# CrashCartCapital/rust-local-rag

Measured on AMD Instinct MI355X. Metric: queries/sec, 768-d cosine top-100 over 10M chunks (single query, f32), higher is better.
Workload: dtype f32

## Files before the change

rust-local-rag_amd/build.py:

```python
from __future__ import annotations

import os
import subprocess
import sys
from concurrent.futures import ThreadPoolExecutor

HERE = os.path.dirname(os.path.abspath(__file__))
CSRC = os.path.join(HERE, "csrc")
OBJ = os.path.join(HERE, "_obj")
SO = os.path.join(HERE, "librlr_gpu.so")
ROOT = os.path.dirname(HERE)

SOURCES = ["scan.hip", "select.hip", "tail.hip", "exact.hip", "gemm.hip", "index.hip", "engine.cpp", "multi.cpp", "lexical.hip", "q8.hip",
           "jsonio.cpp", "text_batch.cpp"]
HEADERS = ["common.h", "kernels.h", "exact_dot.h", "lds_select.h", "staged_dot.h", "select_dev.h", "sort_emit.h", "pool_prepare.h",
           "engine_host.h", "lexical_internal.h", os.path.join(ROOT, "include", "rlr_gpu.h"),
           os.path.join(ROOT, "include", "rlr_engine.h"), os.path.join(ROOT, "include", "rlr_lexical.h")]

FLAGS = ["--offload-arch=gfx950", "-O3", "-std=c++17", "-fPIC", "-ffp-contract=off", "-fno-fast-math",
         "-Wall", "-Wno-unused-function", "-I", os.path.join(ROOT, "include")]


def _hipcc() -> str:
    for c in (os.environ.get("HIPCC"), "/opt/rocm/bin/hipcc", "hipcc"):
        if c and (os.path.isabs(c) and os.path.exists(c) or not os.path.isabs(c)):
            return c
    return "hipcc"


def _newest_header() -> float:
    t = 0.0
    for h in HEADERS:
        p = h if os.path.isabs(h) else os.path.join(CSRC, h)
        if os.path.exists(p):
            t = max(t, os.path.getmtime(p))
    return t


def _compile(src: str, force: bool, keep_temps: bool) -> str:
    sp = os.path.join(CSRC, src)
    obj = os.path.join(OBJ, os.path.splitext(src)[0] + ".o")
    stale = force or not os.path.exists(obj) or os.path.getmtime(obj) < max(os.path.getmtime(sp), _newest_header())
    if stale:
        cmd = [_hipcc(), *FLAGS, "-c", sp, "-o", obj]
        if src.endswith(".cpp"):
            cmd.insert(1, "-x")
            cmd.insert(2, "hip")
        if keep_temps:
            cmd += ["-save-temps=obj"]
        r = subprocess.run(cmd, capture_output=True, text=True, cwd=OBJ)
        if r.returncode != 0:
            raise RuntimeError(f"hipcc failed for {src}:\n{r.stdout}\n{r.stderr}")
        if r.stderr.strip():
            sys.stderr.write(r.stderr)
    return obj


def build(force: bool = False, keep_temps: bool = False) -> str:
    os.makedirs(OBJ, exist_ok=True)
    srcs = [s for s in SOURCES if os.path.exists(os.path.join(CSRC, s))]
    with ThreadPoolExecutor(max_workers=min(6, len(srcs))) as ex:
        objs = list(ex.map(lambda s: _compile(s, force, keep_temps), srcs))
    if force or not os.path.exists(SO) or any(os.path.getmtime(o) > os.path.getmtime(SO) for o in objs):
        cmd = [_hipcc(), "--offload-arch=gfx950", "-shared", "-fPIC", "-o", SO, *objs]
        r = subprocess.run(cmd, capture_output=True, text=True)
        if r.returncode != 0:
            raise RuntimeError(f"link failed:\n{r.stdout}\n{r.stderr}")
    return SO


if __name__ == "__main__":
    print(build(force="--force" in sys.argv, keep_temps="--keep-temps" in sys.argv))
```

rust-local-rag_amd/csrc/exact.hip:

```cpp
#include "common.h"
#include "exact_dot.h"
#include "staged_dot.h"
#include "sort_emit.h"
#include "kernels.h"
#include "../../include/rlr_gpu.h"

#include <algorithm>
#include <atomic>
#include <cstdlib>
#include <cstring>

namespace rlr {

namespace {

__device__ inline void stage_query(float *s_q, const float *__restrict__ query, uint32_t dim)
{
    for (uint32_t i = threadIdx.x; i < dim; i += blockDim.x)
        s_q[i] = query[i];
    __syncthreads();
}

template <bool F16>
__global__ __launch_bounds__(64) void rescore_kernel(const float4 *__restrict__ rows, uint32_t pitch16,
                                                     uint32_t dim, const float *__restrict__ query,
                                                     const uint32_t *__restrict__ cand,
                                                     const SelectState *__restrict__ st,
                                                     uint64_t *__restrict__ packed_out, uint32_t n_pad)
{
    extern __shared__ __attribute__((aligned(16))) float s_q[];
    stage_query(s_q, query, dim);
    const uint32_t n = min(st->n_cand, st->cap);
    const uint32_t i = blockIdx.x * 64 + threadIdx.x;
    if (i >= n_pad)
        return;
    if (i >= n) {
        packed_out[i] = 0;
        return;
    }
    const uint32_t r = cand[i];
    const float s = dot_ref_row<F16>(rows + static_cast<size_t>(r) * pitch16, s_q, dim);
    packed_out[i] = pack_result(s, r);
}

template <bool F16>
__global__ __launch_bounds__(256) void rescore_staged_kernel(const float4 *__restrict__ rows, uint32_t pitch16,
                                                             uint32_t dim, const float *__restrict__ query,
                                                             const uint32_t *__restrict__ cand,
                                                             const SelectState *__restrict__ st,
                                                             uint64_t *__restrict__ packed_out, uint32_t cpb,
                                                             uint32_t *__restrict__ hist_clear)
{
    extern __shared__ __attribute__((aligned(16))) float s_mem[];
    const uint32_t q_floats = (dim + 7) & ~7u;
    float *s_q = s_mem;
    float *s_p = s_mem + q_floats;
    const uint32_t tid = threadIdx.x;
    const uint32_t gid = blockIdx.x * 256 + tid;
    if (hist_clear && gid < 2 * kHistBins)
        hist_clear[gid] = 0;
    const uint32_t n = min(st->n_cand, st->cap);
    const uint32_t base = blockIdx.x * cpb;
    if (base >= n)
        return;
    const uint32_t cnt = min(cpb, n - base);
    __shared__ uint32_t s_cand[16];
    for (uint32_t i = tid; i < q_floats; i += 256)
        s_q[i] = i < dim ? query[i] : 0.0f;
    if (tid < cnt)
        s_cand[tid] = cand[base + tid];
    __syncthreads();
    const float sc = staged_reference_dot<F16>(rows, pitch16, dim, s_q, s_p, s_cand, cnt, tid);
    if (tid < cnt)
        packed_out[base + tid] = pack_result(sc, s_cand[tid]);
}

template <bool F16>
__global__ __launch_bounds__(256) void batch_rescore_kernel(const float4 *__restrict__ rows, uint32_t pitch16,
                                                            uint32_t dim, const float *__restrict__ queries,
                                                            uint32_t q_pitch, uint64_t *__restrict__ band,
                                                            uint32_t band_stride, const SelectState *__restrict__ st,
                                                            uint32_t cpb)
{
    extern __shared__ __attribute__((aligned(16))) float s_mem[];
    const uint32_t q_floats = (dim + 7) & ~7u;
    float *s_q = s_mem;
    float *s_p = s_mem + q_floats;
    __shared__ uint32_t s_cand[16];
    const uint32_t tid = threadIdx.x;
    const uint32_t q = blockIdx.y;
    const uint32_t n = st[q].pad;
    if (blockIdx.x * cpb >= n)
        return;
    const float *query = queries + static_cast<size_t>(q) * q_pitch;
    for (uint32_t i = tid; i < q_floats; i += 256)
        s_q[i] = i < dim ? query[i] : 0.0f;
    uint64_t *b = band + static_cast<size_t>(q) * band_stride;
    for (uint32_t base = blockIdx.x * cpb; base < n; base += gridDim.x * cpb) {
        const uint32_t cnt = min(cpb, n - base);
        __syncthreads();
        if (tid < cnt)
            s_cand[tid] = 0xFFFFFFFFu - static_cast<uint32_t>(b[base + tid] & 0xFFFFFFFFu);
        __syncthreads();
        const float sc = staged_reference_dot<F16>(rows, pitch16, dim, s_q, s_p, s_cand, cnt, tid);
        if (tid < cnt)
            b[base + tid] = pack_result(sc, s_cand[tid]);
    }
}

template <bool F16>
__global__ __launch_bounds__(64) void score_rows_kernel(const float4 *__restrict__ rows, uint32_t pitch16,
                                                        uint32_t dim, const float *__restrict__ query,
                                                        const uint32_t *__restrict__ list, uint32_t n,
                                                        float *__restrict__ out, const uint32_t *__restrict__ n_dev,
                                                        uint32_t n_rows_clamp)
{
    extern __shared__ __attribute__((aligned(16))) float s_q[];
    stage_query(s_q, query, dim);
    if (n_dev)
        n = min(n, *n_dev);
    const uint32_t i = blockIdx.x * 64 + threadIdx.x;
    if (i >= n)
        return;
    const uint32_t r = list[i] < n_rows_clamp ? list[i] : 0u;
    out[i] = dot_ref_row<F16>(rows + static_cast<size_t>(r) * pitch16, s_q, dim);
}

template <bool F16>
__global__ __launch_bounds__(64) void score_rows_batch_kernel(const float4 *__restrict__ rows, uint32_t pitch16, uint32_t dim,
                                                              const float *__restrict__ queries, uint32_t q_pitch,
                                                              const uint32_t *__restrict__ list, uint32_t stride,
                                                              float *__restrict__ out, const uint32_t *__restrict__ n_dev,
                                                              uint32_t n_dev_stride, uint32_t n_rows_clamp)
{
    const uint32_t q = blockIdx.y;
    const uint32_t n = min(stride, n_dev[static_cast<size_t>(q) * n_dev_stride]);
    if (blockIdx.x * 64 >= n)
        return;
    extern __shared__ __attribute__((aligned(16))) float s_q[];
    stage_query(s_q, queries + static_cast<size_t>(q) * q_pitch, dim);
    const uint32_t i = blockIdx.x * 64 + threadIdx.x;
    if (i >= n)
        return;
    const size_t at = static_cast<size_t>(q) * stride + i;
    const uint32_t r = list[at] < n_rows_clamp ? list[at] : 0u;
    out[at] = dot_ref_row<F16>(rows + static_cast<size_t>(r) * pitch16, s_q, dim);
}

template <bool F16>
__global__ __launch_bounds__(256) void score_rows_staged_kernel(const float4 *__restrict__ rows, uint32_t pitch16, uint32_t dim,
                                                               const float *__restrict__ query,
                                                               const uint32_t *__restrict__ list, uint32_t n,
                                                               float *__restrict__ out, uint32_t cpb,
                                                               const uint32_t *__restrict__ n_dev, uint32_t n_rows_clamp)
{
    extern __shared__ __attribute__((aligned(16))) float s_mem[];
    const uint32_t q_floats = (dim + 7) & ~7u;
    float *s_q = s_mem;
    float *s_p = s_mem + q_floats;
    __shared__ uint32_t s_cand[16];
    const uint32_t tid = threadIdx.x;
    const uint32_t base = blockIdx.x * cpb;
    if (n_dev)
        n = min(n, *n_dev);
    if (base >= n)
        return;
    const uint32_t cnt = min(cpb, n - base);
    for (uint32_t i = tid; i < q_floats; i += 256)
        s_q[i] = i < dim ? query[i] : 0.0f;
    if (tid < cnt) {
        const uint32_t r = list[base + tid];
        s_cand[tid] = r < n_rows_clamp ? r : 0u;
    }
    __syncthreads();
    const float sc = staged_reference_dot<F16>(rows, pitch16, dim, s_q, s_p, s_cand, cnt, tid);
    if (tid < cnt)
        out[base + tid] = sc;
}

__global__ __launch_bounds__(64) void sumsq_kernel(const float *__restrict__ staging, uint32_t n,
                                                   uint32_t dim, float *__restrict__ sumsq)
{
    const uint32_t r = blockIdx.x * 64 + threadIdx.x;
    if (r >= n)
        return;
    const float *v = staging + static_cast<size_t>(r) * dim;
    float s = 0.0f;
    for (uint32_t c = 0; c < dim; ++c) {
        float p = v[c] * v[c];
        s = s + p;
    }
    sumsq[r] = s;
}

__device__ inline float sqrt_rn(float x)
{
    float y = __builtin_sqrtf(x);
    const double xd = static_cast<double>(x);
#pragma unroll
    for (int it = 0; it < 2; ++it) {
        const uint32_t yb = __builtin_bit_cast(uint32_t, y);
        const float up = __builtin_bit_cast(float, yb + 1u);
        const float dn = __builtin_bit_cast(float, yb - 1u);
        const double m_hi = 0.5 * (static_cast<double>(y) + static_cast<double>(up));
        const double m_lo = 0.5 * (static_cast<double>(y) + static_cast<double>(dn));
        if (xd > m_hi * m_hi)
            y = up;
        else if (xd < m_lo * m_lo)
            y = dn;
    }
    return y;
}

__device__ inline float ref_scale(float v, float norm_sq, int do_normalize)
{
    if (do_normalize && norm_sq > 1e-20f)
        return __fdiv_rn(v, sqrt_rn(norm_sq));
    return v;
}

template <bool F16>
__global__ __launch_bounds__(256) void scale_store_kernel(const float *__restrict__ staging,
                                                          const float *__restrict__ sumsq, uint32_t n,
                                                          uint32_t dim, int do_normalize,
                                                          void *__restrict__ rows_out, uint32_t pitch16)
{
    const uint32_t pitch_e = F16 ? pitch16 * 8 : pitch16 * 4;
    const size_t total = static_cast<size_t>(n) * pitch_e;
    const size_t stride = static_cast<size_t>(gridDim.x) * 256;
    for (size_t i = static_cast<size_t>(blockIdx.x) * 256 + threadIdx.x; i < total; i += stride) {
        const uint32_t r = static_cast<uint32_t>(i / pitch_e);
        const uint32_t c = static_cast<uint32_t>(i - static_cast<size_t>(r) * pitch_e);
        float v = 0.0f;
        if (c < dim)
            v = ref_scale(staging[static_cast<size_t>(r) * dim + c], do_normalize ? sumsq[r] : 0.0f,
                          do_normalize);
        if constexpr (F16)
            static_cast<_Float16 *>(rows_out)[i] = static_cast<_Float16>(v);
        else
            static_cast<float *>(rows_out)[i] = v;
    }
}

__device__ inline uint64_t mix64(uint64_t z)
{
    z = (z ^ (z >> 30)) * 0xBF58476D1CE4E5B9ULL;
    z = (z ^ (z >> 27)) * 0x94D049BB133111EBULL;
    return z ^ (z >> 31);
}

__device__ inline int32_t ih4(uint64_t h)
{
    return static_cast<int32_t>((h & 0xFFFF) + ((h >> 16) & 0xFFFF) + ((h >> 32) & 0xFFFF) + (h >> 48)) - 131070;
}

__device__ inline float synth_raw(uint64_t s, uint64_t row, uint32_t col, uint32_t d, uint32_t n_clusters)
{
    const uint64_t idx = row * static_cast<uint64_t>(d) + col;
    int32_t t = ih4(mix64(s + (idx + 1) * 0x9E3779B97F4A7C15ULL));
    const bool tight = (n_clusters & 0x80000000u) != 0;
    n_clusters &= 0x7FFFFFFFu;
    if (n_clusters) {
        const uint64_t cl = mix64(s ^ (row + 0x632BE59BD9B4E019ULL)) % n_clusters;
        const uint64_t cidx = cl * static_cast<uint64_t>(d) + col;
        const int32_t c = ih4(mix64((s ^ 0xC1A57E55C1A57E55ULL) + (cidx + 1) * 0x9E3779B97F4A7C15ULL));
        if (tight)
            t = t / 16;
        t += 2 * c;
    }
    return static_cast<float>(t) * (1.0f / 65536.0f);
}

__global__ __launch_bounds__(64) void synth_sumsq_kernel(uint64_t s, uint64_t row0, uint32_t n, uint32_t dim,
                                                         uint32_t n_clusters, float *__restrict__ sumsq)
{
    const uint32_t r = blockIdx.x * 64 + threadIdx.x;
    if (r >= n)
        return;
    float acc = 0.0f;
    for (uint32_t c = 0; c < dim; ++c) {
        const float v = synth_raw(s, row0 + r, c, dim, n_clusters);
        float p = v * v;
        acc = acc + p;
    }
    sumsq[r] = acc;
}

template <bool F16>
__global__ __launch_bounds__(256) void synth_store_kernel(uint64_t s, uint64_t row0, uint32_t n, uint32_t dim,
                                                          uint32_t n_clusters, const float *__restrict__ sumsq,
                                                          void *__restrict__ rows_out, uint32_t pitch16)
{
    const uint32_t pitch_e = F16 ? pitch16 * 8 : pitch16 * 4;
    const size_t total = static_cast<size_t>(n) * pitch_e;
    const size_t stride = static_cast<size_t>(gridDim.x) * 256;
    for (size_t i = static_cast<size_t>(blockIdx.x) * 256 + threadIdx.x; i < total; i += stride) {
        const uint32_t r = static_cast<uint32_t>(i / pitch_e);
        const uint32_t c = static_cast<uint32_t>(i - static_cast<size_t>(r) * pitch_e);
        float v = 0.0f;
        if (c < dim)
            v = ref_scale(synth_raw(s, row0 + r, c, dim, n_clusters), sumsq[r], 1);
        if constexpr (F16)
            static_cast<_Float16 *>(rows_out)[i] = static_cast<_Float16>(v);
        else
            static_cast<float *>(rows_out)[i] = v;
    }
}

template <bool F16>
__global__ __launch_bounds__(256) void gather_f32_kernel(const void *__restrict__ rows, uint32_t pitch16,
                                                         uint32_t dim, const uint32_t *__restrict__ list,
                                                         uint32_t n, float *__restrict__ out)
{
    const size_t total = static_cast<size_t>(n) * dim;
    const size_t stride = static_cast<size_t>(gridDim.x) * 256;
    for (size_t i = static_cast<size_t>(blockIdx.x) * 256 + threadIdx.x; i < total; i += stride) {
        const uint32_t k = static_cast<uint32_t>(i / dim);
        const uint32_t c = static_cast<uint32_t>(i - static_cast<size_t>(k) * dim);
        const size_t r = list[k];
        if constexpr (F16)
            out[i] = h2f(static_cast<const uint16_t *>(rows)[r * pitch16 * 8 + c]);
        else
            out[i] = static_cast<const float *>(rows)[r * pitch16 * 4 + c];
    }
}

__global__ __launch_bounds__(256) void compact_rows_kernel(const float4 *__restrict__ src, float4 *__restrict__ dst,
                                                           uint32_t pitch16, const uint32_t *__restrict__ keep,
                                                           uint32_t n_keep)
{
    const size_t total = static_cast<size_t>(n_keep) * pitch16;
    const size_t stride = static_cast<size_t>(gridDim.x) * 256;
    for (size_t i = static_cast<size_t>(blockIdx.x) * 256 + threadIdx.x; i < total; i += stride) {
        const uint32_t k = static_cast<uint32_t>(i / pitch16);
        const uint32_t u = static_cast<uint32_t>(i - static_cast<size_t>(k) * pitch16);
        dst[i] = src[static_cast<size_t>(keep[k]) * pitch16 + u];
    }
}

__device__ inline bool finite_f(float x)
{
    return (__builtin_bit_cast(uint32_t, x) & 0x7F800000u) != 0x7F800000u;
}

__device__ inline float gram_entry(float dot)
{
    return finite_f(dot) ? dot : -__builtin_inff();
}

__global__ __launch_bounds__(64) void gram_kernel(const float *__restrict__ pool, uint32_t P, uint32_t dim,
                                                  float *__restrict__ gram)
{
    pool += static_cast<size_t>(blockIdx.z) * P * dim;
    gram += static_cast<size_t>(blockIdx.z) * P * P;
    const uint32_t i = blockIdx.y;
    const uint32_t j = blockIdx.x * 64 + threadIdx.x;
    if (j > i || i >= P)
        return;
    const float *a = pool + static_cast<size_t>(i) * dim;
    const float *b = pool + static_cast<size_t>(j) * dim;
    float s = 0.0f;
    uint32_t c = 0;
    if ((dim & 3u) == 0) {
        const float4 *a4 = reinterpret_cast<const float4 *>(a);
        const float4 *b4 = reinterpret_cast<const float4 *>(b);
        for (; c + 16 <= dim; c += 16) {
            float4 x[4], y[4];
#pragma unroll
            for (int u = 0; u < 4; ++u) {
                x[u] = a4[c / 4 + u];
                y[u] = b4[c / 4 + u];
            }
#pragma unroll
            for (int u = 0; u < 4; ++u) {
                float p;
                p = x[u].x * y[u].x; s = s + p;
                p = x[u].y * y[u].y; s = s + p;
                p = x[u].z * y[u].z; s = s + p;
                p = x[u].w * y[u].w; s = s + p;
            }
        }
    }
    for (; c < dim; ++c) {
        float p = a[c] * b[c];
        s = s + p;
    }
    s = gram_entry(s);
    gram[static_cast<size_t>(i) * P + j] = s;
    gram[static_cast<size_t>(j) * P + i] = s;
}

template <int SRC>
__device__ inline float4 gram_load4(const float *pool, const void *rows, uint32_t pitch16, uint32_t dim, uint32_t row, uint32_t col)
{
    if constexpr (SRC == 2) {
        const uint2 h = *reinterpret_cast<const uint2 *>(static_cast<const uint16_t *>(rows) + static_cast<size_t>(row) * pitch16 * 8 + col);
        return make_float4(h2f(static_cast<uint16_t>(h.x)), h2f(static_cast<uint16_t>(h.x >> 16)), h2f(static_cast<uint16_t>(h.y)),
                           h2f(static_cast<uint16_t>(h.y >> 16)));
    } else if constexpr (SRC == 1) {
        return *reinterpret_cast<const float4 *>(static_cast<const float *>(rows) + static_cast<size_t>(row) * pitch16 * 4 + col);
    } else {
        return *reinterpret_cast<const float4 *>(pool + static_cast<size_t>(row) * dim + col);
    }
}


template <int R, int SRC, int GK>
__global__ __launch_bounds__(256) void gram_tiled_kernel(const float *__restrict__ pool, uint32_t P, uint32_t dim,
                                                         float *__restrict__ gram, const void *__restrict__ rows,
                                                         uint32_t pitch16, const uint32_t *__restrict__ list)
{
    constexpr int kGT = 16 * R;
    constexpr int kGK = GK, kGPitch = GK + 4;
    __shared__ __attribute__((aligned(16))) float sa[kGT * kGPitch];
    __shared__ __attribute__((aligned(16))) float sb[kGT * kGPitch];
    if constexpr (SRC == 0)
        pool += static_cast<size_t>(blockIdx.z) * P * dim;
    else
        list += static_cast<size_t>(blockIdx.z) * P;
    gram += static_cast<size_t>(blockIdx.z) * P * P;
    uint32_t bi = 0, rem = blockIdx.x;
    while (rem > bi) {
        rem -= bi + 1;
        ++bi;
    }
    const uint32_t bj = rem;
    const uint32_t i0 = bi * kGT, j0 = bj * kGT;
    const uint32_t t = threadIdx.x, ty = t >> 4, tx = t & 15;
    float acc[R][R];
#pragma unroll
    for (int a = 0; a < R; ++a)
#pragma unroll
        for (int b = 0; b < R; ++b)
            acc[a][b] = 0.0f;
    const bool vec = (dim & 3u) == 0;
    constexpr int kPre = 2 * kGT * (kGK / 4) / 256;
    float4 pre[kPre];
    uint32_t src_row[kPre];
#pragma unroll
    for (int u = 0; u < kPre; ++u) {
        const uint32_t r = (t + 256 * u) / (kGK / 4);
        const uint32_t row = min(r >= kGT ? j0 + (r - kGT) : i0 + r, P - 1);
        src_row[u] = SRC == 0 ? row : list[row];
    }
    auto fetch = [&](uint32_t k0) {
        const uint32_t kc = min(static_cast<uint32_t>(kGK), dim - k0);
        if (vec) {
#pragma unroll
            for (int u = 0; u < kPre; ++u) {
                const uint32_t idx = t + 256 * u;
                const uint32_t r = idx / (kGK / 4), c4 = idx % (kGK / 4);
                const uint32_t row = r >= kGT ? j0 + (r - kGT) : i0 + r;
                const float4 v = gram_load4<SRC>(pool, rows, pitch16, dim, src_row[u], min(k0 + c4 * 4, dim - 4));
                pre[u] = (row < P && c4 * 4 < kc) ? v : make_float4(0.0f, 0.0f, 0.0f, 0.0f);
            }
            return;
        }
#pragma unroll
        for (int u = 0; u < kPre; ++u) {
            const uint32_t idx = t + 256 * u;
            const uint32_t r = idx / (kGK / 4), c4 = idx % (kGK / 4);
            const uint32_t row = r >= kGT ? j0 + (r - kGT) : i0 + r;
            float4 v = make_float4(0.0f, 0.0f, 0.0f, 0.0f);
            if (row < P && c4 * 4 < kc) {
                const uint32_t col = k0 + c4 * 4;
                if constexpr (SRC == 2) {
                    const uint16_t *src = static_cast<const uint16_t *>(rows) + static_cast<size_t>(src_row[u]) * pitch16 * 8 + col;
                    v.x = h2f(src[0]);
                    if (c4 * 4 + 1 < kc) v.y = h2f(src[1]);
                    if (c4 * 4 + 2 < kc) v.z = h2f(src[2]);
                    if (c4 * 4 + 3 < kc) v.w = h2f(src[3]);
                } else {
                    const float *src = SRC == 0 ? pool + static_cast<size_t>(row) * dim + col
                                                : static_cast<const float *>(rows) + static_cast<size_t>(src_row[u]) * pitch16 * 4 + col;
                    v.x = src[0];
                    if (c4 * 4 + 1 < kc) v.y = src[1];
                    if (c4 * 4 + 2 < kc) v.z = src[2];
                    if (c4 * 4 + 3 < kc) v.w = src[3];
                }
            }
            pre[u] = v;
        }
    };
    auto stash = [&]() {
#pragma unroll
        for (int u = 0; u < kPre; ++u) {
            const uint32_t idx = t + 256 * u;
            const uint32_t r = idx / (kGK / 4), c4 = idx % (kGK / 4);
            float *dst = (r >= kGT ? sb + (r - kGT) * kGPitch : sa + r * kGPitch) + c4 * 4;
            *reinterpret_cast<float4 *>(dst) = pre[u];
        }
    };
    fetch(0);
    stash();
    __syncthreads();
    for (uint32_t k0 = 0; k0 < dim; k0 += kGK) {
        const uint32_t kc = min(static_cast<uint32_t>(kGK), dim - k0);
        const bool more = k0 + kGK < dim;
        if (more)
            fetch(k0 + kGK);
        const uint32_t n4 = kc / 4;
        constexpr int kUnroll = R == 1 ? 8 : 1;
#pragma unroll kUnroll
        for (uint32_t c = 0; c < n4; ++c) {
            float4 xa[R], yb[R];
#pragma unroll
            for (int a = 0; a < R; ++a)
                xa[a] = reinterpret_cast<const float4 *>(sa + (ty + 16 * a) * kGPitch)[c];
#pragma unroll
            for (int b = 0; b < R; ++b)
                yb[b] = reinterpret_cast<const float4 *>(sb + (tx + 16 * b) * kGPitch)[c];
#pragma unroll
            for (int a = 0; a < R; ++a)
#pragma unroll
                for (int b = 0; b < R; ++b) {
                    float p;
                    p = xa[a].x * yb[b].x; acc[a][b] = acc[a][b] + p;
                    p = xa[a].y * yb[b].y; acc[a][b] = acc[a][b] + p;
                    p = xa[a].z * yb[b].z; acc[a][b] = acc[a][b] + p;
                    p = xa[a].w * yb[b].w; acc[a][b] = acc[a][b] + p;
                }
        }
        for (uint32_t e = n4 * 4; e < kc; ++e) {
#pragma unroll
            for (int a = 0; a < R; ++a)
#pragma unroll
                for (int b = 0; b < R; ++b) {
                    const float p = sa[(ty + 16 * a) * kGPitch + e] * sb[(tx + 16 * b) * kGPitch + e];
                    acc[a][b] = acc[a][b] + p;
                }
        }
        __syncthreads();
        if (more) {
            stash();
            __syncthreads();
        }
    }
#pragma unroll
    for (int a = 0; a < R; ++a)
#pragma unroll
        for (int b = 0; b < R; ++b) {
            const uint32_t ri = i0 + ty + 16 * a, cj = j0 + tx + 16 * b;
            if (ri < P && cj < P) {
                const float g = gram_entry(acc[a][b]);
                gram[static_cast<size_t>(ri) * P + cj] = g;
                gram[static_cast<size_t>(cj) * P + ri] = g;
            }
        }
}

__global__ __launch_bounds__(64) void mmr_greedy_kernel(const float *__restrict__ gram,
                                                        const float *__restrict__ scores, uint32_t P,
                                                        uint32_t k, float lambda, uint32_t *__restrict__ out_order,
                                                        float *__restrict__ out_mmr, uint32_t *__restrict__ out_n)
{
    extern __shared__ __attribute__((aligned(16))) unsigned char s_raw[];
    uint32_t *rem = reinterpret_cast<uint32_t *>(s_raw);
// ... 779 lines not shown
```

rust-local-rag_amd/csrc/exact_dot.h:

```cpp
#pragma once

#include "common.h"

namespace rlr {

template <bool F16>
__device__ inline float dot_ref_row(const float4 *__restrict__ row, const float *s_q, uint32_t dim)
{
    float s = 0.0f;
    constexpr uint32_t EPU = F16 ? 8 : 4;
    const uint32_t full = dim / EPU;
    uint32_t u = 0;
    for (; u + 4 <= full; u += 4) {
        float4 x[4];
#pragma unroll
        for (int i = 0; i < 4; ++i)
            x[i] = row[u + i];
#pragma unroll
        for (int i = 0; i < 4; ++i) {
            const float *q = s_q + (u + i) * EPU;
            if constexpr (F16) {
                const uint32_t w[4] = {__builtin_bit_cast(uint32_t, x[i].x), __builtin_bit_cast(uint32_t, x[i].y),
                                       __builtin_bit_cast(uint32_t, x[i].z), __builtin_bit_cast(uint32_t, x[i].w)};
#pragma unroll
                for (int j = 0; j < 4; ++j) {
                    float p0 = h2f(static_cast<uint16_t>(w[j] & 0xFFFF)) * q[2 * j];
                    s = s + p0;
                    float p1 = h2f(static_cast<uint16_t>(w[j] >> 16)) * q[2 * j + 1];
                    s = s + p1;
                }
            } else {
                float p;
                p = x[i].x * q[0]; s = s + p;
                p = x[i].y * q[1]; s = s + p;
                p = x[i].z * q[2]; s = s + p;
                p = x[i].w * q[3]; s = s + p;
            }
        }
    }
    if constexpr (F16) {
        const uint16_t *h = reinterpret_cast<const uint16_t *>(row);
        for (uint32_t e = u * EPU; e < dim; ++e) {
            float p = h2f(h[e]) * s_q[e];
            s = s + p;
        }
    } else {
        const float *f = reinterpret_cast<const float *>(row);
        for (uint32_t e = u * EPU; e < dim; ++e) {
            float p = f[e] * s_q[e];
            s = s + p;
        }
    }
    return s;
}

}
```

rust-local-rag_amd/csrc/gemm.hip:

```cpp
#include "common.h"
#include "exact_dot.h"
#include "kernels.h"
#include "lds_select.h"
#include "../../include/rlr_gpu.h"

#include <cstdlib>

namespace rlr {

namespace {

typedef _Float16 half8 __attribute__((ext_vector_type(8)));
typedef _Float16 half2v __attribute__((ext_vector_type(2)));
typedef float f32x4 __attribute__((ext_vector_type(4)));

constexpr int kQB = 256;
constexpr int kNB = kQB / 16;
constexpr int kRG = 2;
constexpr int kGemmWaves = 8;
constexpr int kBM = kGemmWaves * kRG * 16;
constexpr int kKsChunk = 2;
constexpr int kChunkFrags = kKsChunk * kNB * 64;

__global__ __launch_bounds__(256) void prep_queries_kernel(const float *__restrict__ q, uint32_t n_queries,
                                                           uint32_t q_pitch, uint32_t dim, uint32_t n_ksteps,
                                                           uint32_t n_qblocks, int f16_rows,
                                                           _Float16 *__restrict__ out)
{
    const size_t total = static_cast<size_t>(n_qblocks) * n_ksteps * kNB * 64 * 8;
    for (size_t e = static_cast<size_t>(blockIdx.x) * 256 + threadIdx.x; e < total; e += static_cast<size_t>(gridDim.x) * 256) {
        const uint32_t j = e & 7;
        const uint32_t lane = (e >> 3) & 63;
        const uint32_t nb = (e >> 9) & (kNB - 1);
        const size_t rest = e >> 13;
        const uint32_t ks = static_cast<uint32_t>(rest % n_ksteps);
        const uint32_t qb = static_cast<uint32_t>(rest / n_ksteps);
        const uint32_t query = qb * kQB + nb * 16 + (lane & 15);
        const uint32_t g = lane >> 4;
        const uint32_t k = ks * 32 + (f16_rows ? g * 8 + j : (j < 4 ? g * 4 + j : 16 + g * 4 + (j - 4)));
        float v = 0.0f;
        if (query < n_queries && k < dim)
            v = q[static_cast<size_t>(query) * q_pitch + k];
        out[e] = static_cast<_Float16>(v);
    }
}

__device__ inline half8 cvt8(float4 lo, float4 hi)
{
    half8 r;
    r[0] = static_cast<_Float16>(lo.x);
    r[1] = static_cast<_Float16>(lo.y);
    r[2] = static_cast<_Float16>(lo.z);
    r[3] = static_cast<_Float16>(lo.w);
    r[4] = static_cast<_Float16>(hi.x);
    r[5] = static_cast<_Float16>(hi.y);
    r[6] = static_cast<_Float16>(hi.z);
    r[7] = static_cast<_Float16>(hi.w);
    return r;
}

struct GemmArgs {
    const unsigned char *rows;
    uint32_t pitch_bytes;
    uint32_t row_begin, row_end;
    uint32_t n_ksteps;
    const half8 *qfrag;
    uint32_t n_qblocks, n_queries;
    const float *tau;
    uint64_t *cand;
    uint32_t cand_stride;
    SelectState *st;
    float *scores;
    size_t score_stride;
    uint32_t *sync;
    uint32_t sync_every;
    uint32_t a_nt_shared;
};

template <bool MATERIALISE>
__device__ __forceinline__ void gemm_epilogue(const GemmArgs &a, f32x4 (&acc)[kRG][kNB], uint32_t row0, uint32_t last_row,
                                              uint32_t qb, int lane)
{
    const uint32_t qcol = qb * kQB + (lane & 15);
    if constexpr (MATERIALISE) {
#pragma unroll
        for (int rg = 0; rg < kRG; ++rg) {
            const uint32_t r = row0 + rg * 16 + 4 * (lane >> 4);
            const uint32_t rel = r - a.row_begin;
#pragma unroll
            for (int nb = 0; nb < kNB; ++nb) {
                const uint32_t q = qcol + nb * 16;
                if (q >= a.n_queries)
                    continue;
                float *dst = a.scores + static_cast<size_t>(q) * a.score_stride + rel;
                const f32x4 v = acc[rg][nb];
                if (r + 3 <= last_row) {
                    *reinterpret_cast<float4 *>(dst) = make_float4(v[0], v[1], v[2], v[3]);
                } else {
#pragma unroll
                    for (int i = 0; i < 4; ++i)
                        if (r + i <= last_row)
                            dst[i] = v[i];
                }
            }
        }
    } else {
        float tau_l[kNB];
#pragma unroll
        for (int nb = 0; nb < kNB; ++nb) {
            const uint32_t q = qcol + nb * 16;
            tau_l[nb] = q < a.n_queries ? a.tau[q] : __builtin_inff();
        }
#pragma unroll
        for (int rg = 0; rg < kRG; ++rg) {
            const uint32_t r = row0 + rg * 16 + 4 * (lane >> 4);
#pragma unroll
            for (int nb = 0; nb < kNB; ++nb) {
                const f32x4 v = acc[rg][nb];
                const float t = tau_l[nb];
                if (v[0] >= t || v[1] >= t || v[2] >= t || v[3] >= t) {
                    const uint32_t q = qcol + nb * 16;
#pragma unroll
                    for (int i = 0; i < 4; ++i) {
                        if (v[i] >= t && r + i <= last_row) {
                            const uint32_t slot = atomicAdd(&a.st[q].n_cand, 1u);
                            if (slot < a.st[q].cap)
                                a.cand[static_cast<size_t>(q) * a.cand_stride + slot] = pack_result(v[i], r + i);
                        }
                    }
                }
            }
        }
    }
}

template <bool F16ROWS, bool MATERIALISE>
__global__ __launch_bounds__(512) void gemm_nominate_kernel(const GemmArgs a)
{
    __shared__ half8 s_b[2][kChunkFrags];

    const int tid = threadIdx.x;
    const int lane = tid & 63;
    const int wave = __builtin_amdgcn_readfirstlane(tid >> 6);
    const uint32_t bid = blockIdx.x;
    const uint32_t rt = (bid / (8 * a.n_qblocks)) * 8 + (bid & 7);
    const uint32_t qb = (bid >> 3) % a.n_qblocks;
    const uint32_t n_rows = a.row_end - a.row_begin;
    if (rt * kBM >= n_rows)
        return;
    const uint32_t row0 = a.row_begin + rt * kBM + wave * (kRG * 16);
    const uint32_t last_row = a.row_end - 1;

    const unsigned char *ap[kRG];
#pragma unroll
    for (int rg = 0; rg < kRG; ++rg) {
        const uint32_t r = min(row0 + rg * 16 + (lane & 15), last_row);
        ap[rg] = a.rows + static_cast<size_t>(r) * a.pitch_bytes + (lane >> 4) * 16;
    }
    constexpr int kStepBytes = F16ROWS ? 64 : 128;

    const uint32_t n_chunks = a.n_ksteps / kKsChunk;
    const half8 *bsrc = a.qfrag + static_cast<size_t>(qb) * a.n_ksteps * kNB * 64;

    f32x4 acc[kRG][kNB];
#pragma unroll
    for (int rg = 0; rg < kRG; ++rg)
#pragma unroll
        for (int nb = 0; nb < kNB; ++nb)
            acc[rg][nb] = f32x4{0.0f, 0.0f, 0.0f, 0.0f};

    half8 breg[4];
    float4 araw[kRG][kKsChunk][2];
    half8 a_cur[kRG][kKsChunk];

    auto load_b = [&](uint32_t c) {
#pragma unroll
        for (int i = 0; i < 4; ++i)
            breg[i] = bsrc[static_cast<size_t>(c) * kChunkFrags + tid + 512 * i];
    };
    auto store_b = [&](int buf) {
#pragma unroll
        for (int i = 0; i < 4; ++i)
            s_b[buf][tid + 512 * i] = breg[i];
    };
    auto load_a = [&](uint32_t c) {
#pragma unroll
        for (int rg = 0; rg < kRG; ++rg)
#pragma unroll
            for (int ks = 0; ks < kKsChunk; ++ks) {
                const unsigned char *p = ap[rg] + static_cast<size_t>(c * kKsChunk + ks) * kStepBytes;
                if constexpr (F16ROWS) {
                    araw[rg][ks][0] = *reinterpret_cast<const float4 *>(p);
                } else {
                    araw[rg][ks][0] = *reinterpret_cast<const float4 *>(p);
                    araw[rg][ks][1] = *reinterpret_cast<const float4 *>(p + 64);
                }
            }
    };
    auto convert_a = [&]() {
#pragma unroll
        for (int rg = 0; rg < kRG; ++rg)
#pragma unroll
            for (int ks = 0; ks < kKsChunk; ++ks) {
                if constexpr (F16ROWS)
                    a_cur[rg][ks] = __builtin_bit_cast(half8, araw[rg][ks][0]);
                else
                    a_cur[rg][ks] = cvt8(araw[rg][ks][0], araw[rg][ks][1]);
            }
    };

    load_b(0);
    load_a(0);
    store_b(0);
    convert_a();
    __syncthreads();

#pragma unroll 1
    for (uint32_t c = 0; c < n_chunks; ++c) {
        const bool has_next = c + 1 < n_chunks;
        if (has_next) {
            load_b(c + 1);
            load_a(c + 1);
        }
        const half8 *sb = s_b[c & 1];
#pragma unroll
        for (int ks = 0; ks < kKsChunk; ++ks) {
#pragma unroll
            for (int nb = 0; nb < kNB; ++nb) {
                const half8 b = sb[(ks * kNB + nb) * 64 + lane];
#pragma unroll
                for (int rg = 0; rg < kRG; ++rg)
                    acc[rg][nb] = __builtin_amdgcn_mfma_f32_16x16x32_f16(a_cur[rg][ks], b, acc[rg][nb], 0, 0, 0);
            }
        }
        if (has_next) {
            store_b((c + 1) & 1);
            convert_a();
        }
        __syncthreads();
    }

    gemm_epilogue<MATERIALISE>(a, acc, row0, last_row, qb, lane);
}

template <bool F16ROWS>
__global__ __launch_bounds__(256) void build_image_kernel(const unsigned char *__restrict__ rows, uint32_t pitch_bytes,
                                                          uint32_t n_rows, uint32_t n_chunks, uint32_t tile_begin,
                                                          uint32_t tile_end, half8 *__restrict__ image)
{
    const size_t per_tile = static_cast<size_t>(n_chunks) * 8 * 4 * 64;
    const size_t first = static_cast<size_t>(tile_begin) * per_tile;
    const size_t total = static_cast<size_t>(tile_end - tile_begin) * per_tile;
    for (size_t i = static_cast<size_t>(blockIdx.x) * 256 + threadIdx.x; i < total; i += static_cast<size_t>(gridDim.x) * 256) {
        const size_t e = first + i;
        const uint32_t lane = e & 63;
        const uint32_t ks = (e >> 6) & 1;
        const uint32_t rg = (e >> 7) & 1;
        const uint32_t w = (e >> 8) & 7;
        const size_t tc = e >> 11;
        const uint32_t c = static_cast<uint32_t>(tc % n_chunks);
        const uint32_t t = static_cast<uint32_t>(tc / n_chunks);
        const uint32_t row = t * 256 + w * 32 + rg * 16 + (lane & 15);
        const uint32_t k = c * 64 + ks * 32 + (lane >> 4) * 8;
        half8 v;
#pragma unroll
        for (int j = 0; j < 8; ++j)
            v[j] = static_cast<_Float16>(0.0f);
        if (row < n_rows) {
            const unsigned char *src = rows + static_cast<size_t>(row) * pitch_bytes;
            if constexpr (F16ROWS) {
                v = *reinterpret_cast<const half8 *>(src + k * 2);
            } else {
                const float4 lo = *reinterpret_cast<const float4 *>(src + k * 4);
                const float4 hi = *reinterpret_cast<const float4 *>(src + k * 4 + 16);
                v = cvt8(lo, hi);
            }
        }
        image[e] = v;
    }
}

constexpr int kRGI = 4;

template <bool MATERIALISE, int NBW>
__device__ __forceinline__ void gemm_image_epilogue(const GemmArgs &a, f32x4 (&acc)[kRGI][NBW], uint32_t row0,
                                                    uint32_t last_row, uint32_t q0, int lane)
{
    constexpr int kNBI = NBW;
    const uint32_t qcol = q0 + (lane & 15);
    if constexpr (MATERIALISE) {
#pragma unroll
        for (int rg = 0; rg < kRGI; ++rg) {
            const uint32_t r = row0 + rg * 16 + 4 * (lane >> 4);
            const uint32_t rel = r - a.row_begin;
#pragma unroll
            for (int nb = 0; nb < kNBI; ++nb) {
                const uint32_t q = qcol + nb * 16;
                if (q >= a.n_queries)
                    continue;
                float *dst = a.scores + static_cast<size_t>(q) * a.score_stride + rel;
                const f32x4 v = acc[rg][nb];
                if (r + 3 <= last_row) {
                    *reinterpret_cast<float4 *>(dst) = make_float4(v[0], v[1], v[2], v[3]);
                } else {
#pragma unroll
                    for (int i = 0; i < 4; ++i)
                        if (r + i <= last_row)
                            dst[i] = v[i];
                }
            }
        }
    } else {
        float tau_l[kNBI];
#pragma unroll
        for (int nb = 0; nb < kNBI; ++nb) {
            const uint32_t q = qcol + nb * 16;
            tau_l[nb] = q < a.n_queries ? a.tau[q] : __builtin_inff();
        }
#pragma unroll
        for (int rg = 0; rg < kRGI; ++rg) {
            const uint32_t r = row0 + rg * 16 + 4 * (lane >> 4);
#pragma unroll
            for (int nb = 0; nb < kNBI; ++nb) {
                const f32x4 v = acc[rg][nb];
                const float t = tau_l[nb];
                if (v[0] >= t || v[1] >= t || v[2] >= t || v[3] >= t) {
                    const uint32_t q = qcol + nb * 16;
#pragma unroll
                    for (int i = 0; i < 4; ++i) {
                        if (v[i] >= t && r + i <= last_row) {
                            const uint32_t slot = atomicAdd(&a.st[q].n_cand, 1u);
                            if (slot < a.st[q].cap)
                                a.cand[static_cast<size_t>(q) * a.cand_stride + slot] = pack_result(v[i], r + i);
                        }
                    }
                }
            }
        }
    }
}

constexpr int kHalfBytes = 16384;
constexpr uint32_t kG8ListCap = 2048;
constexpr int kG8OffPack = 8 * kHalfBytes;
constexpr int kG8OffQid = kG8OffPack + kG8ListCap * 8;
constexpr int kG8OffTau = kG8OffQid + kG8ListCap * 4;
constexpr int kG8OffCnt = kG8OffTau + 2 * 256 * 4;
constexpr int kG8LdsBytes = kG8OffCnt + 64;

#define RLR_GLDS16(src, dst)                                                                               \
    __builtin_amdgcn_global_load_lds((const __attribute__((address_space(1))) void *)(src),                \
                                     (__attribute__((address_space(3))) void *)(dst), 16, 0, 0)
#define RLR_FENCE() asm volatile("" ::: "memory")

__device__ __forceinline__ uint32_t lds_add_rtn_u32(uint32_t addr, uint32_t v)
{
    uint32_t r;
// ... 441 lines not shown
                                                                                 acc[rg][nb], 0, 0, 0);
                }
                RLR_RES_LOAD_A(min(cc + kResSlots, last_c), sl);
                __builtin_amdgcn_sched_barrier(0);
            }
        }
    }
#undef RLR_RES_LOAD_A
    gemm_image_epilogue<MATERIALISE, kResNB>(a, acc, row0, last_row, qg * kResQ, lane);
}

constexpr uint32_t kFinCap = 8192;
constexpr uint32_t kBandCap = 2048;

__device__ inline void bitonic_desc_lds(uint64_t *s, uint32_t n_pad, uint32_t nthreads)
{
    for (uint32_t k = 2; k <= n_pad; k <<= 1) {
        for (uint32_t j = k >> 1; j > 0; j >>= 1) {
            for (uint32_t i = threadIdx.x; i < n_pad; i += nthreads) {
                const uint32_t ixj = i ^ j;
                if (ixj > i) {
                    const uint64_t x = s[i], y = s[ixj];
                    const bool desc = (i & k) == 0;
                    if (desc ? (x < y) : (x > y)) {
                        s[i] = y;
                        s[ixj] = x;
                    }
                }
            }
            __syncthreads();
        }
    }
}

template <bool F16ROWS>
__global__ __launch_bounds__(256) void batch_finish_kernel(const float4 *__restrict__ rows, uint32_t pitch16, uint32_t dim,
                                                           const float *__restrict__ queries, uint32_t q_pitch,
                                                           const uint64_t *__restrict__ cand, uint32_t cand_stride,
                                                           const SelectState *__restrict__ st, uint32_t k, float two_eps,
                                                           uint64_t *__restrict__ out, uint32_t *__restrict__ status)
{
    __shared__ uint64_t s_c[kFinCap];
    __shared__ uint32_t s_band;
    extern __shared__ __attribute__((aligned(16))) float s_q[];
    const uint32_t q = blockIdx.x;
    const uint32_t n_raw = st[q].n_cand;
    uint64_t *o = out + static_cast<size_t>(q) * k;
    if (n_raw > st[q].cap || n_raw > kFinCap || n_raw < k) {
        if (threadIdx.x == 0)
            status[q] = n_raw < k ? 2u : 1u;
        return;
    }
    for (uint32_t i = threadIdx.x; i < dim; i += 256)
        s_q[i] = queries[static_cast<size_t>(q) * q_pitch + i];
    uint32_t n_pad = 1;
    while (n_pad < n_raw)
        n_pad <<= 1;
    const uint64_t *c = cand + static_cast<size_t>(q) * cand_stride;
    for (uint32_t i = threadIdx.x; i < n_pad; i += 256)
        s_c[i] = i < n_raw ? c[i] : 0ull;
    if (threadIdx.x == 0)
        s_band = 0;
    __syncthreads();
    bitonic_desc_lds(s_c, n_pad, 256);
    const float fk = key_score(static_cast<uint32_t>(s_c[k - 1] >> 32));
    const uint32_t key_lo = score_key(fk - two_eps);
    if (key_lo < st[q].key_lo) {
        if (threadIdx.x == 0)
            status[q] = 2u;
        return;
    }
    for (uint32_t i = threadIdx.x; i < n_raw; i += 256)
        if (static_cast<uint32_t>(s_c[i] >> 32) >= key_lo)
            atomicMax(&s_band, i + 1);
    __syncthreads();
    const uint32_t band = s_band;
    if (band > kBandCap) {
        if (threadIdx.x == 0)
            status[q] = 1u;
        return;
    }
    for (uint32_t i = threadIdx.x; i < band; i += 256) {
        const uint32_t r = 0xFFFFFFFFu - static_cast<uint32_t>(s_c[i] & 0xFFFFFFFFu);
        const float e = dot_ref_row<F16ROWS>(rows + static_cast<size_t>(r) * pitch16, s_q, dim);
        s_c[i] = pack_result(e, r);
    }
    uint32_t b_pad = 1;
    while (b_pad < band)
        b_pad <<= 1;
    for (uint32_t i = band + threadIdx.x; i < b_pad; i += 256)
        s_c[i] = 0ull;
    __syncthreads();
    bitonic_desc_lds(s_c, b_pad, 256);
    for (uint32_t i = threadIdx.x; i < k; i += 256)
        o[i] = s_c[i];
    if (threadIdx.x == 0)
        status[q] = 0u;
}

__global__ __launch_bounds__(1024) void batch_band_kernel(uint64_t *__restrict__ cand, uint32_t cand_stride,
                                                          SelectState *__restrict__ st, uint32_t k, float two_eps,
                                                          uint32_t *__restrict__ status)
{
    __shared__ uint64_t s_c[kFinCap];
    __shared__ uint32_t s_hist[2048];
    __shared__ uint32_t s_sel[3];
    __shared__ uint32_t s_band;
    const uint32_t q = blockIdx.x;
    const uint32_t n_raw = st[q].n_cand;
    if (n_raw > st[q].cap || n_raw > kFinCap || n_raw < k) {
        if (threadIdx.x == 0) {
            status[q] = n_raw < k ? 2u : 1u;
            st[q].pad = 0;
        }
        return;
    }
    uint64_t *c = cand + static_cast<size_t>(q) * cand_stride;
    for (uint32_t i = threadIdx.x; i < n_raw; i += 1024)
        s_c[i] = c[i];
    if (threadIdx.x == 0)
        s_band = 0;
    __syncthreads();
    const float fk = key_score(lds_kth_key(s_c, n_raw, k, s_hist, s_sel, 1024));
    const uint32_t key_lo = score_key(fk - two_eps);
    if (key_lo < st[q].key_lo) {
        if (threadIdx.x == 0) {
            status[q] = 2u;
            st[q].pad = 0;
        }
        return;
    }
    for (uint32_t i = threadIdx.x; i < n_raw; i += 1024) {
        const uint64_t v = s_c[i];
        if (static_cast<uint32_t>(v >> 32) >= key_lo) {
            const uint32_t slot = atomicAdd(&s_band, 1u);
            if (slot < kBandCap)
                c[slot] = v;
        }
    }
    __syncthreads();
    const uint32_t band = s_band;
    if (threadIdx.x == 0) {
        if (band > kBandCap) {
            status[q] = 1u;
            st[q].pad = 0;
        } else {
            st[q].pad = band;
            status[q] = 0u;
        }
    }
}

__global__ __launch_bounds__(1024) void batch_tighten_kernel(uint64_t *__restrict__ cand, uint32_t cand_stride,
                                                             SelectState *__restrict__ st, uint32_t k, float two_eps,
                                                             float *__restrict__ tau)
{
    __shared__ uint64_t s_c[kFinCap];
    __shared__ uint32_t s_keep;
    const uint32_t q = blockIdx.x;
    const uint32_t n_raw = st[q].n_cand;
    if (n_raw > st[q].cap || n_raw > kFinCap || n_raw < k)
        return;
    uint32_t n_pad = 1;
    while (n_pad < n_raw)
        n_pad <<= 1;
    uint64_t *c = cand + static_cast<size_t>(q) * cand_stride;
    for (uint32_t i = threadIdx.x; i < n_pad; i += 1024)
        s_c[i] = i < n_raw ? c[i] : 0ull;
    if (threadIdx.x == 0)
        s_keep = 0;
    __syncthreads();
    bitonic_desc_lds(s_c, n_pad, 1024);
    const float fk = key_score(static_cast<uint32_t>(s_c[k - 1] >> 32));
    const uint32_t key_lo = score_key(fk - two_eps);
    for (uint32_t i = threadIdx.x; i < n_raw; i += 1024)
        if (static_cast<uint32_t>(s_c[i] >> 32) >= key_lo)
            atomicMax(&s_keep, i + 1);
    __syncthreads();
    const uint32_t keep = s_keep;
    for (uint32_t i = threadIdx.x; i < keep; i += 1024)
        c[i] = s_c[i];
    if (threadIdx.x == 0) {
        st[q].n_cand = keep;
        tau[q] = key_lo == 0 ? -__builtin_inff() : key_score(key_lo);
    }
}

__global__ __launch_bounds__(1024) void batch_emit_kernel(const uint64_t *__restrict__ cand, uint32_t cand_stride,
                                                          const SelectState *__restrict__ st, uint32_t k,
                                                          uint64_t *__restrict__ out)
{
    __shared__ uint64_t s_c[kBandCap];
    const uint32_t q = blockIdx.x;
    const uint32_t band = st[q].pad;
    if (band == 0)
        return;
    uint32_t b_pad = 1;
    while (b_pad < band)
        b_pad <<= 1;
    const uint64_t *c = cand + static_cast<size_t>(q) * cand_stride;
    for (uint32_t i = threadIdx.x; i < b_pad; i += 1024)
        s_c[i] = i < band ? c[i] : 0ull;
    __syncthreads();
    bitonic_desc_lds(s_c, b_pad, 1024);
    uint64_t *o = out + static_cast<size_t>(q) * k;
    for (uint32_t i = threadIdx.x; i < k; i += 1024)
        o[i] = s_c[i];
}

}

float nomination_eps(uint32_t dim, int dtype, float prod, float norm_sum)
{
    const float op = dtype == RLR_F16 ? 4.8828125e-4f : 9.765625e-4f;
    const float acc = 2.0f * (static_cast<float>(dim) + 64.0f) * 5.9604645e-8f;
    const float sub = 2.9802322e-8f * __builtin_sqrtf(static_cast<float>(dim));
    return ((op * 1.001f + acc) * prod + sub * norm_sum) * 1.0625f;
}

hipError_t launch_prep_queries(const float *q, uint32_t n_queries, uint32_t q_pitch, uint32_t dim, int dtype,
                               void *qfrag, hipStream_t s)
{
    const uint32_t n_ksteps = dim / 32;
    const uint32_t n_qblocks = (n_queries + kQB - 1) / kQB;
    const size_t total = static_cast<size_t>(n_qblocks) * n_ksteps * kNB * 64 * 8;
    const uint32_t blocks = static_cast<uint32_t>(std::min<size_t>((total + 255) / 256, 4096));
    hipLaunchKernelGGL(prep_queries_kernel, dim3(blocks), dim3(256), 0, s, q, n_queries, q_pitch, dim, n_ksteps,
                       n_qblocks, dtype == RLR_F16 ? 1 : 0, static_cast<_Float16 *>(qfrag));
    return hipGetLastError();
}

bool gemm_image_usable(uint32_t dim)
{
    return dim % 128 == 0;
}

static uint32_t persistent_grid()
{
    static uint32_t cus[64] = {0};
    int dev = 0;
    if (hipGetDevice(&dev) != hipSuccess || dev < 0 || dev >= 64)
        return 256;
    if (cus[dev] == 0) {
        int n = 0;
        if (hipDeviceGetAttribute(&n, hipDeviceAttributeMultiprocessorCount, dev) != hipSuccess || n < 8)
            n = 256;
        cus[dev] = static_cast<uint32_t>(n) / 8 * 8;
    }
    return cus[dev];
}

hipError_t launch_gemm_nominate(const void *rows, uint32_t pitch16, uint32_t dim, int dtype, uint32_t row_begin,
                                uint32_t row_end, const void *qfrag, uint32_t n_queries, const float *tau,
                                uint64_t *cand, uint32_t cand_stride, SelectState *st, float *scores,
                                size_t score_stride, const void *image, hipStream_t s, uint32_t *sync_ws)
{
    if (row_end <= row_begin)
        return hipSuccess;
    GemmArgs a;
    a.rows = static_cast<const unsigned char *>(rows);
    a.pitch_bytes = pitch16 * 16;
    a.row_begin = row_begin;
    a.row_end = row_end;
    a.n_ksteps = dim / 32;
    a.qfrag = static_cast<const half8 *>(qfrag);
    a.n_qblocks = (n_queries + kQB - 1) / kQB;
    a.n_queries = n_queries;
    a.tau = tau;
    a.cand = cand;
    a.cand_stride = cand_stride;
    a.st = st;
    a.scores = scores;
    a.score_stride = score_stride;
    a.sync = nullptr;
    a.sync_every = 4;
    a.a_nt_shared = 0;
    const uint32_t n_rt = (row_end - row_begin + kBM - 1) / kBM;
    const uint32_t grid = ((n_rt + 7) / 8) * 8 * a.n_qblocks;
    const bool mat = scores != nullptr;
    static const uint32_t resident_max = [] {
        const char *v = getenv("RLR_GEMM_RESIDENT_MAX");
        return v ? static_cast<uint32_t>(strtoul(v, nullptr, 0)) : 128u;
    }();
    if (image && n_queries <= resident_max && row_begin % kBM == 0 && a.n_ksteps <= kResMaxKsteps &&
        a.n_ksteps % (kKsChunk * kResSlots) == 0) {
        const half8 *img = static_cast<const half8 *>(image);
        const uint32_t n_qg = (n_queries + kResQ - 1) / kResQ;
        const uint32_t n_rg = (row_end - row_begin + kResRows - 1) / kResRows;
        const uint32_t rgrid = ((n_rg + 7) / 8) * 8 * n_qg;
        if (mat)
            hipLaunchKernelGGL((gemm_resident_kernel<true>), dim3(rgrid), dim3(512), 0, s, a, img, n_qg);
        else
            hipLaunchKernelGGL((gemm_resident_kernel<false>), dim3(rgrid), dim3(512), 0, s, a, img, n_qg);
        return hipGetLastError();
    }
    if (image && row_begin % kBM == 0 && a.n_ksteps % 4 == 0) {
        const uint32_t n_units = n_rt * a.n_qblocks;
        const uint32_t g8 = std::max<uint32_t>(8, std::min<uint32_t>(persistent_grid(), (n_units + 7) / 8 * 8));
        const char *img = static_cast<const char *>(image);
        static const bool no_sync = getenv("RLR_GEMM8_NO_SIBLING_SYNC") != nullptr;
        if (sync_ws && a.n_qblocks > 1 && g8 == persistent_grid() && !no_sync) {
            const hipError_t e = hipMemsetAsync(sync_ws, 0, 256 * sizeof(uint32_t), s);
            if (e != hipSuccess)
                return e;
            a.sync = sync_ws;
            static const uint32_t every = getenv("RLR_GEMM8_SYNC_EVERY") ? static_cast<uint32_t>(std::max(1, atoi(getenv("RLR_GEMM8_SYNC_EVERY")))) : 4u;
            a.sync_every = every;
        }
        static const bool a_nt = getenv("RLR_GEMM8_A_NT") != nullptr;
        a.a_nt_shared = a_nt ? 1u : 0u;
        static const int var = [] {
// ... 127 lines not shown
```

rust-local-rag_amd/csrc/index.hip:

```cpp
#include "../../include/rlr_gpu.h"
#include "common.h"
#include "kernels.h"
#include "lds_select.h"
#include "sort_emit.h"
#include "pool_prepare.h"
#include "lexical_internal.h"

#include <algorithm>
#include <atomic>
#include <chrono>
#include <cmath>
#include <condition_variable>
#include <cstdarg>
#include <cstdio>
#include <cstring>
#include <mutex>
#include <memory>
#include <new>
#include <string>
#include <thread>
#include <vector>

#include <time.h>

using namespace rlr;

namespace {

thread_local char g_err[512] = "";

int32_t fail(int32_t code, const char *fmt, ...)
{
    va_list ap;
    va_start(ap, fmt);
    vsnprintf(g_err, sizeof(g_err), fmt, ap);
    va_end(ap);
    return code;
}

}

namespace rlr {
int32_t set_error(int32_t code, const char *fmt, ...)
{
    va_list ap;
    va_start(ap, fmt);
    vsnprintf(g_err, sizeof(g_err), fmt, ap);
    va_end(ap);
    return code;
}
}

namespace {

#define RLR_HIP(call)                                                                              \
    do {                                                                                           \
        hipError_t e_ = (call);                                                                    \
        if (e_ != hipSuccess)                                                                      \
            return fail(e_ == hipErrorOutOfMemory ? RLR_E_OOM : RLR_E_HIP, "%s failed: %s (%s:%d)", \
                        #call, hipGetErrorString(e_), __FILE__, __LINE__);                         \
    } while (0)

#define RLR_TRY(call)                                                                              \
    do {                                                                                           \
        int32_t s_ = (call);                                                                       \
        if (s_ != RLR_OK)                                                                          \
            return s_;                                                                             \
    } while (0)

constexpr uint32_t kLdsSortCap = 4096;
constexpr uint32_t kMaxDim = 8192;

uint32_t next_pow2(uint32_t v)
{
    uint32_t p = 1;
    while (p < v)
        p <<= 1;
    return p;
}

struct RowBlock {
    void *raw = nullptr;
    size_t raw_bytes = 0;
    std::vector<hipMemGenericAllocationHandle_t> handles;
    size_t slab = 0;
// ... 10 lines not shown
    float *d_query = nullptr;
    uint32_t q_cap = 0;
    float *d_scores = nullptr;
    uint64_t score_cap = 0;
    uint32_t *d_hist = nullptr;
    SelectState *d_state = nullptr;
    uint32_t *d_cand = nullptr;
    uint64_t *d_packed = nullptr;
    uint32_t cand_cap = 0;
    uint64_t *d_out = nullptr;
    uint64_t out_cap = 0;
    uint32_t *d_list = nullptr;
    float *d_vals = nullptr;
    uint32_t list_cap = 0;
    float *d_pool = nullptr;
    uint64_t pool_cap = 0;
    void *d_qfrag = nullptr;
    uint64_t qfrag_cap = 0;
    float *d_tau = nullptr;
    SelectState *d_bstate = nullptr;
    uint32_t *d_bhist = nullptr;
    uint32_t *d_bstatus = nullptr;
    uint32_t *d_gsync = nullptr;
    void *h_batch = nullptr;
    uint32_t bq_cap = 0;
    bool no_f16 = false;
    uint64_t *d_bcand = nullptr;
    uint64_t bcand_cap = 0;
    float *d_sample = nullptr;
    uint64_t sample_cap = 0;
    hipEvent_t bev[5] = {nullptr, nullptr, nullptr, nullptr, nullptr};
    void *h_pin = nullptr;
    size_t h_pin_bytes = 0;
    std::vector<float> q_norm;
    WaitEma wait_ema;
    const float *h_q_kq = nullptr;
    bool hist_dirty = false;
    uint32_t *h_assert = nullptr;
    hipStream_t pending_stream = nullptr;
    uint32_t pending_q = 0, pending_k = 0;
    bool pending_timed = false;
    const uint64_t *pending_meta = nullptr;
};

struct CoalesceMember {
    const float *query;
    uint32_t k;
    uint64_t *rows_out;
    float *cos_out;
    uint32_t *n_out;
};

struct CoalesceGroup {
    uint32_t key = 0;
    uint32_t cap = 0;
    std::vector<CoalesceMember *> members;
    bool sealed = false;
    bool go = false;
    bool done = false;
    int32_t status = 0;
    char msg[512] = "";
};

}

struct rlr_index {
    uint32_t dim = 0;
    int32_t dtype = RLR_F32;
    int32_t device = 0;
    uint32_t pitch16 = 0;
    uint32_t q_pitch = 0;
    uint64_t n_rows = 0;
    uint64_t cap_rows = 0;
    void *d_rows = nullptr;
    RowBlock rows_block;
    int n_cu = 256;
    int scan_variant = 0;
    int fused_tail = -1;
    uint32_t tail_direct_max = 3584;
    bool hybrid_fetch_full = false;
    uint32_t batch_min = 0;
    float max_row_sumsq = 1.0f;
    bool f16_overflow = false;
    bool image_enabled = false;
    bool image_scan = false;
    bool q8_enabled = false;
    void *d_q8 = nullptr;
    float *d_q8_scale = nullptr;
    uint32_t *d_q8_stats = nullptr;
    uint64_t q8_cap_rows = 0;
    float q8_delta = 0.0f, q8_scale_max = 0.0f;
    bool q8_has_inf = false;
    void *d_image = nullptr;
    size_t image_cap = 0;
    std::mutex mu;
    std::condition_variable ctx_cv;
    std::vector<Ctx *> free_ctx;
    int ctx_made = 0;
    int ctx_cap = 16;
    bool profiling = false;
    rlr_profile prof{};
    std::atomic<uint32_t> co_max{0};
    uint32_t co_linger_us = 0;
    std::mutex co_mu;
    std::condition_variable co_cv;
    int co_running = 0;
    std::vector<std::shared_ptr<CoalesceGroup>> co_pending;
    rlr_coalesce_stats co_stats{};
};

namespace {

size_t row_bytes(const rlr_index *ix)
{
    return static_cast<size_t>(ix->pitch16) * 16;
}

}

namespace rlr {
bool poison_mode()
{
    static const bool poison = [] {
        const char *v = getenv("RLR_POISON_ALLOC");
        return v && v[0] == '1';
    }();
    return poison;
}

hipError_t dev_malloc(void **p, size_t bytes)
{
    const bool poison = poison_mode();
    hipError_t e = hipMalloc(p, bytes);
    if (e != hipSuccess)
        (void)hipGetLastError();
    if (e == hipSuccess && poison && bytes) {
        e = hipMemset(*p, 0xFF, bytes);
        if (e == hipSuccess)
            e = hipDeviceSynchronize();
    }
    return e;
}
}

namespace {
int32_t use_device(const rlr_index *ix)
{
    RLR_HIP(hipSetDevice(ix->device));
    return RLR_OK;
}

template <typename T>
int32_t grow(T **p, uint64_t *cap, uint64_t want, bool keep = false)
{
    if (*cap >= want && *p)
        return RLR_OK;
    T *n = nullptr;
    RLR_HIP(rlr::dev_malloc(reinterpret_cast<void **>(&n), want * sizeof(T)));
    if (keep && *p && *cap) {
        RLR_HIP(hipMemcpy(n, *p, *cap * sizeof(T), hipMemcpyDeviceToDevice));
        RLR_HIP(hipStreamSynchronize(nullptr));
    }
    if (*p)
        (void)hipFree(*p);
    *p = n;
    *cap = want;
// ... 452 lines not shown
    const uint64_t want = std::max<uint64_t>(ix->cap_rows, ix->n_rows);
    if (ix->q8_cap_rows < want || !ix->d_q8) {
        if (ix->d_q8) (void)hipFree(ix->d_q8);
        if (ix->d_q8_scale) (void)hipFree(ix->d_q8_scale);
        ix->d_q8 = nullptr;
        ix->d_q8_scale = nullptr;
        ix->q8_cap_rows = 0;
        RLR_HIP(rlr::dev_malloc(&ix->d_q8, std::max<uint64_t>(want, 1) * ix->dim));
        RLR_HIP(rlr::dev_malloc(reinterpret_cast<void **>(&ix->d_q8_scale), std::max<uint64_t>(want, 1) * sizeof(float)));
        ix->q8_cap_rows = want;
        first_row = 0;
    }
    if (!ix->d_q8_stats)
        RLR_HIP(rlr::dev_malloc(reinterpret_cast<void **>(&ix->d_q8_stats), 4 * sizeof(uint32_t)));
    if (first_row == 0)
        RLR_HIP(hipMemset(ix->d_q8_stats, 0, 4 * sizeof(uint32_t)));
    RLR_HIP(launch_q8_build(ix->d_rows, ix->pitch16, ix->dim, ix->dtype, static_cast<uint32_t>(first_row),
                            static_cast<uint32_t>(ix->n_rows), ix->d_q8, ix->d_q8_scale, ix->d_q8_stats, nullptr));
    uint32_t h[4] = {0, 0, 0, 0};
    RLR_HIP(hipMemcpy(h, ix->d_q8_stats, sizeof(h), hipMemcpyDeviceToHost));
    std::memcpy(&ix->q8_delta, &h[0], 4);
    std::memcpy(&ix->q8_scale_max, &h[1], 4);
    ix->q8_has_inf = h[2] != 0;
    return RLR_OK;
}

int32_t sync_image(rlr_index *ix, uint64_t first_row)
{
    RLR_TRY(sync_q8(ix, first_row));
    if (!ix->image_enabled)
        return RLR_OK;
    const size_t need = image_bytes(ix->dim, std::max<uint64_t>(ix->cap_rows, ix->n_rows));
    if (ix->image_cap < need) {
        if (ix->d_image)
            (void)hipFree(ix->d_image);
        ix->d_image = nullptr;
        ix->image_cap = 0;
        RLR_HIP(rlr::dev_malloc(&ix->d_image, std::max<size_t>(need, 256)));
        ix->image_cap = std::max<size_t>(need, 256);
        first_row = 0;
    }
    const uint32_t t0 = static_cast<uint32_t>(first_row / 256);
    const uint32_t t1 = static_cast<uint32_t>((ix->n_rows + 255) / 256);
    RLR_HIP(launch_build_image(ix->d_rows, ix->pitch16, ix->dim, ix->dtype, static_cast<uint32_t>(ix->n_rows), t0, t1,
                               ix->d_image, nullptr));
    RLR_HIP(hipStreamSynchronize(nullptr));
    return RLR_OK;
}

static bool beyond_f16(const float *v, uint32_t n)
{
    for (uint32_t i = 0; i < n; ++i)
        if (std::fabs(v[i]) > 65504.0f)
            return true;
    return false;
}

constexpr double kF16MaxSq = 65504.0 * 65504.0;

int32_t ingest(rlr_index *ix, const float *rows, uint64_t n, uint64_t first, int normalize)
{
    if (n == 0)
        return RLR_OK;
    const uint64_t chunk_rows = std::max<uint64_t>(1, (64ull << 20) / (static_cast<uint64_t>(ix->dim) * 4));
    float *d_stage = nullptr, *d_norm = nullptr;
    const uint64_t cr = std::min(chunk_rows, n);
    RLR_HIP(rlr::dev_malloc(reinterpret_cast<void **>(&d_stage), cr * ix->dim * sizeof(float)));
    hipError_t e = rlr::dev_malloc(reinterpret_cast<void **>(&d_norm), cr * sizeof(float));
    if (e != hipSuccess) {
        (void)hipFree(d_stage);
        return fail(RLR_E_OOM, "staging allocation failed");
    }
    int32_t st = RLR_OK;
    std::vector<float> h_norm;
    for (uint64_t r0 = 0; r0 < n && st == RLR_OK; r0 += cr) {
        const uint64_t m = std::min(cr, n - r0);
        e = hipMemcpy(d_stage, rows + r0 * ix->dim, m * ix->dim * sizeof(float), hipMemcpyHostToDevice);
        if (e == hipSuccess)
            e = launch_normalize_store(d_stage, static_cast<uint32_t>(m), ix->dim, normalize,
                                       static_cast<char *>(ix->d_rows) + (first + r0) * row_bytes(ix), ix->pitch16,
                                       ix->dtype, d_norm, nullptr);
        if (e == hipSuccess)
            e = hipStreamSynchronize(nullptr);
        if (e == hipSuccess && !normalize) {
            h_norm.resize(m);
            e = hipMemcpy(h_norm.data(), d_norm, m * sizeof(float), hipMemcpyDeviceToHost);
            for (uint64_t i = 0; i < m && e == hipSuccess; ++i) {
                if (h_norm[i] > ix->max_row_sumsq)
                    ix->max_row_sumsq = h_norm[i];
                if (ix->dtype == RLR_F32 && !ix->f16_overflow && h_norm[i] > 0.999 * kF16MaxSq &&
                    beyond_f16(rows + (r0 + i) * ix->dim, ix->dim))
                    ix->f16_overflow = true;
            }
        }
        if (e != hipSuccess)
            st = fail(RLR_E_HIP, "row ingest failed: %s", hipGetErrorString(e));
    }
    (void)hipFree(d_stage);
    (void)hipFree(d_norm);
    return st;
}

enum WaitMode { kWaitHybrid = 0, kWaitSpin = 1, kWaitBlock = 2 };

WaitMode wait_mode()
{
    static const WaitMode m = [] {
        const char *v = getenv("RLR_WAIT");
        if (v && v[0] == 's')
            return kWaitSpin;
        if (v && v[0] == 'b')
            return kWaitBlock;
        return kWaitHybrid;
    }();
    return m;
}

inline void cpu_relax()
{
#if defined(__x86_64__) || defined(__i386__)
    __builtin_ia32_pause();
#else
    __asm__ __volatile__("" ::: "memory");
#endif
}

template <typename Complete>
int32_t wait_polling(Complete &&complete, hipStream_t s, WaitEma *c, uint32_t key)
{
    using clk = std::chrono::steady_clock;
    const WaitMode mode = wait_mode();
    if (mode == kWaitBlock) {
        RLR_HIP(hipStreamSynchronize(s));
        return RLR_OK;
    }
    const auto t0 = clk::now();
    bool slept = false;
    if (c && c->key != key) {
        c->key = key;
        c->us = 0.0;
    }
    if (mode == kWaitHybrid && c && c->us > 1500.0) {
        const double sleep_us = 0.7 * c->us - 150.0;
        if (sleep_us > 20.0) {
            timespec ts;
            clock_gettime(CLOCK_MONOTONIC, &ts);
            const long add = static_cast<long>(sleep_us * 1000.0);
            ts.tv_sec += (ts.tv_nsec + add) / 1000000000L;
            ts.tv_nsec = (ts.tv_nsec + add) % 1000000000L;
            (void)clock_nanosleep(CLOCK_MONOTONIC, TIMER_ABSTIME, &ts, nullptr);
            slept = true;
        }
    }
    uint32_t polls = 0;
    for (;;) {
        std::atomic_thread_fence(std::memory_order_acquire);
        if (complete())
            break;
        if ((++polls & 0x3FFu) == 0) {
            const hipError_t e = hipStreamQuery(s);
            if (e == hipSuccess) {
                bool ok = false;
                for (int spin = 0; spin < 100000 && !ok; ++spin) {
                    std::atomic_thread_fence(std::memory_order_acquire);
                    ok = complete();
                    cpu_relax();
                }
                if (ok)
                    break;
// ... 633 lines not shown
        if (!status && got < n_rows && got > 0) {
            const float t0 = w_e * key_score(s_emin);
            const float t1 = w_l * 0.0f;
            const float c_tail = t0 + t1;
            const bool ok = n_cand >= need && (c_tail != c_tail || s_cneed > c_tail);
            if (!ok)
                status = 2u;
        }
        info[0] = status ? 0u : n_pool;
        info[1] = status;
        s_pick[0] = status;
    }
    if (h_out) {
        __syncthreads();
        const uint32_t status = s_pick[0];
        hybrid_emit_body(list, comb, cosv, lexv, status ? 0u : min(n_pool, k_cap), status, k_cap, h_out);
    }
}

__global__ __launch_bounds__(1024) void hybrid_pool_kernel(const uint64_t *__restrict__ packed, uint32_t fetch, uint32_t need,
                                                           uint32_t n_rows, float w_e, float w_l,
                                                           const uint32_t *__restrict__ lrow, const float *__restrict__ lscore,
                                                           const float *__restrict__ lcos,
                                                           const HybridLexHeader *__restrict__ hdr,
                                                           float *__restrict__ cand, uint32_t *__restrict__ list,
                                                           float *__restrict__ comb, float *__restrict__ cosv,
                                                           float *__restrict__ lexv, uint32_t *__restrict__ info,
                                                           uint32_t k_cap, uint32_t *__restrict__ h_out)
{
    hybrid_pool_body(packed, fetch, need, n_rows, w_e, w_l, lrow, lscore, lcos, hdr, cand, list, comb, cosv, lexv, info, k_cap,
                     h_out);
}

__global__ __launch_bounds__(1024) void hybrid_pool_batch_kernel(const uint64_t *__restrict__ packed, uint32_t fetch, uint32_t need,
                                                                 uint32_t n_rows, float w_e, float w_l, uint32_t bound,
                                                                 const uint32_t *__restrict__ lrow, const float *__restrict__ lscore,
                                                                 const float *__restrict__ lcos,
                                                                 const HybridLexHeader *__restrict__ hdr, float *__restrict__ cand,
                                                                 uint32_t *__restrict__ list, float *__restrict__ comb,
                                                                 float *__restrict__ cosv, float *__restrict__ lexv,
                                                                 uint32_t *__restrict__ info, uint32_t *__restrict__ sizes)
{
    const uint32_t q = blockIdx.x;
    const size_t lo = static_cast<size_t>(q) * bound, po = static_cast<size_t>(q) * need;
    hybrid_pool_body(packed + static_cast<size_t>(q) * fetch, fetch, need, n_rows, w_e, w_l, lrow + lo, lscore + lo, lcos + lo,
                     hdr + q, cand + static_cast<size_t>(q) * 3 * kHybridSlots, list + po, comb + po, cosv + po, lexv + po,
                     info + 2 * q, 0u, nullptr);
    if (threadIdx.x == 0)
        sizes[q] = info[2 * q];
}

__global__ __launch_bounds__(256) void hybrid_emit_kernel(const uint32_t *__restrict__ list, const float *__restrict__ comb,
                                                          const float *__restrict__ cosv, const float *__restrict__ lexv,
                                                          const uint32_t *__restrict__ info, uint32_t k_cap,
                                                          uint32_t *__restrict__ h_out)
{
    hybrid_emit_body(list, comb, cosv, lexv, info[1] ? 0u : min(info[0], k_cap), info[1], k_cap, h_out);
}
}

namespace {

bool scan_over_image(const rlr_index *ix, const Ctx *c)
{
    return ix->image_scan && ix->image_enabled && ix->d_image && ix->dtype == RLR_F32 && !(c && c->no_f16);
}

void stage_query_norms(const rlr_index *ix, Ctx *c, const float *queries, uint32_t nq)
{
    if (!ix->q8_enabled)
        return;
    c->q_norm.resize(nq);
    for (uint32_t q = 0; q < nq; ++q) {
        const double s2 = sumsq_f64(queries + static_cast<size_t>(q) * ix->dim, ix->dim);
        c->q_norm[q] = std::isfinite(s2) ? static_cast<float>(std::sqrt(s2) * 1.000001) : 1.0f;
    }
}

bool scan_over_q8(const rlr_index *ix)
{
    return ix->q8_enabled && ix->d_q8 && !ix->q8_has_inf;
}

bool scans_take_host_query(const rlr_index *ix, const Ctx *c, const float *h_q)
{
    if (scan_over_q8(ix) || scan_over_image(ix, c) || ix->n_rows == 0)
        return false;
    ScanArgs sa;
    sa.rows = ix->d_rows;
    sa.query = nullptr;
    sa.scores = nullptr;
    sa.hist = nullptr;
    sa.n_rows = static_cast<uint32_t>(ix->n_rows);
    sa.dim = ix->dim;
    sa.pitch16 = ix->pitch16;
    sa.dtype = ix->dtype;
    sa.n_cu = ix->n_cu;
    sa.variant = ix->scan_variant;
    sa.query_host = h_q;
    return launch_scan_takes_host_query(sa);
}

float q8_two_eps(const rlr_index *ix, float q_norm, float guard_eps)
{
    const float dflt = rlr_default_guard_eps(ix->dim);
    const float scale = guard_eps > dflt ? guard_eps / dflt : 1.0f;
    const float qn = q_norm * 1.0001f + 1e-30f;
    return 2.0f * (ix->q8_delta * qn + q8_arith_eps(ix->dim, ix->q8_scale_max, qn) + dflt) * scale;
}

float image_two_eps(const rlr_index *ix, float eps, const SearchPlan &p)
{
    const float dflt = rlr_default_guard_eps(ix->dim) * p.scale;
    const float scale = eps > dflt ? eps / dflt : 1.0f;
    return 2.0f * nomination_eps(ix->dim, ix->dtype, p.scale, p.norm_sum) * scale;
}

void count_f16_fallbacks(rlr_index *ix, const SearchPlan &p, uint32_t nq, bool batch_f16)
{
    if (p.f16_ok || !(batch_f16 || scan_over_image(ix, nullptr)))
        return;
    std::lock_guard<std::mutex> lk(ix->mu);
    ix->prof.n_f16_range_fallbacks += nq;
}

int32_t check_hist_assert(Ctx *c)
{
    if (c->h_assert && *c->h_assert) {
        const uint32_t n = *c->h_assert;
        *c->h_assert = 0;
        return fail(RLR_E_INTERNAL, "zero-histogram invariant violated: %u non-zero bins in front of a scan", n);
    }
    return RLR_OK;
}

hipError_t enqueue_query_scan(rlr_index *ix, Ctx *c, uint32_t qi, bool timed)
{
    hipStream_t s = c->stream;
    hipError_t e;
    const uint32_t n = static_cast<uint32_t>(ix->n_rows);
    uint32_t *hist1 = c->d_hist;
    const float *dq = c->d_query + static_cast<size_t>(qi) * ix->q_pitch;

    if (c->h_assert) {
        hipLaunchKernelGGL(rlr::hist_assert_zero_kernel, dim3(4), dim3(256), 0, s, c->d_hist, 2u * kHistBins, c->h_assert);
        if ((e = hipGetLastError()) != hipSuccess) return e;
    }
    if (timed && (e = hipEventRecord(c->ev[0], s)) != hipSuccess) return e;
    ScanArgs sa;
    sa.rows = ix->d_rows;
    sa.query = dq;
    sa.scores = c->d_scores;
    sa.hist = hist1;
    sa.n_rows = n;
    sa.dim = ix->dim;
    sa.pitch16 = ix->pitch16;
    sa.dtype = ix->dtype;
    sa.n_cu = ix->n_cu;
    sa.variant = ix->scan_variant;
    sa.query_host = c->h_q_kq ? c->h_q_kq + static_cast<size_t>(qi) * ix->q_pitch : nullptr;
    static const bool variant_dyn = getenv("RLR_SCAN_VARIANT_DYN") != nullptr;
    if (variant_dyn)
        if (const char *v = getenv("RLR_SCAN_VARIANT"))
            sa.variant = static_cast<int>(strtol(v, nullptr, 0));
    const bool q8 = scan_over_q8(ix);
    const bool img = !q8 && scan_over_image(ix, c);
    if (q8)
        e = launch_q8_scan(ix->d_q8, ix->d_q8_scale, n, ix->dim, dq, c->d_scores, hist1, ix->n_cu, s);
    else if (img)
        e = launch_scan_image(ix->d_image, n, ix->dim, dq, c->d_scores, hist1, ix->n_cu, s);
    else
        e = launch_scan(sa, s);
    if (e != hipSuccess) return e;
    if (timed && (e = hipEventRecord(c->ev[1], s)) != hipSuccess) return e;
    return hipSuccess;
}

hipError_t enqueue_query_rest(rlr_index *ix, Ctx *c, uint32_t qi, const SearchPlan &p, uint64_t *d_out_q, uint64_t *d_meta_q,
                              bool timed, bool emit = true, const PoolArgs *pool = nullptr, bool *pool_done = nullptr)
{
    if (pool_done)
        *pool_done = false;
    hipStream_t s = c->stream;
    hipError_t e;
    const uint32_t n = static_cast<uint32_t>(ix->n_rows);
    uint32_t *hist1 = c->d_hist, *hist2 = c->d_hist + kHistBins;
    SelectState *st = c->d_state + qi;
    const float *dq = c->d_query + static_cast<size_t>(qi) * ix->q_pitch;
    const bool q8 = scan_over_q8(ix);
    const bool img = !q8 && scan_over_image(ix, c);
    const float band = q8 ? q8_two_eps(ix, qi < c->q_norm.size() ? c->q_norm[qi] : 1.0f, p.two_eps * 0.5f)
                          : (img ? p.two_eps_img : p.two_eps);
    const bool fused = ix->fused_tail < 0 ? ix->n_rows <= 4000000ull : ix->fused_tail != 0;
    if (fused && p.cap <= kLdsSortCap && tail_fits(ix->pitch16, ix->dim, ix->dtype)) {
        TailArgs ta;
        ta.scores = c->d_scores;
        ta.n = n;
        ta.hist = c->d_hist;
        ta.st = st;
        ta.k = p.k;
        ta.cap = p.cap;
        ta.two_eps = band;
        ta.rows = ix->d_rows;
        ta.pitch16 = ix->pitch16;
        ta.dim = ix->dim;
        ta.dtype = ix->dtype;
        ta.query = dq;
        ta.packed = c->d_packed;
        ta.out = emit ? d_out_q : nullptr;
        ta.meta = d_meta_q;
        ta.unordered = p.unordered;
        ta.pool = emit ? nullptr : pool;
        ta.direct_max = ta.pool ? std::min<uint32_t>(ix->tail_direct_max, 1024u) : ix->tail_direct_max;
        ta.n_cu = ix->n_cu;
        if (pool_done)
            *pool_done = ta.pool != nullptr;
        if ((e = launch_tail_stage1(ta, s)) != hipSuccess) return e;
        if (timed && (e = hipEventRecord(c->ev[2], s)) != hipSuccess) return e;
        if ((e = launch_tail_stage2(ta, s)) != hipSuccess) return e;
        if (timed && (e = hipEventRecord(c->ev[3], s)) != hipSuccess) return e;
        return hipSuccess;
    }
    if ((e = launch_hist2_find1(c->d_scores, n, hist1, hist2, st, p.k, p.cap, ix->n_cu, s)) != hipSuccess) return e;
    if ((e = launch_collect_find2(c->d_scores, n, hist2, st, band, c->d_cand, ix->n_cu, s)) != hipSuccess)
        return e;
    if (timed && (e = hipEventRecord(c->ev[2], s)) != hipSuccess) return e;
    const uint32_t n_max = std::min<uint32_t>(p.cap, kLdsSortCap);
    if (!launch_rescore_staged(ix->d_rows, ix->pitch16, ix->dim, ix->dtype, dq, c->d_cand, st, c->d_packed, n_max,
                               c->d_hist, s, &e)) {
        if ((e = launch_rescore(ix->d_rows, ix->pitch16, ix->dim, ix->dtype, dq, c->d_cand, st, c->d_packed, n_max, s)) !=
            hipSuccess)
            return e;
        e = hipMemsetAsync(c->d_hist, 0, 2 * kHistBins * sizeof(uint32_t), s);
    }
    if (e != hipSuccess) return e;
    if (emit) {
        hipLaunchKernelGGL(rlr::sort_emit_kernel, dim3(1), dim3(1024), 0, s, c->d_packed, st, d_out_q, p.k, d_meta_q, p.unordered);
        if ((e = hipGetLastError()) != hipSuccess) return e;
    }
    if (timed && (e = hipEventRecord(c->ev[3], s)) != hipSuccess) return e;
    return hipSuccess;
}

hipError_t enqueue_query(rlr_index *ix, Ctx *c, uint32_t qi, const SearchPlan &p, uint64_t *d_out_q, uint64_t *d_meta_q,
                         bool timed, bool emit = true, const PoolArgs *pool = nullptr, bool *pool_done = nullptr)
{
    const hipError_t e = enqueue_query_scan(ix, c, qi, timed);
    return e != hipSuccess ? e : enqueue_query_rest(ix, c, qi, p, d_out_q, d_meta_q, timed, emit, pool, pool_done);
}

int32_t big_query(rlr_index *ix, Ctx *c, uint32_t qi, const SearchPlan &p, uint32_t n_cand, bool rescan,
                  uint64_t *d_out_q)
{
    hipStream_t s = c->stream;
    const uint32_t n = static_cast<uint32_t>(ix->n_rows);
    const uint32_t cap = next_pow2(std::max<uint32_t>(n_cand, p.k));
    SearchPlan big = p;
    big.cap = cap;
    if (c->cand_cap < cap) {
        if (c->d_cand) (void)hipFree(c->d_cand);
        if (c->d_packed) (void)hipFree(c->d_packed);
        c->d_cand = nullptr;
        c->d_packed = nullptr;
        c->cand_cap = 0;
        RLR_HIP(rlr::dev_malloc(reinterpret_cast<void **>(&c->d_cand), static_cast<size_t>(cap) * sizeof(uint32_t)));
        RLR_HIP(rlr::dev_malloc(reinterpret_cast<void **>(&c->d_packed), static_cast<size_t>(cap) * sizeof(uint64_t)));
        c->cand_cap = cap;
    }
    SelectState *st = c->d_state + qi;
    const float *dq = c->d_query + static_cast<size_t>(qi) * ix->q_pitch;
    if (rescan) {
        ScanArgs sa;
        sa.rows = ix->d_rows;
        sa.query = dq;
        sa.scores = c->d_scores;
        sa.hist = nullptr;
        sa.n_rows = n;
        sa.dim = ix->dim;
        sa.pitch16 = ix->pitch16;
        sa.dtype = ix->dtype;
        sa.n_cu = ix->n_cu;
        sa.variant = ix->scan_variant;
        RLR_HIP(launch_scan(sa, s));
    }
    SelectState h;
    RLR_HIP(hipMemcpyAsync(&h, st, sizeof(h), hipMemcpyDeviceToHost, s));
    RLR_HIP(hipStreamSynchronize(s));
    h.n_cand = 0;
    h.cap = cap;
    RLR_HIP(hipMemcpyAsync(st, &h, sizeof(h), hipMemcpyHostToDevice, s));
    RLR_HIP(launch_collect(c->d_scores, n, st, c->d_cand, ix->n_cu, s));
    static const bool old_finish = getenv("RLR_BIG_QUERY_SORT") != nullptr;
    hipError_t e = hipSuccess;
    const bool second_level = !old_finish && p.k <= kLdsSortCap;
    const bool staged = second_level && launch_rescore_staged(ix->d_rows, ix->pitch16, ix->dim, ix->dtype, dq, c->d_cand, st,
                                                              c->d_packed, cap, nullptr, s, &e);
    RLR_HIP(e);
    if (!staged)
        RLR_HIP(launch_rescore(ix->d_rows, ix->pitch16, ix->dim, ix->dtype, dq, c->d_cand, st, c->d_packed, cap, s));
    if (second_level) {
        hipLaunchKernelGGL(rlr::topk_global_kernel, dim3(1), dim3(1024), 0, s, c->d_packed, st, cap, d_out_q, p.k);
    } else {
        RLR_HIP(launch_sort_desc(c->d_packed, cap, s));
        hipLaunchKernelGGL(rlr::emit_kernel, dim3((p.k + 255) / 256), dim3(256), 0, s, c->d_packed, n_cand, d_out_q, p.k);
    }
    RLR_HIP(hipGetLastError());
    RLR_HIP(hipStreamSynchronize(s));
    return RLR_OK;
}

constexpr uint32_t kBatchMaxQueries = 1024;

bool env_is_one(const char *name)
{
    const char *v = getenv(name);
    return v && v[0] == '1';
}

bool batch_multi_shape(const rlr_index *ix, uint32_t nq, bool coalesced = false)
{
    if (coalesced && ix->dtype == RLR_F16)
        return nq <= 8 && ix->pitch16 % 32 == 0 && ix->pitch16 / 32 <= 4 && ix->pitch16 * 8 == ix->dim;
    return nq <= 8 && ix->dtype == RLR_F32 && ix->pitch16 % 64 == 0 && ix->pitch16 / 64 <= 4 && ix->pitch16 * 4 == ix->dim;
}

bool batch_eligible(const rlr_index *ix, uint32_t nq, uint32_t k, bool f16_ok = true, bool coalesced = false)
{
    if (nq < 2 || ix->dim % 128 != 0 || ix->n_rows < 4096 || k * 8 > batch_finish_capacity())
        return false;
    if (!f16_ok && !(batch_multi_shape(ix, nq, coalesced) && !(ix->image_enabled && ix->d_image) && !env_is_one("RLR_NO_MULTI_SCAN")))
        return false;
    if (ix->batch_min > 0)
        return nq >= ix->batch_min;
    const double row_bytes = static_cast<double>(ix->n_rows) * ix->dim * (ix->dtype == RLR_F16 ? 2.0 : 4.0);
    const double scan_bytes = static_cast<double>(ix->n_rows) * ix->dim *
                              (scan_over_q8(ix) ? 1.0 : (scan_over_image(ix, nullptr) || ix->dtype == RLR_F16) ? 2.0 : 4.0);
    const double t_single = 60e-6 + scan_bytes / 6.2e12;
    const bool image = ix->image_enabled && ix->d_image;
    const double pass = image ? static_cast<double>(ix->n_rows) * ix->dim * 2.0 / (nq <= 128 ? 5.0e12 : 3.0e12)
                              : row_bytes / 3.7e12;
    const bool multi = batch_multi_shape(ix, nq, coalesced) && !image;
    if (multi)
        return nq * t_single > 0.3e-3 + row_bytes / 5.5e12 + nq * (static_cast<double>(ix->n_rows) * 12.0 / 3.0e12);
    const double t_batch = 0.8e-3 + pass * ((nq + 255) / 256);
    return nq * t_single > t_batch;
}

int32_t run_batched(rlr_index *ix, Ctx *c, uint32_t q0, uint32_t nq, const SearchPlan &p, uint64_t *d_out,
                    std::vector<uint32_t> &h_status, uint64_t *h_res_out, bool coalesced = false)
{
    hipStream_t s = c->stream;
    const uint32_t n = static_cast<uint32_t>(ix->n_rows);
    const uint32_t fin_cap = batch_finish_capacity();
    const uint32_t n_qblocks = (nq + 255) / 256;
    const bool use_multi = batch_multi_shape(ix, nq, coalesced) && !(ix->image_enabled && ix->d_image) && !env_is_one("RLR_NO_MULTI_SCAN");
    const float eps_nom = use_multi ? 0.5f * p.two_eps : nomination_eps(ix->dim, ix->dtype, p.scale, p.norm_sum);
    const float two_eps = 2.0f * eps_nom;
    static const uint32_t rank_div = [] {
        const char *v = getenv("RLR_BATCH_RANK_DIV");
        const long d = v ? strtol(v, nullptr, 10) : 4;
        return static_cast<uint32_t>(d >= 1 && d <= 64 ? d : 4);
    }();
    uint32_t rank = std::max<uint32_t>(std::min<uint32_t>(p.k, 16), p.k / rank_div);
    uint64_t S = (static_cast<uint64_t>(rank) * n * 5 / 2 + fin_cap - 1) / fin_cap;
    S = std::max<uint64_t>(S, std::min<uint64_t>(n, 65536));
// ... 489 lines not shown
            const auto left = deadline - std::chrono::steady_clock::now();
            ix->co_cv.wait_until(lk, std::chrono::system_clock::now() +
                                         std::chrono::duration_cast<std::chrono::system_clock::duration>(left));
        } else
            ix->co_cv.wait(lk);
    }
    g->sealed = true;
    ix->co_pending.erase(std::find(ix->co_pending.begin(), ix->co_pending.end(), g));
    int32_t st;
    if (g->members.size() == 1) {
        ix->co_stats.n_solo += 1;
        lk.unlock();
        st = search_topk_host(ix, query, 1, k, guard_eps, rows_out, cos_out, n_out);
        lk.lock();
        g->status = st;
    } else {
        lk.unlock();
        coalesce_run(ix, g.get(), guard_eps);
        lk.lock();
        st = g->status;
    }
    g->done = true;
    coalesce_retire(ix);
    return st;
}

bool coalesce_hands_back(rlr_index *ix, uint32_t k)
{
    if (ix->co_max.load(std::memory_order_relaxed) < 2 || !coalesce_eligible(ix, k))
        return false;
    std::lock_guard<std::mutex> lk(ix->co_mu);
    ix->co_stats.n_engine_handbacks += 1;
    return true;
}

}

extern "C" {

int32_t rlr_version(void)
{
    return RLR_VERSION;
}

int32_t rlr_device_count(void)
{
    int n = 0;
    if (hipGetDeviceCount(&n) != hipSuccess)
        return 0;
    return n;
}

const char *rlr_last_error(void)
{
    return g_err;
}

float rlr_default_guard_eps(uint32_t dim)
{
    return (static_cast<float>(dim) + 64.0f) * 5.9604645e-8f * 1.0625f;
}

int32_t rlr_index_create(uint32_t dim, int32_t dtype, int32_t device_id, rlr_index **out)
{
    if (!out)
        return fail(RLR_E_INVALID, "out is null");
    *out = nullptr;
    if (dim == 0 || dim > kMaxDim)
        return fail(RLR_E_INVALID, "dim must be in [1, %u]", kMaxDim);
    if (dtype != RLR_F32 && dtype != RLR_F16)
        return fail(RLR_E_INVALID, "unknown dtype %d", dtype);
    int n_dev = rlr_device_count();
    if (n_dev <= 0)
        return fail(RLR_E_NO_DEVICE, "no HIP device is visible (this library has no CPU path)");
    if (device_id < 0 || device_id >= n_dev)
        return fail(RLR_E_NO_DEVICE, "device %d out of range (%d visible)", device_id, n_dev);
    rlr_index *ix = new (std::nothrow) rlr_index();
    if (!ix)
        return fail(RLR_E_OOM, "host allocation failed");
    ix->dim = dim;
    ix->dtype = dtype;
    ix->device = device_id;
    const uint32_t elem = dtype == RLR_F16 ? 2 : 4;
    ix->pitch16 = (dim * elem + 15) / 16;
    ix->q_pitch = ix->pitch16 * (16 / elem);
    hipDeviceProp_t prop;
    if (hipSetDevice(device_id) != hipSuccess || hipGetDeviceProperties(&prop, device_id) != hipSuccess) {
        delete ix;
        return fail(RLR_E_HIP, "cannot query device %d", device_id);
    }
    ix->n_cu = prop.multiProcessorCount > 0 ? prop.multiProcessorCount : 256;
    if (const char *v = getenv("RLR_SCAN_VARIANT"))
        ix->scan_variant = static_cast<int>(strtol(v, nullptr, 0));
    if (const char *v = getenv("RLR_TAIL"))
        ix->fused_tail = v[0] != '0' ? 1 : 0;
    if (const char *v = getenv("RLR_TAIL_DIRECT_MAX"))
        ix->tail_direct_max = static_cast<uint32_t>(std::min<unsigned long>(strtoul(v, nullptr, 0), 4096));
    if (const char *v = getenv("RLR_HYBRID_FETCH"))
        ix->hybrid_fetch_full = !strcmp(v, "full");
    if (const char *v = getenv("RLR_BATCH_MIN"))
        ix->batch_min = static_cast<uint32_t>(strtoul(v, nullptr, 0));
    if (const char *v = getenv("RLR_MAX_CONTEXTS"))
        ix->ctx_cap = static_cast<int>(std::min<long>(std::max<long>(strtol(v, nullptr, 0), 1), 64));
    *out = ix;
    return RLR_OK;
}

int32_t rlr_index_destroy(rlr_index *ix)
{
    if (!ix)
        return RLR_OK;
    (void)hipSetDevice(ix->device);
    (void)hipDeviceSynchronize();
    for (Ctx *c : ix->free_ctx)
        ctx_free(c);
    rows_free(&ix->rows_block);
    ix->d_rows = nullptr;
    if (ix->d_q8) (void)hipFree(ix->d_q8);
    if (ix->d_q8_scale) (void)hipFree(ix->d_q8_scale);
    if (ix->d_q8_stats) (void)hipFree(ix->d_q8_stats);
    if (ix->d_image)
        (void)hipFree(ix->d_image);
    delete ix;
    return RLR_OK;
}

int32_t rlr_index_info(const rlr_index *ix, uint64_t *n_rows, uint32_t *dim, int32_t *dtype, int32_t *device_id)
{
    RLR_TRY(check_handle(ix));
    if (n_rows) *n_rows = ix->n_rows;
    if (dim) *dim = ix->dim;
    if (dtype) *dtype = ix->dtype;
    if (device_id) *device_id = ix->device;
    return RLR_OK;
}

int32_t rlr_index_reserve(rlr_index *ix, uint64_t n_rows)
{
    RLR_TRY(check_handle(ix));
    RLR_TRY(use_device(ix));
    return ensure_rows(ix, n_rows);
}

int32_t rlr_index_upload(rlr_index *ix, const float *rows, uint64_t n_rows, int32_t normalize_on_device)
{
    RLR_TRY(check_handle(ix));
    if (n_rows && !rows)
        return fail(RLR_E_INVALID, "rows is null");
    RLR_TRY(use_device(ix));
    ix->n_rows = 0;
    ix->max_row_sumsq = 1.0f;
    ix->f16_overflow = false;
    RLR_TRY(ensure_rows(ix, n_rows));
    RLR_TRY(ingest(ix, rows, n_rows, 0, normalize_on_device));
    ix->n_rows = n_rows;
    return sync_image(ix, 0);
}

int32_t rlr_index_append(rlr_index *ix, const float *rows, uint64_t n_rows, int32_t normalize_on_device,
                         uint64_t *first_row_out)
{
    RLR_TRY(check_handle(ix));
    if (n_rows && !rows)
        return fail(RLR_E_INVALID, "rows is null");
    RLR_TRY(use_device(ix));
    const uint64_t first = ix->n_rows;
    RLR_TRY(ensure_rows(ix, first + n_rows));
    RLR_TRY(ingest(ix, rows, n_rows, first, normalize_on_device));
    ix->n_rows = first + n_rows;
    if (first_row_out)
        *first_row_out = first;
    return sync_image(ix, first);
}

int32_t rlr_index_delete_rows(rlr_index *ix, const uint64_t *rows, uint64_t n)
{
    RLR_TRY(check_handle(ix));
    if (n == 0)
        return RLR_OK;
    if (!rows)
        return fail(RLR_E_INVALID, "rows is null");
    RLR_TRY(use_device(ix));
    const uint64_t N = ix->n_rows;
    std::vector<uint8_t> dead(N, 0);
    for (uint64_t i = 0; i < n; ++i) {
        if (rows[i] >= N)
            return fail(RLR_E_RANGE, "row %llu out of range (index holds %llu rows)",
                        static_cast<unsigned long long>(rows[i]), static_cast<unsigned long long>(N));
        dead[rows[i]] = 1;
    }
    uint64_t first_dead = 0;
    while (first_dead < N && !dead[first_dead])
        ++first_dead;
    std::vector<uint32_t> keep;
    keep.reserve(N - first_dead);
    for (uint64_t r = first_dead; r < N; ++r)
        if (!dead[r])
            keep.push_back(static_cast<uint32_t>(r));
    const uint64_t chunk = std::max<uint64_t>(1, (256ull << 20) / row_bytes(ix));
    void *d_bounce = nullptr;
    uint32_t *d_keep = nullptr;
    const uint64_t cr = std::min<uint64_t>(chunk, std::max<size_t>(keep.size(), 1));
    RLR_HIP(rlr::dev_malloc(&d_bounce, cr * row_bytes(ix)));
    hipError_t e = rlr::dev_malloc(reinterpret_cast<void **>(&d_keep), cr * sizeof(uint32_t));
    if (e != hipSuccess) {
        (void)hipFree(d_bounce);
        return fail(RLR_E_OOM, "compaction buffer allocation failed");
    }
    int32_t st = RLR_OK;
    for (uint64_t i0 = 0; i0 < keep.size() && st == RLR_OK; i0 += cr) {
        const uint64_t m = std::min<uint64_t>(cr, keep.size() - i0);
        e = hipMemcpy(d_keep, keep.data() + i0, m * sizeof(uint32_t), hipMemcpyHostToDevice);
        if (e == hipSuccess)
            e = launch_compact_rows(ix->d_rows, d_bounce, ix->pitch16, d_keep, static_cast<uint32_t>(m), nullptr);
        if (e == hipSuccess)
            e = hipMemcpyAsync(static_cast<char *>(ix->d_rows) + (first_dead + i0) * row_bytes(ix), d_bounce,
                               m * row_bytes(ix), hipMemcpyDeviceToDevice, nullptr);
        if (e == hipSuccess)
            e = hipStreamSynchronize(nullptr);
        if (e != hipSuccess)
            st = fail(RLR_E_HIP, "row compaction failed: %s", hipGetErrorString(e));
    }
    (void)hipFree(d_bounce);
    (void)hipFree(d_keep);
    if (st == RLR_OK) {
        ix->n_rows = first_dead + keep.size();
        st = sync_image(ix, first_dead);
    }
    return st;
}

int32_t rlr_index_enable_batch_image(rlr_index *ix, int32_t enable)
{
    RLR_TRY(check_handle(ix));
    RLR_TRY(use_device(ix));
// ... 1291 lines not shown
```

rust-local-rag_amd/csrc/kernels.h:

```cpp
#pragma once

#include <hip/hip_runtime.h>
#include <stdint.h>

namespace rlr {

hipError_t dev_malloc(void **p, size_t bytes);
bool poison_mode();

int32_t set_error(int32_t code, const char *fmt, ...);

struct ScanArgs {
    const void *rows;
    const float *query;
    float *scores;
    uint32_t *hist;
    uint32_t n_rows;
    uint32_t dim;
    uint32_t pitch16;
    int dtype;
    int n_cu;
    int variant;
    const float *query_host = nullptr;
};
hipError_t launch_scan(const ScanArgs &a, hipStream_t stream);
bool launch_scan_takes_host_query(const ScanArgs &a);
bool launch_scan_multi(const ScanArgs &a, uint32_t q_pitch, uint32_t n_queries, size_t score_stride, hipStream_t s,
                       hipError_t *err);
bool launch_scan_multi_f16(const ScanArgs &a, uint32_t q_pitch, uint32_t n_queries, size_t score_stride, hipStream_t s,
                           hipError_t *err);

hipError_t launch_probe_read(const void *p, size_t bytes, float *sink, int n_cu, int shape, hipStream_t s);

struct SelectState {
    uint32_t k;
    uint32_t bin1;
    uint32_t k2;
    uint32_t bin2;
    uint32_t key_lo;
    uint32_t n_cand;
    uint32_t cap;
    uint32_t pad;
    uint32_t n_work;
    uint32_t done;
    uint32_t flags;
    uint32_t mode;
};
hipError_t launch_collect(const float *scores, uint32_t n, SelectState *st, uint32_t *cand,
                          int n_cu, hipStream_t s);
hipError_t launch_hist2_find1(const float *scores, uint32_t n, const uint32_t *hist1, uint32_t *hist2,
                              SelectState *st, uint32_t k, uint32_t cap, int n_cu, hipStream_t s);
hipError_t launch_collect_find2(const float *scores, uint32_t n, const uint32_t *hist2, SelectState *st,
                                float two_eps, uint32_t *cand, int n_cu, hipStream_t s);
hipError_t launch_sort_desc(uint64_t *packed, uint32_t n_pad, hipStream_t s);

hipError_t launch_batch_select(const float *scores, uint32_t n, size_t score_stride, uint32_t q_count,
                               uint32_t *hist, SelectState *st, float two_eps, float *tau_out, uint64_t *cand,
                               uint32_t cand_stride, int n_cu, hipStream_t s);

struct PoolArgs {
    uint32_t fetch, need, n_rows;
    float w_e, w_l;
    uint32_t *list;
    float *comb;
    float *cosv;
    uint32_t *info;
};
struct TailArgs {
    const float *scores;
    uint32_t n;
    uint32_t *hist;
    SelectState *st;
    uint32_t k, cap;
    float two_eps;
    const void *rows;
    uint32_t pitch16, dim;
    int dtype;
    const float *query;
    uint64_t *packed;
    uint64_t *out;
    uint64_t *meta;
    bool unordered;
    uint32_t direct_max;
    int n_cu;
    const PoolArgs *pool = nullptr;
};
bool tail_fits(uint32_t pitch16, uint32_t dim, int dtype);
hipError_t launch_tail_stage1(const TailArgs &a, hipStream_t s);
hipError_t launch_tail_stage2(const TailArgs &a, hipStream_t s);

float nomination_eps(uint32_t dim, int dtype, float prod = 1.0f, float norm_sum = 2.0f);
uint32_t batch_finish_capacity();
hipError_t launch_prep_queries(const float *q, uint32_t n_queries, uint32_t q_pitch, uint32_t dim, int dtype,
                               void *qfrag, hipStream_t s);
hipError_t launch_gemm_nominate(const void *rows, uint32_t pitch16, uint32_t dim, int dtype, uint32_t row_begin,
                                uint32_t row_end, const void *qfrag, uint32_t n_queries, const float *tau,
                                uint64_t *cand, uint32_t cand_stride, SelectState *st, float *scores,
                                size_t score_stride, const void *image, hipStream_t s, uint32_t *sync_ws = nullptr);
size_t image_bytes(uint32_t dim, uint64_t n_rows);
bool gemm_image_usable(uint32_t dim);
hipError_t launch_scan_image(const void *image, uint32_t n_rows, uint32_t dim, const float *query, float *scores,
                             uint32_t *hist, int n_cu, hipStream_t s);
hipError_t launch_build_image(const void *rows, uint32_t pitch16, uint32_t dim, int dtype, uint32_t n_rows,
                              uint32_t tile_begin, uint32_t tile_end, void *image, hipStream_t s);
hipError_t launch_batch_finish(const void *rows, uint32_t pitch16, uint32_t dim, int dtype, const float *queries,
                               uint32_t q_pitch, uint32_t n_queries, uint64_t *cand, uint32_t cand_stride,
// ... 53 lines not shown
```

rust-local-rag_amd/csrc/q8.hip:

```cpp
#include "common.h"
#include "kernels.h"
#include "../../include/rlr_gpu.h"

#include <algorithm>
#include <cstdlib>

namespace rlr {

namespace {

typedef unsigned int u32x4 __attribute__((ext_vector_type(4)));

__device__ inline float wave_max_abs(float v)
{
#pragma unroll
    for (int off = 32; off > 0; off >>= 1)
        v = fmaxf(v, __shfl_xor(v, off));
    return v;
}

__device__ inline float wave_add_all(float v)
{
#pragma unroll
    for (int off = 32; off > 0; off >>= 1)
        v += __shfl_xor(v, off);
    return v;
}

template <bool F16>
__global__ __launch_bounds__(256) void q8_build_kernel(const void *__restrict__ rows, uint32_t pitch_bytes, uint32_t dim,
                                                       uint32_t row_begin, uint32_t n_rows, uint8_t *__restrict__ q8,
                                                       float *__restrict__ scale, uint32_t *__restrict__ stats)
{
    const int lane = threadIdx.x & 63;
    const uint32_t row = row_begin + blockIdx.x * 4 + (threadIdx.x >> 6);
    if (row >= n_rows)
        return;
    const unsigned char *rowp = static_cast<const unsigned char *>(rows) + static_cast<size_t>(row) * pitch_bytes;
    auto elem = [&](uint32_t e) -> float {
        if constexpr (F16)
            return h2f(reinterpret_cast<const uint16_t *>(rowp)[e]);
        else
            return reinterpret_cast<const float *>(rowp)[e];
    };
    float m = 0.0f;
    bool has_nan = false, has_inf = false;
    for (uint32_t e = lane; e < dim; e += 64) {
        const float v = elem(e);
        has_nan |= v != v;
        has_inf |= __builtin_fabsf(v) > 3.4028234e38f;
        m = fmaxf(m, __builtin_fabsf(v));
    }
    has_nan = __ballot(has_nan) != 0;
    has_inf = __ballot(has_inf) != 0;
    const bool bad = has_nan || has_inf;
    m = wave_max_abs(m);
    const float s = (bad || m == 0.0f) ? 1.0f : m / 127.0f;
    float err2 = 0.0f;
    uint8_t *out = q8 + static_cast<size_t>(row) * dim;
    for (uint32_t e = lane; e < dim; e += 64) {
        const float v = bad ? 0.0f : elem(e);
        float k = __builtin_rintf(v / s);
        k = fminf(fmaxf(k, -127.0f), 127.0f);
        const float d = v - s * k;
        err2 += d * d;
        out[e] = static_cast<uint8_t>(static_cast<int>(k) + 128);
    }
    err2 = wave_add_all(err2);
    if (lane == 0) {
        scale[row] = bad ? __builtin_bit_cast(float, 0x7FC00000u) : s;
        if (has_inf && !has_nan)
            atomicOr(&stats[2], 1u);
        const float delta = __builtin_sqrtf(err2) * 1.001f + 1e-30f;
        if (!bad) {
            atomicMax(&stats[0], __builtin_bit_cast(uint32_t, delta));
            atomicMax(&stats[1], __builtin_bit_cast(uint32_t, s));
        }
    }
}

template <int B>
__device__ inline float ubyte_f32(uint32_t w)
{
    return static_cast<float>((w >> (8 * B)) & 0xFFu);
}

__device__ inline float dot16_u8(u32x4 x, const float (&q)[16], float acc)
{
    acc = __builtin_fmaf(ubyte_f32<0>(x[0]), q[0], acc);
    acc = __builtin_fmaf(ubyte_f32<1>(x[0]), q[1], acc);
    acc = __builtin_fmaf(ubyte_f32<2>(x[0]), q[2], acc);
    acc = __builtin_fmaf(ubyte_f32<3>(x[0]), q[3], acc);
    acc = __builtin_fmaf(ubyte_f32<0>(x[1]), q[4], acc);
    acc = __builtin_fmaf(ubyte_f32<1>(x[1]), q[5], acc);
    acc = __builtin_fmaf(ubyte_f32<2>(x[1]), q[6], acc);
    acc = __builtin_fmaf(ubyte_f32<3>(x[1]), q[7], acc);
    acc = __builtin_fmaf(ubyte_f32<0>(x[2]), q[8], acc);
    acc = __builtin_fmaf(ubyte_f32<1>(x[2]), q[9], acc);
    acc = __builtin_fmaf(ubyte_f32<2>(x[2]), q[10], acc);
    acc = __builtin_fmaf(ubyte_f32<3>(x[2]), q[11], acc);
    acc = __builtin_fmaf(ubyte_f32<0>(x[3]), q[12], acc);
    acc = __builtin_fmaf(ubyte_f32<1>(x[3]), q[13], acc);
    acc = __builtin_fmaf(ubyte_f32<2>(x[3]), q[14], acc);
    acc = __builtin_fmaf(ubyte_f32<3>(x[3]), q[15], acc);
    return acc;
}

template <int R, int L>
__global__ __launch_bounds__(256) void q8_scan_kernel(const uint8_t *__restrict__ q8, const float *__restrict__ scale,
                                                      const float *__restrict__ query, float *__restrict__ scores,
                                                      uint32_t *__restrict__ g_hist, uint32_t n_rows, uint32_t dim,
                                                      uint32_t group_rows)
{
    __shared__ uint32_t s_hist[kHistBins];
    const int tid = threadIdx.x;
    const int lane = tid & 63;
    const int wave = __builtin_amdgcn_readfirstlane(tid >> 6);
    for (int i = tid; i < kHistBins; i += 256)
        s_hist[i] = 0;
    const uint32_t p16 = dim / 16;
    bool active[L];
    float qv[L][16];
    float qs = 0.0f;
#pragma unroll
    for (int l = 0; l < L; ++l) {
        active[l] = static_cast<uint32_t>(lane + 64 * l) < p16;
// ... 217 lines not shown
```

rust-local-rag_amd/csrc/scan.hip:

```cpp
#include <algorithm>
#include <cstring>

#include "common.h"
#include "kernels.h"
#include "../../include/rlr_gpu.h"

namespace rlr {

namespace {

typedef float f32x4 __attribute__((ext_vector_type(4)));

template <bool NT>
__device__ inline float4 ld16(const float4 *p)
{
    if constexpr (NT) {
        const f32x4 v = __builtin_nontemporal_load(reinterpret_cast<const f32x4 *>(p));
        return make_float4(v.x, v.y, v.z, v.w);
    } else {
        return *p;
    }
}

__device__ inline float dot4(float4 x, float4 q, float acc)
{
    acc = __builtin_fmaf(x.x, q.x, acc);
    acc = __builtin_fmaf(x.y, q.y, acc);
    acc = __builtin_fmaf(x.z, q.z, acc);
    acc = __builtin_fmaf(x.w, q.w, acc);
    return acc;
}

__device__ inline float dot8h(float4 raw, float4 q0, float4 q1, float acc)
{
    uint32_t w0 = __builtin_bit_cast(uint32_t, raw.x), w1 = __builtin_bit_cast(uint32_t, raw.y);
    uint32_t w2 = __builtin_bit_cast(uint32_t, raw.z), w3 = __builtin_bit_cast(uint32_t, raw.w);
    acc = __builtin_fmaf(h2f(static_cast<uint16_t>(w0 & 0xFFFF)), q0.x, acc);
    acc = __builtin_fmaf(h2f(static_cast<uint16_t>(w0 >> 16)), q0.y, acc);
    acc = __builtin_fmaf(h2f(static_cast<uint16_t>(w1 & 0xFFFF)), q0.z, acc);
    acc = __builtin_fmaf(h2f(static_cast<uint16_t>(w1 >> 16)), q0.w, acc);
    acc = __builtin_fmaf(h2f(static_cast<uint16_t>(w2 & 0xFFFF)), q1.x, acc);
    acc = __builtin_fmaf(h2f(static_cast<uint16_t>(w2 >> 16)), q1.y, acc);
    acc = __builtin_fmaf(h2f(static_cast<uint16_t>(w3 & 0xFFFF)), q1.z, acc);
    acc = __builtin_fmaf(h2f(static_cast<uint16_t>(w3 >> 16)), q1.w, acc);
    return acc;
}

__device__ inline void hist_flush(const uint32_t *s_hist, uint32_t *g_hist)
{
    for (int i = threadIdx.x; i < kHistBins; i += blockDim.x) {
        uint32_t c = s_hist[i];
        if (c)
            atomicAdd(&g_hist[i], c);
    }
}

template <int CH>
struct QueryArg {
    float4 v[CH * 64];
};

template <int CH, int R, bool F16, bool NT, bool KQ = false>
__global__ __launch_bounds__(256) void scan_fixed_kernel(const float4 *__restrict__ rows,
                                                         const float *__restrict__ query,
                                                         float *__restrict__ scores,
                                                         uint32_t *__restrict__ g_hist,
                                                         uint32_t n_rows, uint32_t group_rows,
                                                         QueryArg<KQ ? CH : 0> qarg = QueryArg<KQ ? CH : 0>())
{
    constexpr int P16 = CH * 64;
    constexpr int QF4 = F16 ? 2 * P16 : P16;
    __shared__ float4 s_q[QF4];
    __shared__ uint32_t s_hist[kHistBins];

    const int tid = threadIdx.x;
    const int lane = tid & 63;
    const int wave = __builtin_amdgcn_readfirstlane(tid >> 6);
    if constexpr (KQ) {
        for (int i = tid; i < QF4; i += 256) {
            const float4 v = qarg.v[i];
            s_q[i] = v;
            if (blockIdx.x == 0)
                reinterpret_cast<float4 *>(const_cast<float *>(query))[i] = v;
        }
    } else {
        for (int i = tid; i < QF4; i += 256)
            s_q[i] = reinterpret_cast<const float4 *>(query)[i];
    }
    for (int i = tid; i < kHistBins; i += 256)
        s_hist[i] = 0;
    __syncthreads();

    float4 qv[F16 ? 2 * CH : CH];
#pragma unroll
    for (int c = 0; c < CH; ++c) {
        if constexpr (F16) {
            qv[2 * c] = s_q[2 * (c * 64 + lane)];
            qv[2 * c + 1] = s_q[2 * (c * 64 + lane) + 1];
        } else {
            qv[c] = s_q[c * 64 + lane];
        }
    }

    const uint32_t n_groups = (n_rows + group_rows - 1) / group_rows;
    const uint32_t n_waves = gridDim.x * 4;
    for (uint32_t g = blockIdx.x * 4 + wave; g < n_groups; g += n_waves) {
        const uint32_t row0 = g * group_rows;
        const uint32_t nr = min(group_rows, n_rows - row0);
        float mine = 0.0f;
        for (uint32_t r = 0; r < nr; r += R) {
            float4 x[R][CH];
#pragma unroll
            for (int rr = 0; rr < R; ++rr) {
                const uint32_t row = min(row0 + r + rr, row0 + nr - 1);
                const float4 *p = rows + static_cast<size_t>(row) * P16 + lane;
#pragma unroll
                for (int c = 0; c < CH; ++c)
                    x[rr][c] = ld16<NT>(p + c * 64);
            }
#pragma unroll
            for (int rr = 0; rr < R; ++rr) {
                float acc = 0.0f;
#pragma unroll
                for (int c = 0; c < CH; ++c) {
                    if constexpr (F16)
                        acc = dot8h(x[rr][c], qv[2 * c], qv[2 * c + 1], acc);
                    else
                        acc = dot4(x[rr][c], qv[c], acc);
                }
                const float tot = wave_sum(acc);
                if (static_cast<uint32_t>(lane) == r + rr)
                    mine = tot;
            }
        }
        if (static_cast<uint32_t>(lane) < nr) {
            scores[row0 + lane] = mine;
            if (g_hist)
                atomicAdd(&s_hist[score_key(mine) >> 21], 1u);
        }
    }
    if (g_hist) {
        __syncthreads();
        hist_flush(s_hist, g_hist);
    }
}

template <int CH, int Q>
__global__ __launch_bounds__(256) void scan_multi_kernel(const float4 *__restrict__ rows, const float *__restrict__ queries,
                                                         uint32_t q_pitch, uint32_t n_queries, float *__restrict__ scores,
                                                         size_t score_stride, uint32_t n_rows, uint32_t group_rows)
{
    constexpr int P16 = CH * 64;
    constexpr int R = 2;
    const int tid = threadIdx.x;
    const int lane = tid & 63;
    const int wave = __builtin_amdgcn_readfirstlane(tid >> 6);
    float4 qv[Q][CH];
#pragma unroll
    for (int q = 0; q < Q; ++q)
#pragma unroll
        for (int c = 0; c < CH; ++c)
            qv[q][c] = static_cast<uint32_t>(q) < n_queries
                           ? reinterpret_cast<const float4 *>(queries + static_cast<size_t>(q) * q_pitch)[c * 64 + lane]
                           : make_float4(0.0f, 0.0f, 0.0f, 0.0f);

    const uint32_t n_groups = (n_rows + group_rows - 1) / group_rows;
    const uint32_t n_waves = gridDim.x * 4;
    for (uint32_t g = blockIdx.x * 4 + wave; g < n_groups; g += n_waves) {
        const uint32_t row0 = g * group_rows;
        const uint32_t nr = min(group_rows, n_rows - row0);
        float mine[Q];
#pragma unroll
        for (int q = 0; q < Q; ++q)
            mine[q] = 0.0f;
        for (uint32_t r = 0; r < nr; r += R) {
            float4 x[R][CH];
#pragma unroll
            for (int rr = 0; rr < R; ++rr) {
                const uint32_t row = min(row0 + r + rr, row0 + nr - 1);
                const float4 *p = rows + static_cast<size_t>(row) * P16 + lane;
#pragma unroll
                for (int c = 0; c < CH; ++c)
                    x[rr][c] = ld16<true>(p + c * 64);
            }
#pragma unroll
            for (int rr = 0; rr < R; ++rr) {
#pragma unroll
                for (int q = 0; q < Q; ++q) {
                    float acc = 0.0f;
#pragma unroll
                    for (int c = 0; c < CH; ++c)
                        acc = dot4(x[rr][c], qv[q][c], acc);
                    const float tot = wave_sum(acc);
                    if (static_cast<uint32_t>(lane) == r + rr)
                        mine[q] = tot;
                }
            }
        }
        if (static_cast<uint32_t>(lane) < nr) {
#pragma unroll
            for (int q = 0; q < Q; ++q)
                if (static_cast<uint32_t>(q) < n_queries)
                    scores[static_cast<size_t>(q) * score_stride + row0 + lane] = mine[q];
        }
    }
}

typedef float f32x2 __attribute__((ext_vector_type(2)));

__device__ inline f32x2 h2f_lo(uint32_t w)
{
    return f32x2{h2f(static_cast<uint16_t>(w & 0xFFFF)), h2f(static_cast<uint16_t>(w >> 16))};
}

template <int C, int Q>
__global__ __launch_bounds__(256) void scan_multi_h_kernel(const uint2 *__restrict__ rows, const float *__restrict__ queries,
                                                           uint32_t q_pitch, uint32_t n_queries, float *__restrict__ scores,
                                                           size_t score_stride, uint32_t n_rows, uint32_t group_rows)
{
    constexpr int P8 = C * 64;
    constexpr int R = 2;
    const int tid = threadIdx.x;
    const int lane = tid & 63;
    const int wave = __builtin_amdgcn_readfirstlane(tid >> 6);
    f32x2 qv[Q][C][2];
#pragma unroll
    for (int q = 0; q < Q; ++q)
#pragma unroll
        for (int c = 0; c < C; ++c) {
            float4 v = make_float4(0.0f, 0.0f, 0.0f, 0.0f);
            if (static_cast<uint32_t>(q) < n_queries)
                v = reinterpret_cast<const float4 *>(queries + static_cast<size_t>(q) * q_pitch)[c * 64 + lane];
            qv[q][c][0] = f32x2{v.x, v.y};
            qv[q][c][1] = f32x2{v.z, v.w};
        }

    const uint32_t n_groups = (n_rows + group_rows - 1) / group_rows;
    const uint32_t n_waves = gridDim.x * 4;
    for (uint32_t g = blockIdx.x * 4 + wave; g < n_groups; g += n_waves) {
        const uint32_t row0 = g * group_rows;
        const uint32_t nr = min(group_rows, n_rows - row0);
        float mine[Q];
#pragma unroll
        for (int q = 0; q < Q; ++q)
            mine[q] = 0.0f;
        for (uint32_t r = 0; r < nr; r += R) {
            uint2 x[R][C];
#pragma unroll
            for (int rr = 0; rr < R; ++rr) {
                const uint32_t row = min(row0 + r + rr, row0 + nr - 1);
                const uint2 *p = rows + static_cast<size_t>(row) * P8 + lane;
#pragma unroll
                for (int c = 0; c < C; ++c) {
                    typedef unsigned int u32x2 __attribute__((ext_vector_type(2)));
                    const u32x2 v = __builtin_nontemporal_load(reinterpret_cast<const u32x2 *>(p + c * 64));
                    x[rr][c] = make_uint2(v.x, v.y);
                }
            }
#pragma unroll
            for (int rr = 0; rr < R; ++rr) {
                f32x2 xf[C][2];
#pragma unroll
                for (int c = 0; c < C; ++c) {
                    xf[c][0] = h2f_lo(x[rr][c].x);
                    xf[c][1] = h2f_lo(x[rr][c].y);
                }
#pragma unroll
                for (int q = 0; q < Q; ++q) {
                    f32x2 acc = f32x2{0.0f, 0.0f};
#pragma unroll
                    for (int c = 0; c < C; ++c) {
                        acc = __builtin_elementwise_fma(xf[c][0], qv[q][c][0], acc);
                        acc = __builtin_elementwise_fma(xf[c][1], qv[q][c][1], acc);
                    }
                    const float tot = wave_sum(acc.x + acc.y);
                    if (static_cast<uint32_t>(lane) == r + rr)
                        mine[q] = tot;
                }
            }
        }
        if (static_cast<uint32_t>(lane) < nr) {
#pragma unroll
            for (int q = 0; q < Q; ++q)
                if (static_cast<uint32_t>(q) < n_queries)
                    scores[static_cast<size_t>(q) * score_stride + row0 + lane] = mine[q];
        }
    }
}

constexpr int pack_gcd(int a, int b) { return b == 0 ? a : pack_gcd(b, a % b); }

template <int P16>
struct PackShape {
    static constexpr int G = 64 / pack_gcd(P16, 64);
    static constexpr int M = G * P16 / 64;
    static constexpr int R = M >= 9 ? 1 : (M >= 5 ? 2 : (M >= 2 ? 4 : 8));
};

template <int P16, bool F16>
__global__ __launch_bounds__(256) void scan_packed_kernel(const float4 *__restrict__ rows,
                                                          const float *__restrict__ query,
                                                          float *__restrict__ scores,
                                                          uint32_t *__restrict__ g_hist,
                                                          uint32_t n_rows, uint32_t group_rows)
{
    constexpr int G = PackShape<P16>::G, M = PackShape<P16>::M, R = PackShape<P16>::R;
    constexpr int QF4 = F16 ? 2 * P16 : P16;
    __shared__ float4 s_q[QF4];
    __shared__ uint32_t s_hist[kHistBins];

    const int tid = threadIdx.x;
    const int lane = tid & 63;
    const int wave = __builtin_amdgcn_readfirstlane(tid >> 6);
    for (int i = tid; i < QF4; i += 256)
        s_q[i] = reinterpret_cast<const float4 *>(query)[i];
    for (int i = tid; i < kHistBins; i += 256)
        s_hist[i] = 0;
    __syncthreads();

    float4 qv[F16 ? 2 * M : M];
#pragma unroll
    for (int j = 0; j < M; ++j) {
        const int col = (j * 64 + lane) % P16;
        if constexpr (F16) {
            qv[2 * j] = s_q[2 * col];
            qv[2 * j + 1] = s_q[2 * col + 1];
        } else {
            qv[j] = s_q[col];
        }
    }

    const size_t last_unit = static_cast<size_t>(n_rows) * P16 - 1;
    const uint32_t n_groups = (n_rows + group_rows - 1) / group_rows;
    const uint32_t n_waves = gridDim.x * 4;
    for (uint32_t g = blockIdx.x * 4 + wave; g < n_groups; g += n_waves) {
        const uint32_t row0 = g * group_rows;
        const uint32_t nr = min(group_rows, n_rows - row0);
        float mine = 0.0f;
        for (uint32_t r = 0; r < nr; r += R * G) {
            float4 x[R][M];
#pragma unroll
            for (int rr = 0; rr < R; ++rr) {
                const uint32_t pack_row = min(row0 + r + rr * G, row0 + ((nr - 1) / G) * G);
                const size_t base = static_cast<size_t>(pack_row) * P16 + lane;
#pragma unroll
                for (int j = 0; j < M; ++j)
                    x[rr][j] = ld16<true>(rows + min(base + j * 64, last_unit));
            }
#pragma unroll
            for (int rr = 0; rr < R; ++rr) {
                float acc[G];
#pragma unroll
                for (int k = 0; k < G; ++k)
                    acc[k] = 0.0f;
#pragma unroll
                for (int j = 0; j < M; ++j) {
                    const int g_lo = (j * 64) / P16, g_hi = (j * 64 + 63) / P16;
                    if (g_lo == g_hi) {
                        if constexpr (F16)
                            acc[g_lo] = dot8h(x[rr][j], qv[2 * j], qv[2 * j + 1], acc[g_lo]);
                        else
                            acc[g_lo] = dot4(x[rr][j], qv[j], acc[g_lo]);
                    } else {
                        float t;
                        if constexpr (F16)
                            t = dot8h(x[rr][j], qv[2 * j], qv[2 * j + 1], 0.0f);
                        else
                            t = dot4(x[rr][j], qv[j], 0.0f);
                        const int lane_row = (j * 64 + lane) / P16;
#pragma unroll
                        for (int k = 0; k < G; ++k)
                            if (k >= g_lo && k <= g_hi)
                                acc[k] += lane_row == k ? t : 0.0f;
                    }
                }
#pragma unroll
                for (int k = 0; k < G; ++k) {
                    const float tot = wave_sum(acc[k]);
                    if (static_cast<uint32_t>(lane) == r + rr * G + k)
                        mine = tot;
                }
            }
        }
        if (static_cast<uint32_t>(lane) < nr) {
            scores[row0 + lane] = mine;
            if (g_hist)
                atomicAdd(&s_hist[score_key(mine) >> 21], 1u);
        }
    }
    if (g_hist) {
        __syncthreads();
        hist_flush(s_hist, g_hist);
    }
}

template <int R, bool F16>
__global__ __launch_bounds__(256) void scan_generic_kernel(const float4 *__restrict__ rows,
                                                           const float *__restrict__ query,
                                                           float *__restrict__ scores,
                                                           uint32_t *__restrict__ g_hist,
                                                           uint32_t n_rows, uint32_t group_rows,
                                                           uint32_t pitch16)
{
    extern __shared__ __attribute__((aligned(16))) unsigned char s_raw[];
    uint32_t *s_hist = reinterpret_cast<uint32_t *>(s_raw);
    float4 *s_q = reinterpret_cast<float4 *>(s_raw + kHistBins * sizeof(uint32_t));

    const int tid = threadIdx.x;
    const int lane = tid & 63;
    const int wave = __builtin_amdgcn_readfirstlane(tid >> 6);
    const uint32_t qf4 = F16 ? 2 * pitch16 : pitch16;
    for (uint32_t i = tid; i < qf4; i += 256)
        s_q[i] = reinterpret_cast<const float4 *>(query)[i];
    for (int i = tid; i < kHistBins; i += 256)
        s_hist[i] = 0;
    __syncthreads();

    const uint32_t n_groups = (n_rows + group_rows - 1) / group_rows;
    const uint32_t n_waves = gridDim.x * 4;
    for (uint32_t g = blockIdx.x * 4 + wave; g < n_groups; g += n_waves) {
        const uint32_t row0 = g * group_rows;
        const uint32_t nr = min(group_rows, n_rows - row0);
        float mine = 0.0f;
        for (uint32_t r = 0; r < nr; r += R) {
            float acc[R];
            const float4 *p[R];
#pragma unroll
            for (int rr = 0; rr < R; ++rr) {
                acc[rr] = 0.0f;
                const uint32_t row = min(row0 + r + rr, row0 + nr - 1);
                p[rr] = rows + static_cast<size_t>(row) * pitch16;
            }
            for (uint32_t c = lane; c < pitch16; c += 64) {
                float4 x[R];
#pragma unroll
                for (int rr = 0; rr < R; ++rr)
                    x[rr] = ld16<true>(p[rr] + c);
                if constexpr (F16) {
                    const float4 q0 = s_q[2 * c], q1 = s_q[2 * c + 1];
#pragma unroll
                    for (int rr = 0; rr < R; ++rr)
                        acc[rr] = dot8h(x[rr], q0, q1, acc[rr]);
                } else {
                    const float4 q0 = s_q[c];
#pragma unroll
                    for (int rr = 0; rr < R; ++rr)
                        acc[rr] = dot4(x[rr], q0, acc[rr]);
                }
            }
#pragma unroll
            for (int rr = 0; rr < R; ++rr) {
                const float tot = wave_sum(acc[rr]);
                if (static_cast<uint32_t>(lane) == r + rr)
                    mine = tot;
            }
        }
        if (static_cast<uint32_t>(lane) < nr) {
            scores[row0 + lane] = mine;
            if (g_hist)
                atomicAdd(&s_hist[score_key(mine) >> 21], 1u);
        }
    }
    if (g_hist) {
        __syncthreads();
        hist_flush(s_hist, g_hist);
    }
}

struct ScanPlan {
    uint32_t group_rows;
    uint32_t blocks;
    int r;
    bool nt;
};

ScanPlan plan_scan(const ScanArgs &a)
{
    ScanPlan p;
    const int v = a.variant;
    const int r_code = v & 0xF;
    const bool small = (a.n_rows + 15) / 16 < static_cast<uint32_t>(a.n_cu) * 4 * 4 * 3;
    p.r = r_code == 0 ? (small ? 4 : 8) : r_code;
    p.nt = ((v >> 4) & 1) == 0;
    int blocks_per_cu = (v >> 8) & 0xFF;
    if (blocks_per_cu == 0)
        blocks_per_cu = small ? 8 : 4;
    uint32_t group = (v >> 16) & 0xFF;
    const uint32_t max_blocks = static_cast<uint32_t>(a.n_cu) * blocks_per_cu;
    if (group == 0) {
        group = 64;
        while (group > 16 && (a.n_rows + group - 1) / group < max_blocks * 4 * 4)
            group >>= 1;
        if (a.dtype == RLR_F32 && a.pitch16 == 192)
            group = 16;
    }
    if (group > 64)
        group = 64;
    group = (group / p.r) * p.r;
    if (group == 0)
        group = p.r;
    if (r_code == 0 && ((v >> 8) & 0xFF) == 0 && ((v >> 16) & 0xFF) == 0) {
        const uint32_t elems = a.dtype == RLR_F16 ? a.pitch16 * 8 : a.pitch16 * 4;
        if (elems == a.dim && a.dtype == RLR_F32 && a.pitch16 == 192) {
            p.r = 4;
            blocks_per_cu = 1;
            group = 8;
        } else if (elems == a.dim && a.dtype == RLR_F32 && a.pitch16 == 384) {
            blocks_per_cu = 1;
            group = 8;
        } else if (elems == a.dim && a.dtype == RLR_F16 && a.pitch16 == 192) {
            blocks_per_cu = 1;
            group = 16;
        }
    }
    p.group_rows = group;
    const uint32_t n_groups = (a.n_rows + group - 1) / group;
    uint32_t blocks = (n_groups + 3) / 4;
    if (blocks > static_cast<uint32_t>(a.n_cu) * blocks_per_cu)
        blocks = static_cast<uint32_t>(a.n_cu) * blocks_per_cu;
    if (blocks == 0)
        blocks = 1;
    p.blocks = blocks;
    return p;
}

bool kq_enabled()
{
    static const bool on = [] {
        const char *v = getenv("RLR_SCAN_KQ");
        return !(v && v[0] == '0');
    }();
    return on;
}

template <int CH>
hipError_t launch_fixed_kq(const ScanArgs &a, const ScanPlan &p, hipStream_t s)
{
    const float4 *rows = static_cast<const float4 *>(a.rows);
    QueryArg<CH> q;
    std::memcpy(q.v, a.query_host, sizeof(q.v));
#define RLR_SCAN_KQ_CASE(RV)                                                                                  \
    hipLaunchKernelGGL((scan_fixed_kernel<CH, RV, false, true, true>), dim3(p.blocks), dim3(256), 0, s, rows, \
                       a.query, a.scores, a.hist, a.n_rows, p.group_rows, q)
    switch (p.r) {
    case 1: RLR_SCAN_KQ_CASE(1); break;
    case 2: RLR_SCAN_KQ_CASE(2); break;
    case 8: RLR_SCAN_KQ_CASE(8); break;
    default: RLR_SCAN_KQ_CASE(4); break;
    }
#undef RLR_SCAN_KQ_CASE
    return hipGetLastError();
}

template <int CH, bool F16>
hipError_t launch_fixed(const ScanArgs &a, const ScanPlan &p, hipStream_t s)
{
    if constexpr (!F16 && CH <= 3) {
        if (a.query_host && p.nt && kq_enabled())
            return launch_fixed_kq<CH>(a, p, s);
    }
    const float4 *rows = static_cast<const float4 *>(a.rows);
#define RLR_SCAN_CASE(RV, NTV)                                                                    \
    hipLaunchKernelGGL((scan_fixed_kernel<CH, RV, F16, NTV>), dim3(p.blocks), dim3(256), 0, s,   \
                       rows, a.query, a.scores, a.hist, a.n_rows, p.group_rows)
    if (p.nt) {
        switch (p.r) {
        case 1: RLR_SCAN_CASE(1, true); break;
        case 2: RLR_SCAN_CASE(2, true); break;
        case 8: RLR_SCAN_CASE(8, true); break;
        default: RLR_SCAN_CASE(4, true); break;
        }
    } else {
        switch (p.r) {
        case 1: RLR_SCAN_CASE(1, false); break;
        case 2: RLR_SCAN_CASE(2, false); break;
        case 8: RLR_SCAN_CASE(8, false); break;
        default: RLR_SCAN_CASE(4, false); break;
        }
    }
#undef RLR_SCAN_CASE
    return hipGetLastError();
}

bool fixed_shape(const ScanArgs &a, int *ch)
{
    if (a.pitch16 % 64 != 0)
        return false;
    const int c = a.pitch16 / 64;
    const uint32_t elems = a.dtype == RLR_F16 ? a.pitch16 * 8 : a.pitch16 * 4;
    if (elems != a.dim)
        return false;
    if (a.dtype == RLR_F16) {
        if (c < 1 || c > 4)
            return false;
    } else if (c < 1 || c > 8 || c == 7) {
        return false;
    }
    *ch = c;
    return true;
}

template <int CH, bool F16>
hipError_t launch_fixed_wide(const ScanArgs &a, ScanPlan p, hipStream_t s)
{
    p.r = 2;
    p.group_rows = std::max<uint32_t>((p.group_rows / 2) * 2, 2);
    p.blocks = std::max<uint32_t>(1, std::min<uint32_t>(p.blocks, ((a.n_rows + p.group_rows - 1) / p.group_rows + 3) / 4));
    hipLaunchKernelGGL((scan_fixed_kernel<CH, 2, F16, true>), dim3(p.blocks), dim3(256), 0, s,
                       static_cast<const float4 *>(a.rows), a.query, a.scores, a.hist, a.n_rows, p.group_rows);
    return hipGetLastError();
}

template <int P16, bool F16>
hipError_t launch_packed_one(const ScanArgs &a, ScanPlan p, hipStream_t s)
{
    constexpr uint32_t step = PackShape<P16>::R * PackShape<P16>::G;
    uint32_t group = std::max<uint32_t>(p.group_rows, step);
    group = std::min<uint32_t>(64, (group / step) * step);
    const uint32_t n_groups = (a.n_rows + group - 1) / group;
    const uint32_t blocks = std::max<uint32_t>(1, std::min<uint32_t>((n_groups + 3) / 4, static_cast<uint32_t>(a.n_cu) * 8));
    hipLaunchKernelGGL((scan_packed_kernel<P16, F16>), dim3(blocks), dim3(256), 0, s, static_cast<const float4 *>(a.rows),
                       a.query, a.scores, a.hist, a.n_rows, group);
    return hipGetLastError();
}

bool launch_packed(const ScanArgs &a, const ScanPlan &p, hipStream_t s, hipError_t *e)
{
    const uint32_t elems = a.dtype == RLR_F16 ? a.pitch16 * 8 : a.pitch16 * 4;
    if (elems != a.dim || (a.variant & 0x20))
        return false;
    const bool h = a.dtype == RLR_F16;
    switch (a.pitch16) {
    case 16: *e = h ? launch_packed_one<16, true>(a, p, s) : launch_packed_one<16, false>(a, p, s); return true;
    case 32: *e = h ? launch_packed_one<32, true>(a, p, s) : launch_packed_one<32, false>(a, p, s); return true;
    default: return false;
    }
}

}

bool launch_scan_takes_host_query(const ScanArgs &a)
{
    int ch = 0;
    if (!a.query_host || a.n_rows == 0 || a.dtype != RLR_F32 || !fixed_shape(a, &ch) || ch > 3 || !kq_enabled())
        return false;
    return plan_scan(a).nt;
}

hipError_t launch_scan(const ScanArgs &a, hipStream_t s)
{
    if (a.n_rows == 0)
        return hipSuccess;
    ScanPlan p = plan_scan(a);
    int ch = 0;
    if (fixed_shape(a, &ch)) {
        if (a.dtype == RLR_F16) {
            if (p.r == 8) {
                p.r = 4;
                p.group_rows = (p.group_rows / 4) * 4;
            }
            switch (ch) {
            case 1: return launch_fixed<1, true>(a, p, s);
            case 2: return launch_fixed<2, true>(a, p, s);
            case 3: return launch_fixed_wide<3, true>(a, p, s);
            default: return launch_fixed_wide<4, true>(a, p, s);
            }
        }
        switch (ch) {
        case 1: return launch_fixed<1, false>(a, p, s);
        case 2: return launch_fixed<2, false>(a, p, s);
        case 3: return launch_fixed<3, false>(a, p, s);
        case 4: return launch_fixed<4, false>(a, p, s);
        case 5: return launch_fixed_wide<5, false>(a, p, s);
        case 6: return launch_fixed_wide<6, false>(a, p, s);
        default: return launch_fixed_wide<8, false>(a, p, s);
        }
    }
    hipError_t pe = hipSuccess;
    if (launch_packed(a, p, s, &pe))
        return pe;
    const uint32_t qf4 = a.dtype == RLR_F16 ? 2 * a.pitch16 : a.pitch16;
    const size_t lds = kHistBins * sizeof(uint32_t) + static_cast<size_t>(qf4) * 16;
    const float4 *rows = static_cast<const float4 *>(a.rows);
    p.r = 2;
    p.group_rows = (p.group_rows / 2) * 2;
    if (p.group_rows == 0)
        p.group_rows = 2;
    if (a.dtype == RLR_F16)
        hipLaunchKernelGGL((scan_generic_kernel<2, true>), dim3(p.blocks), dim3(256), lds, s, rows,
                           a.query, a.scores, a.hist, a.n_rows, p.group_rows, a.pitch16);
    else
        hipLaunchKernelGGL((scan_generic_kernel<2, false>), dim3(p.blocks), dim3(256), lds, s, rows,
                           a.query, a.scores, a.hist, a.n_rows, p.group_rows, a.pitch16);
    return hipGetLastError();
}

template <int U>
__global__ __launch_bounds__(256) void probe_read_kernel(const float4 *__restrict__ p, size_t n_kib, float *__restrict__ sink)
{
    const int lane = threadIdx.x & 63;
    const size_t wave = static_cast<size_t>(blockIdx.x) * 4 + (threadIdx.x >> 6);
    const size_t n_waves = static_cast<size_t>(gridDim.x) * 4;
    float acc = 0.0f;
    for (size_t b = wave * U; b < n_kib; b += n_waves * U) {
        float4 x[U];
#pragma unroll
        for (int u = 0; u < U; ++u)
            x[u] = ld16<true>(p + min(b + u, n_kib - 1) * 64 + lane);
#pragma unroll
        for (int u = 0; u < U; ++u)
            acc += (x[u].x + x[u].y) + (x[u].z + x[u].w);
    }
    sink[wave * 64 + lane] = acc;
}

hipError_t launch_probe_read(const void *p, size_t bytes, float *sink, int n_cu, int shape, hipStream_t s)
{
    const size_t n_kib = bytes / 1024;
    if (n_kib == 0)
        return hipSuccess;
    const float4 *p4 = static_cast<const float4 *>(p);
    if (shape == 0)
        hipLaunchKernelGGL(probe_read_kernel<12>, dim3(n_cu), dim3(256), 0, s, p4, n_kib, sink);
    else if (shape == 1)
        hipLaunchKernelGGL(probe_read_kernel<8>, dim3(n_cu * 4), dim3(256), 0, s, p4, n_kib, sink);
    else
        hipLaunchKernelGGL(probe_read_kernel<4>, dim3(n_cu * 8), dim3(256), 0, s, p4, n_kib, sink);
    return hipGetLastError();
}

bool launch_scan_multi_f16(const ScanArgs &a, uint32_t q_pitch, uint32_t n_queries, size_t score_stride, hipStream_t s,
                           hipError_t *err)
{
    if (a.dtype != RLR_F16 || n_queries < 2 || n_queries > 8 || a.pitch16 % 32 != 0 || a.pitch16 / 32 < 1 ||
        a.pitch16 / 32 > 4 || a.pitch16 * 8 != a.dim || q_pitch < a.dim)
        return false;
    const uint32_t group = 32;
    const uint32_t n_groups = (a.n_rows + group - 1) / group;
    const uint32_t wgs = n_queries > 4 && a.pitch16 / 32 >= 3 ? 2u : 4u;
    const uint32_t blocks = std::max<uint32_t>(1, std::min<uint32_t>((n_groups + 3) / 4, static_cast<uint32_t>(a.n_cu) * wgs));
    const uint2 *rows = static_cast<const uint2 *>(a.rows);
#define RLR_MULTI_H(CV, QV)                                                                                      \
    hipLaunchKernelGGL((scan_multi_h_kernel<CV, QV>), dim3(blocks), dim3(256), 0, s, rows, a.query, q_pitch,     \
                       n_queries, a.scores, score_stride, a.n_rows, group)
#define RLR_MULTI_H_Q(CV)                                 \
    do {                                                  \
        if (n_queries <= 2) RLR_MULTI_H(CV, 2);           \
        else if (n_queries <= 4) RLR_MULTI_H(CV, 4);      \
        else RLR_MULTI_H(CV, 8);                          \
    } while (0)
    switch (a.pitch16 / 32) {
    case 1: RLR_MULTI_H_Q(1); break;
    case 2: RLR_MULTI_H_Q(2); break;
    case 3: RLR_MULTI_H_Q(3); break;
    default: RLR_MULTI_H_Q(4); break;
    }
#undef RLR_MULTI_H_Q
#undef RLR_MULTI_H
    *err = hipGetLastError();
    return true;
}

bool launch_scan_multi(const ScanArgs &a, uint32_t q_pitch, uint32_t n_queries, size_t score_stride, hipStream_t s,
                       hipError_t *err)
{
    int ch = 0;
    if (a.dtype != RLR_F32 || n_queries < 2 || n_queries > 8 || !fixed_shape(a, &ch) || ch > 4)
        return false;
    static const int tune = [] {
        const char *v = getenv("RLR_SCAN_MULTI_VARIANT");
        return v ? static_cast<int>(strtol(v, nullptr, 0)) : 0;
    }();
    const uint32_t group = ((tune >> 8) & 0xFF) ? static_cast<uint32_t>((tune >> 8) & 0xFE) : 32u;
    const uint32_t wgs = (tune & 0xFF) ? static_cast<uint32_t>(tune & 0xFF) : 4u;
    const uint32_t n_groups = (a.n_rows + group - 1) / group;
    const uint32_t blocks = std::max<uint32_t>(1, std::min<uint32_t>((n_groups + 3) / 4, static_cast<uint32_t>(a.n_cu) * wgs));
// ... 24 lines not shown
```

rust-local-rag_amd/csrc/staged_dot.h:

```cpp
#pragma once

#include "common.h"

namespace rlr {

__device__ inline float chain_sum_lds(const float4 *__restrict__ p4, const float *__restrict__ p, uint32_t dim)
{
    float s = 0.0f;
    const uint32_t units = dim / 4;
    uint32_t u = 0;
    float4 a[4], b[4];
    if (units >= 4) {
#pragma unroll
        for (int i = 0; i < 4; ++i)
            a[i] = p4[i];
    }
    for (; u + 8 <= units; u += 8) {
#pragma unroll
        for (int i = 0; i < 4; ++i)
            b[i] = p4[u + 4 + i];
#pragma unroll
        for (int i = 0; i < 4; ++i) {
            s = s + a[i].x; s = s + a[i].y; s = s + a[i].z; s = s + a[i].w;
        }
        if (u + 12 <= units) {
#pragma unroll
            for (int i = 0; i < 4; ++i)
                a[i] = p4[u + 8 + i];
        }
#pragma unroll
        for (int i = 0; i < 4; ++i) {
            s = s + b[i].x; s = s + b[i].y; s = s + b[i].z; s = s + b[i].w;
        }
    }
    if (u + 4 <= units) {
#pragma unroll
        for (int i = 0; i < 4; ++i) {
            s = s + a[i].x; s = s + a[i].y; s = s + a[i].z; s = s + a[i].w;
        }
        u += 4;
    }
    for (uint32_t e = u * 4; e < dim; ++e)
        s = s + p[e];
    return s;
}

template <bool F16, int NT = 256>
__device__ __forceinline__ float staged_reference_dot(const float4 *__restrict__ rows, uint32_t pitch16, uint32_t dim,
                                                      const float *s_q, float *s_p, const uint32_t *s_cand, uint32_t cnt,
                                                      uint32_t tid)
{
    const uint32_t q_floats = (dim + 7) & ~7u;
    const uint32_t p_pitch = q_floats + 4;
    const uint32_t units = F16 ? q_floats / 8 : q_floats / 4;
    const uint32_t total = cnt * units;
    constexpr int kBatch = 6;
    for (uint32_t idx0 = tid; idx0 < total; idx0 += NT * kBatch) {
        float4 x[kBatch];
        uint32_t ci[kBatch], uu[kBatch];
#pragma unroll
        for (int j = 0; j < kBatch; ++j) {
            const uint32_t idx = idx0 + NT * j;
            ci[j] = idx / units;
            uu[j] = idx - ci[j] * units;
            if (idx < total)
                x[j] = rows[static_cast<size_t>(s_cand[ci[j]]) * pitch16 + uu[j]];
        }
#pragma unroll
        for (int j = 0; j < kBatch; ++j) {
            if (idx0 + NT * j >= total)
                continue;
            const uint32_t u = uu[j];
            float *dst = s_p + ci[j] * p_pitch;
            if constexpr (F16) {
                const uint32_t w[4] = {__builtin_bit_cast(uint32_t, x[j].x), __builtin_bit_cast(uint32_t, x[j].y),
                                       __builtin_bit_cast(uint32_t, x[j].z), __builtin_bit_cast(uint32_t, x[j].w)};
                const float *q = s_q + u * 8;
                float4 lo, hi;
                lo.x = h2f(static_cast<uint16_t>(w[0] & 0xFFFF)) * q[0];
                lo.y = h2f(static_cast<uint16_t>(w[0] >> 16)) * q[1];
                lo.z = h2f(static_cast<uint16_t>(w[1] & 0xFFFF)) * q[2];
                lo.w = h2f(static_cast<uint16_t>(w[1] >> 16)) * q[3];
                hi.x = h2f(static_cast<uint16_t>(w[2] & 0xFFFF)) * q[4];
                hi.y = h2f(static_cast<uint16_t>(w[2] >> 16)) * q[5];
                hi.z = h2f(static_cast<uint16_t>(w[3] & 0xFFFF)) * q[6];
                hi.w = h2f(static_cast<uint16_t>(w[3] >> 16)) * q[7];
                reinterpret_cast<float4 *>(dst)[2 * u] = lo;
                reinterpret_cast<float4 *>(dst)[2 * u + 1] = hi;
            } else {
                const float4 q = reinterpret_cast<const float4 *>(s_q)[u];
                float4 pr;
                pr.x = x[j].x * q.x;
                pr.y = x[j].y * q.y;
                pr.z = x[j].z * q.z;
                pr.w = x[j].w * q.w;
                reinterpret_cast<float4 *>(dst)[u] = pr;
            }
        }
    }
    __syncthreads();
    float sc = 0.0f;
    if (tid < cnt) {
        const float *pr = s_p + tid * p_pitch;
        sc = chain_sum_lds(reinterpret_cast<const float4 *>(pr), pr, dim);
    }
    return sc;
}

}
```

Baseline: 220.1.

## Store f32 rows as split hi/lo halves and scan only high halves

Result: faster. 404.2 (median of 6 runs) (+83.7%).

```diff
diff --git a/rust-local-rag_amd/build.py b/rust-local-rag_amd/build.py
--- a/rust-local-rag_amd/build.py
+++ b/rust-local-rag_amd/build.py
@@ -13,7 +13,7 @@
 
 SOURCES = ["scan.hip", "select.hip", "tail.hip", "exact.hip", "gemm.hip", "index.hip", "engine.cpp", "multi.cpp", "lexical.hip", "q8.hip",
            "jsonio.cpp", "text_batch.cpp"]
-HEADERS = ["common.h", "kernels.h", "exact_dot.h", "lds_select.h", "staged_dot.h", "select_dev.h", "sort_emit.h", "pool_prepare.h",
+HEADERS = ["common.h", "kernels.h", "row_layout.h", "exact_dot.h", "lds_select.h", "staged_dot.h", "select_dev.h", "sort_emit.h", "pool_prepare.h",
            "engine_host.h", "lexical_internal.h", os.path.join(ROOT, "include", "rlr_gpu.h"),
            os.path.join(ROOT, "include", "rlr_engine.h"), os.path.join(ROOT, "include", "rlr_lexical.h")]
 
diff --git a/rust-local-rag_amd/csrc/exact.hip b/rust-local-rag_amd/csrc/exact.hip
--- a/rust-local-rag_amd/csrc/exact.hip
+++ b/rust-local-rag_amd/csrc/exact.hip
@@ -2,6 +2,7 @@
 #include "exact_dot.h"
 #include "staged_dot.h"
 #include "sort_emit.h"
+#include "row_layout.h"
 #include "kernels.h"
 #include "../../include/rlr_gpu.h"
 
@@ -39,7 +40,7 @@
         return;
     }
     const uint32_t r = cand[i];
-    const float s = dot_ref_row<F16>(rows + static_cast<size_t>(r) * pitch16, s_q, dim);
+    const float s = dot_ref_row<F16>(rows + static_cast<size_t>(r) * pitch16, s_q, dim, pitch16);
     packed_out[i] = pack_result(s, r);
 }
 
@@ -123,7 +124,7 @@
     if (i >= n)
         return;
     const uint32_t r = list[i] < n_rows_clamp ? list[i] : 0u;
-    out[i] = dot_ref_row<F16>(rows + static_cast<size_t>(r) * pitch16, s_q, dim);
+    out[i] = dot_ref_row<F16>(rows + static_cast<size_t>(r) * pitch16, s_q, dim, pitch16);
 }
 
 template <bool F16>
@@ -144,7 +145,7 @@
         return;
     const size_t at = static_cast<size_t>(q) * stride + i;
     const uint32_t r = list[at] < n_rows_clamp ? list[at] : 0u;
-    out[at] = dot_ref_row<F16>(rows + static_cast<size_t>(r) * pitch16, s_q, dim);
+    out[at] = dot_ref_row<F16>(rows + static_cast<size_t>(r) * pitch16, s_q, dim, pitch16);
 }
 
 template <bool F16>
@@ -238,7 +239,7 @@
         if constexpr (F16)
             static_cast<_Float16 *>(rows_out)[i] = static_cast<_Float16>(v);
         else
-            static_cast<float *>(rows_out)[i] = v;
+            split_store(static_cast<char *>(rows_out) + static_cast<size_t>(r) * pitch16 * 16, pitch16, c, v);
     }
 }
 
@@ -303,7 +304,7 @@
         if constexpr (F16)
             static_cast<_Float16 *>(rows_out)[i] = static_cast<_Float16>(v);
         else
-            static_cast<float *>(rows_out)[i] = v;
+            split_store(static_cast<char *>(rows_out) + static_cast<size_t>(r) * pitch16 * 16, pitch16, c, v);
     }
 }
 
@@ -321,7 +322,7 @@
         if constexpr (F16)
             out[i] = h2f(static_cast<const uint16_t *>(rows)[r * pitch16 * 8 + c]);
         else
-            out[i] = static_cast<const float *>(rows)[r * pitch16 * 4 + c];
+            out[i] = split_load(static_cast<const char *>(rows) + r * pitch16 * 16, pitch16, c);
     }
 }
 
@@ -398,7 +399,7 @@
         return make_float4(h2f(static_cast<uint16_t>(h.x)), h2f(static_cast<uint16_t>(h.x >> 16)), h2f(static_cast<uint16_t>(h.y)),
                            h2f(static_cast<uint16_t>(h.y >> 16)));
     } else if constexpr (SRC == 1) {
-        return *reinterpret_cast<const float4 *>(static_cast<const float *>(rows) + static_cast<size_t>(row) * pitch16 * 4 + col);
+        return split_load4(static_cast<const char *>(rows) + static_cast<size_t>(row) * pitch16 * 16, pitch16, col);
     } else {
         return *reinterpret_cast<const float4 *>(pool + static_cast<size_t>(row) * dim + col);
     }
@@ -470,9 +471,14 @@
                     if (c4 * 4 + 1 < kc) v.y = h2f(src[1]);
                     if (c4 * 4 + 2 < kc) v.z = h2f(src[2]);
                     if (c4 * 4 + 3 < kc) v.w = h2f(src[3]);
+                } else if constexpr (SRC == 1) {
+                    const char *src = static_cast<const char *>(rows) + static_cast<size_t>(src_row[u]) * pitch16 * 16;
+                    v.x = split_load(src, pitch16, col);
+                    if (c4 * 4 + 1 < kc) v.y = split_load(src, pitch16, col + 1);
+                    if (c4 * 4 + 2 < kc) v.z = split_load(src, pitch16, col + 2);
+                    if (c4 * 4 + 3 < kc) v.w = split_load(src, pitch16, col + 3);
                 } else {
-                    const float *src = SRC == 0 ? pool + static_cast<size_t>(row) * dim + col
-                                                : static_cast<const float *>(rows) + static_cast<size_t>(src_row[u]) * pitch16 * 4 + col;
+                    const float *src = pool + static_cast<size_t>(row) * dim + col;
                     v.x = src[0];
                     if (c4 * 4 + 1 < kc) v.y = src[1];
                     if (c4 * 4 + 2 < kc) v.z = src[2];
diff --git a/rust-local-rag_amd/csrc/exact_dot.h b/rust-local-rag_amd/csrc/exact_dot.h
--- a/rust-local-rag_amd/csrc/exact_dot.h
+++ b/rust-local-rag_amd/csrc/exact_dot.h
@@ -1,11 +1,12 @@
 #pragma once
 
 #include "common.h"
+#include "row_layout.h"
 
 namespace rlr {
 
 template <bool F16>
-__device__ inline float dot_ref_row(const float4 *__restrict__ row, const float *s_q, uint32_t dim)
+__device__ inline float dot_ref_row(const float4 *__restrict__ row, const float *s_q, uint32_t dim, uint32_t pitch16)
 {
     float s = 0.0f;
     constexpr uint32_t EPU = F16 ? 8 : 4;
@@ -14,8 +15,12 @@
     for (; u + 4 <= full; u += 4) {
         float4 x[4];
 #pragma unroll
-        for (int i = 0; i < 4; ++i)
-            x[i] = row[u + i];
+        for (int i = 0; i < 4; ++i) {
+            if constexpr (F16)
+                x[i] = row[u + i];
+            else
+                x[i] = split_load4(row, pitch16, (u + i) * 4);
+        }
 #pragma unroll
         for (int i = 0; i < 4; ++i) {
             const float *q = s_q + (u + i) * EPU;
@@ -45,9 +50,8 @@
             s = s + p;
         }
     } else {
-        const float *f = reinterpret_cast<const float *>(row);
         for (uint32_t e = u * EPU; e < dim; ++e) {
-            float p = f[e] * s_q[e];
+            float p = split_load(row, pitch16, e) * s_q[e];
             s = s + p;
         }
     }
diff --git a/rust-local-rag_amd/csrc/gemm.hip b/rust-local-rag_amd/csrc/gemm.hip
--- a/rust-local-rag_amd/csrc/gemm.hip
+++ b/rust-local-rag_amd/csrc/gemm.hip
@@ -1,4 +1,5 @@
 #include "common.h"
+#include "row_layout.h"
 #include "exact_dot.h"
 #include "kernels.h"
 #include "lds_select.h"
@@ -24,8 +25,7 @@
 
 __global__ __launch_bounds__(256) void prep_queries_kernel(const float *__restrict__ q, uint32_t n_queries,
                                                            uint32_t q_pitch, uint32_t dim, uint32_t n_ksteps,
-                                                           uint32_t n_qblocks, int f16_rows,
-                                                           _Float16 *__restrict__ out)
+                                                           uint32_t n_qblocks, _Float16 *__restrict__ out)
 {
     const size_t total = static_cast<size_t>(n_qblocks) * n_ksteps * kNB * 64 * 8;
     for (size_t e = static_cast<size_t>(blockIdx.x) * 256 + threadIdx.x; e < total; e += static_cast<size_t>(gridDim.x) * 256) {
@@ -37,7 +37,7 @@
         const uint32_t qb = static_cast<uint32_t>(rest / n_ksteps);
         const uint32_t query = qb * kQB + nb * 16 + (lane & 15);
         const uint32_t g = lane >> 4;
-        const uint32_t k = ks * 32 + (f16_rows ? g * 8 + j : (j < 4 ? g * 4 + j : 16 + g * 4 + (j - 4)));
+        const uint32_t k = ks * 32 + g * 8 + j;
         float v = 0.0f;
         if (query < n_queries && k < dim)
             v = q[static_cast<size_t>(query) * q_pitch + k];
@@ -157,7 +157,7 @@
         const uint32_t r = min(row0 + rg * 16 + (lane & 15), last_row);
         ap[rg] = a.rows + static_cast<size_t>(r) * a.pitch_bytes + (lane >> 4) * 16;
     }
-    constexpr int kStepBytes = F16ROWS ? 64 : 128;
+    constexpr int kStepBytes = 64;
 
     const uint32_t n_chunks = a.n_ksteps / kKsChunk;
     const half8 *bsrc = a.qfrag + static_cast<size_t>(qb) * a.n_ksteps * kNB * 64;
@@ -189,12 +189,9 @@
 #pragma unroll
             for (int ks = 0; ks < kKsChunk; ++ks) {
                 const unsigned char *p = ap[rg] + static_cast<size_t>(c * kKsChunk + ks) * kStepBytes;
-                if constexpr (F16ROWS) {
-                    araw[rg][ks][0] = *reinterpret_cast<const float4 *>(p);
-                } else {
-                    araw[rg][ks][0] = *reinterpret_cast<const float4 *>(p);
-                    araw[rg][ks][1] = *reinterpret_cast<const float4 *>(p + 64);
-                }
+                araw[rg][ks][0] = *reinterpret_cast<const float4 *>(p);
+                if constexpr (!F16ROWS)
+                    araw[rg][ks][1] = *reinterpret_cast<const float4 *>(p + a.pitch_bytes / 2);
             }
     };
     auto convert_a = [&]() {
@@ -202,10 +199,13 @@
         for (int rg = 0; rg < kRG; ++rg)
 #pragma unroll
             for (int ks = 0; ks < kKsChunk; ++ks) {
-                if constexpr (F16ROWS)
+                if constexpr (F16ROWS) {
                     a_cur[rg][ks] = __builtin_bit_cast(half8, araw[rg][ks][0]);
-                else
-                    a_cur[rg][ks] = cvt8(araw[rg][ks][0], araw[rg][ks][1]);
+                } else {
+                    float4 lo, hi;
+                    split_decode8(__builtin_bit_cast(uint4, araw[rg][ks][0]), __builtin_bit_cast(uint4, araw[rg][ks][1]), &lo, &hi);
+                    a_cur[rg][ks] = cvt8(lo, hi);
+                }
             }
     };
 
@@ -271,8 +271,9 @@
             if constexpr (F16ROWS) {
                 v = *reinterpret_cast<const half8 *>(src + k * 2);
             } else {
-                const float4 lo = *reinterpret_cast<const float4 *>(src + k * 4);
-                const float4 hi = *reinterpret_cast<const float4 *>(src + k * 4 + 16);
+                float4 lo, hi;
+                split_decode8(*reinterpret_cast<const uint4 *>(src + k * 2),
+                              *reinterpret_cast<const uint4 *>(src + (pitch_bytes / 2) + k * 2), &lo, &hi);
                 v = cvt8(lo, hi);
             }
         }
@@ -880,7 +881,7 @@
     }
     for (uint32_t i = threadIdx.x; i < band; i += 256) {
         const uint32_t r = 0xFFFFFFFFu - static_cast<uint32_t>(s_c[i] & 0xFFFFFFFFu);
-        const float e = dot_ref_row<F16ROWS>(rows + static_cast<size_t>(r) * pitch16, s_q, dim);
+        const float e = dot_ref_row<F16ROWS>(rows + static_cast<size_t>(r) * pitch16, s_q, dim, pitch16);
         s_c[i] = pack_result(e, r);
     }
     uint32_t b_pad = 1;
@@ -1024,7 +1025,7 @@
     const size_t total = static_cast<size_t>(n_qblocks) * n_ksteps * kNB * 64 * 8;
     const uint32_t blocks = static_cast<uint32_t>(std::min<size_t>((total + 255) / 256, 4096));
     hipLaunchKernelGGL(prep_queries_kernel, dim3(blocks), dim3(256), 0, s, q, n_queries, q_pitch, dim, n_ksteps,
-                       n_qblocks, dtype == RLR_F16 ? 1 : 0, static_cast<_Float16 *>(qfrag));
+                       n_qblocks, static_cast<_Float16 *>(qfrag));
     return hipGetLastError();
 }
 
diff --git a/rust-local-rag_amd/csrc/index.hip b/rust-local-rag_amd/csrc/index.hip
--- a/rust-local-rag_amd/csrc/index.hip
+++ b/rust-local-rag_amd/csrc/index.hip
@@ -1,6 +1,7 @@
 #include "../../include/rlr_gpu.h"
 #include "common.h"
 #include "kernels.h"
+#include "row_layout.h"
 #include "lds_select.h"
 #include "sort_emit.h"
 #include "pool_prepare.h"
@@ -177,6 +178,7 @@
     uint32_t batch_min = 0;
     float max_row_sumsq = 1.0f;
     bool f16_overflow = false;
+    bool nonfinite_rows = false;
     bool image_enabled = false;
     bool image_scan = false;
     bool q8_enabled = false;
@@ -795,9 +797,14 @@
                                        ix->dtype, d_norm, nullptr);
         if (e == hipSuccess)
             e = hipStreamSynchronize(nullptr);
-        if (e == hipSuccess && !normalize) {
+        if (e == hipSuccess && (!normalize || ix->dtype == RLR_F32)) {
             h_norm.resize(m);
             e = hipMemcpy(h_norm.data(), d_norm, m * sizeof(float), hipMemcpyDeviceToHost);
+        }
+        for (uint64_t i = 0; i < m && e == hipSuccess && ix->dtype == RLR_F32 && !ix->nonfinite_rows; ++i)
+            if (!std::isfinite(h_norm[i]))
+                ix->nonfinite_rows = true;
+        if (e == hipSuccess && !normalize) {
             for (uint64_t i = 0; i < m && e == hipSuccess; ++i) {
                 if (h_norm[i] > ix->max_row_sumsq)
                     ix->max_row_sumsq = h_norm[i];
@@ -1597,6 +1604,16 @@
     return ix->q8_enabled && ix->d_q8 && !ix->q8_has_inf;
 }
 
+bool scan_over_hi(const rlr_index *ix)
+{
+    if (ix->dtype != RLR_F32 || ix->nonfinite_rows)
+        return false;
+    static const char *force = getenv("RLR_SCAN_HI");
+    if (force)
+        return force[0] != '0';
+    return ix->n_rows * row_bytes(ix) >= (1ull << 30);
+}
+
 bool scans_take_host_query(const rlr_index *ix, const Ctx *c, const float *h_q)
 {
     if (scan_over_q8(ix) || scan_over_image(ix, c) || ix->n_rows == 0)
@@ -1613,6 +1630,7 @@
     sa.n_cu = ix->n_cu;
     sa.variant = ix->scan_variant;
     sa.query_host = h_q;
+    sa.full_rows = !scan_over_hi(ix);
     return launch_scan_takes_host_query(sa);
 }
 
@@ -1622,6 +1640,16 @@
     const float scale = guard_eps > dflt ? guard_eps / dflt : 1.0f;
     const float qn = q_norm * 1.0001f + 1e-30f;
     return 2.0f * (ix->q8_delta * qn + q8_arith_eps(ix->dim, ix->q8_scale_max, qn) + dflt) * scale;
+}
+
+float split_hi_two_eps(const rlr_index *ix, float eps, const SearchPlan &p)
+{
+    const float dflt = rlr_default_guard_eps(ix->dim) * p.scale;
+    const float scale = eps > dflt ? eps / dflt : 1.0f;
+    const float trunc = 7.8125e-3f * 1.001f;
+    const float acc = 2.0f * (static_cast<float>(ix->dim) + 64.0f) * 5.9604645e-8f;
+    const float sub = 1.0e-38f * __builtin_sqrtf(static_cast<float>(ix->dim));
+    return 2.0f * ((trunc + acc) * p.scale + sub * p.norm_sum) * 1.0625f * scale;
 }
 
 float image_two_eps(const rlr_index *ix, float eps, const SearchPlan &p)
@@ -1674,6 +1702,7 @@
     sa.n_cu = ix->n_cu;
     sa.variant = ix->scan_variant;
     sa.query_host = c->h_q_kq ? c->h_q_kq + static_cast<size_t>(qi) * ix->q_pitch : nullptr;
+    sa.full_rows = !scan_over_hi(ix);
     static const bool variant_dyn = getenv("RLR_SCAN_VARIANT_DYN") != nullptr;
     if (variant_dyn)
         if (const char *v = getenv("RLR_SCAN_VARIANT"))
@@ -1705,7 +1734,7 @@
     const bool q8 = scan_over_q8(ix);
     const bool img = !q8 && scan_over_image(ix, c);
     const float band = q8 ? q8_two_eps(ix, qi < c->q_norm.size() ? c->q_norm[qi] : 1.0f, p.two_eps * 0.5f)
-                          : (img ? p.two_eps_img : p.two_eps);
+                          : img ? p.two_eps_img : scan_over_hi(ix) ? split_hi_two_eps(ix, p.two_eps * 0.5f, p) : p.two_eps;
     const bool fused = ix->fused_tail < 0 ? ix->n_rows <= 4000000ull : ix->fused_tail != 0;
     if (fused && p.cap <= kLdsSortCap && tail_fits(ix->pitch16, ix->dim, ix->dtype)) {
         TailArgs ta;
@@ -1796,6 +1825,7 @@
         sa.dtype = ix->dtype;
         sa.n_cu = ix->n_cu;
         sa.variant = ix->scan_variant;
+        sa.full_rows = scan_over_q8(ix) || scan_over_image(ix, c) || !scan_over_hi(ix);
         RLR_HIP(launch_scan(sa, s));
     }
     SelectState h;
@@ -2451,7 +2481,7 @@
     ix->dtype = dtype;
     ix->device = device_id;
     const uint32_t elem = dtype == RLR_F16 ? 2 : 4;
-    ix->pitch16 = (dim * elem + 15) / 16;
+    ix->pitch16 = dtype == RLR_F16 ? (dim * elem + 15) / 16 : split_pitch16(dim);
     ix->q_pitch = ix->pitch16 * (16 / elem);
     hipDeviceProp_t prop;
     if (hipSetDevice(device_id) != hipSuccess || hipGetDeviceProperties(&prop, device_id) != hipSuccess) {
@@ -2520,6 +2550,7 @@
     ix->n_rows = 0;
     ix->max_row_sumsq = 1.0f;
     ix->f16_overflow = false;
+    ix->nonfinite_rows = false;
     RLR_TRY(ensure_rows(ix, n_rows));
     RLR_TRY(ingest(ix, rows, n_rows, 0, normalize_on_device));
     ix->n_rows = n_rows;
diff --git a/rust-local-rag_amd/csrc/kernels.h b/rust-local-rag_amd/csrc/kernels.h
--- a/rust-local-rag_amd/csrc/kernels.h
+++ b/rust-local-rag_amd/csrc/kernels.h
@@ -22,6 +22,7 @@
     int n_cu;
     int variant;
     const float *query_host = nullptr;
+    bool full_rows = true;
 };
 hipError_t launch_scan(const ScanArgs &a, hipStream_t stream);
 bool launch_scan_takes_host_query(const ScanArgs &a);
diff --git a/rust-local-rag_amd/csrc/q8.hip b/rust-local-rag_amd/csrc/q8.hip
--- a/rust-local-rag_amd/csrc/q8.hip
+++ b/rust-local-rag_amd/csrc/q8.hip
@@ -1,4 +1,5 @@
 #include "common.h"
+#include "row_layout.h"
 #include "kernels.h"
 #include "../../include/rlr_gpu.h"
 
@@ -41,7 +42,7 @@
         if constexpr (F16)
             return h2f(reinterpret_cast<const uint16_t *>(rowp)[e]);
         else
-            return reinterpret_cast<const float *>(rowp)[e];
+            return split_load(rowp, pitch_bytes / 16, e);
     };
     float m = 0.0f;
     bool has_nan = false, has_inf = false;
diff --git a/rust-local-rag_amd/csrc/row_layout.h b/rust-local-rag_amd/csrc/row_layout.h
--- /dev/null
+++ b/rust-local-rag_amd/csrc/row_layout.h
@@ -0,0 +1,66 @@
+#pragma once
+
+#include <hip/hip_runtime.h>
+#include <stdint.h>
+
+namespace rlr {
+
+__host__ __device__ constexpr uint32_t split_half16(uint32_t dim) { return (dim + 7) / 8; }
+__host__ __device__ constexpr uint32_t split_pitch16(uint32_t dim) { return 2 * split_half16(dim); }
+
+__host__ __device__ inline uint16_t split_hi(float v) { return static_cast<uint16_t>(__builtin_bit_cast(uint32_t, v) >> 16); }
+__host__ __device__ inline uint16_t split_lo(float v) { return static_cast<uint16_t>(__builtin_bit_cast(uint32_t, v)); }
+__host__ __device__ inline float split_join(uint16_t hi, uint16_t lo)
+{
+    return __builtin_bit_cast(float, (static_cast<uint32_t>(hi) << 16) | lo);
+}
+__host__ __device__ inline float split_hi_value(uint16_t hi) { return __builtin_bit_cast(float, static_cast<uint32_t>(hi) << 16); }
+
+__host__ __device__ inline void split_store(void *row, uint32_t pitch16, uint32_t i, float v)
+{
+    uint16_t *h = static_cast<uint16_t *>(row);
+    h[i] = split_hi(v);
+    h[static_cast<size_t>(pitch16) * 4 + i] = split_lo(v);
+}
+
+__host__ __device__ inline float split_load(const void *row, uint32_t pitch16, uint32_t i)
+{
+    const uint16_t *h = static_cast<const uint16_t *>(row);
+    return split_join(h[i], h[static_cast<size_t>(pitch16) * 4 + i]);
+}
+
+__host__ __device__ inline float split_join_lo_word(uint32_t hw, uint32_t lw)
+{
+    return __builtin_bit_cast(float, (hw << 16) | (lw & 0xFFFFu));
+}
+__host__ __device__ inline float split_join_hi_word(uint32_t hw, uint32_t lw)
+{
+    return __builtin_bit_cast(float, (hw & 0xFFFF0000u) | (lw >> 16));
+}
+
+__device__ inline float4 split_load4(const void *row, uint32_t pitch16, uint32_t e0)
+{
+    const uint16_t *h = static_cast<const uint16_t *>(row);
+    const uint2 hi = *reinterpret_cast<const uint2 *>(h + e0);
+    const uint2 lo = *reinterpret_cast<const uint2 *>(h + static_cast<size_t>(pitch16) * 4 + e0);
+    return make_float4(split_join_lo_word(hi.x, lo.x), split_join_hi_word(hi.x, lo.x), split_join_lo_word(hi.y, lo.y),
+                       split_join_hi_word(hi.y, lo.y));
+}
+
+__device__ inline void split_decode8(uint4 hi, uint4 lo, float4 *a, float4 *b)
+{
+    *a = make_float4(split_join_lo_word(hi.x, lo.x), split_join_hi_word(hi.x, lo.x), split_join_lo_word(hi.y, lo.y),
+                     split_join_hi_word(hi.y, lo.y));
+    *b = make_float4(split_join_lo_word(hi.z, lo.z), split_join_hi_word(hi.z, lo.z), split_join_lo_word(hi.w, lo.w),
+                     split_join_hi_word(hi.w, lo.w));
+}
+
+__device__ inline void split_widen_hi8(uint4 hi, float4 *a, float4 *b)
+{
+    *a = make_float4(__builtin_bit_cast(float, hi.x << 16), __builtin_bit_cast(float, hi.x & 0xFFFF0000u),
+                     __builtin_bit_cast(float, hi.y << 16), __builtin_bit_cast(float, hi.y & 0xFFFF0000u));
+    *b = make_float4(__builtin_bit_cast(float, hi.z << 16), __builtin_bit_cast(float, hi.z & 0xFFFF0000u),
+                     __builtin_bit_cast(float, hi.w << 16), __builtin_bit_cast(float, hi.w & 0xFFFF0000u));
+}
+
+}
diff --git a/rust-local-rag_amd/csrc/scan.hip b/rust-local-rag_amd/csrc/scan.hip
--- a/rust-local-rag_amd/csrc/scan.hip
+++ b/rust-local-rag_amd/csrc/scan.hip
@@ -3,6 +3,7 @@
 
 #include "common.h"
 #include "kernels.h"
+#include "row_layout.h"
 #include "../../include/rlr_gpu.h"
 
 namespace rlr {
@@ -68,6 +69,7 @@
                                                          uint32_t n_rows, uint32_t group_rows,
                                                          QueryArg<KQ ? CH : 0> qarg = QueryArg<KQ ? CH : 0>())
 {
+    static_assert(F16, "plain rows are binary16 only: f32 rows are split (row_layout.h) and take scan_split_kernel");
     constexpr int P16 = CH * 64;
     constexpr int QF4 = F16 ? 2 * P16 : P16;
     __shared__ float4 s_q[QF4];
@@ -145,6 +147,15 @@
     }
 }
 
+__device__ inline float4 ld_split4_nt(const uint2 *hi, const uint2 *lo)
+{
+    typedef unsigned int u32x2 __attribute__((ext_vector_type(2)));
+    const u32x2 h = __builtin_nontemporal_load(reinterpret_cast<const u32x2 *>(hi));
+    const u32x2 l = __builtin_nontemporal_load(reinterpret_cast<const u32x2 *>(lo));
+    return make_float4(split_join_lo_word(h.x, l.x), split_join_hi_word(h.x, l.x), split_join_lo_word(h.y, l.y),
+                       split_join_hi_word(h.y, l.y));
+}
+
 template <int CH, int Q>
 __global__ __launch_bounds__(256) void scan_multi_kernel(const float4 *__restrict__ rows, const float *__restrict__ queries,
                                                          uint32_t q_pitch, uint32_t n_queries, float *__restrict__ scores,
@@ -178,10 +189,10 @@
 #pragma unroll
             for (int rr = 0; rr < R; ++rr) {
                 const uint32_t row = min(row0 + r + rr, row0 + nr - 1);
-                const float4 *p = rows + static_cast<size_t>(row) * P16 + lane;
+                const uint2 *p = reinterpret_cast<const uint2 *>(rows + static_cast<size_t>(row) * P16) + lane;
 #pragma unroll
                 for (int c = 0; c < CH; ++c)
-                    x[rr][c] = ld16<true>(p + c * 64);
+                    x[rr][c] = ld_split4_nt(p + c * 64, p + P16 + c * 64);
             }
 #pragma unroll
             for (int rr = 0; rr < R; ++rr) {
@@ -304,6 +315,7 @@
                                                           uint32_t *__restrict__ g_hist,
                                                           uint32_t n_rows, uint32_t group_rows)
 {
+    static_assert(F16, "plain rows are binary16 only: f32 rows are split (row_layout.h) and take scan_split_kernel");
     constexpr int G = PackShape<P16>::G, M = PackShape<P16>::M, R = PackShape<P16>::R;
     constexpr int QF4 = F16 ? 2 * P16 : P16;
     __shared__ float4 s_q[QF4];
@@ -402,6 +414,7 @@
                                                            uint32_t n_rows, uint32_t group_rows,
                                                            uint32_t pitch16)
 {
+    static_assert(F16, "plain rows are binary16 only: f32 rows are split (row_layout.h) and take scan_split_generic_kernel");
     extern __shared__ __attribute__((aligned(16))) unsigned char s_raw[];
     uint32_t *s_hist = reinterpret_cast<uint32_t *>(s_raw);
     float4 *s_q = reinterpret_cast<float4 *>(s_raw + kHistBins * sizeof(uint32_t));
@@ -446,6 +459,216 @@
 #pragma unroll
                     for (int rr = 0; rr < R; ++rr)
                         acc[rr] = dot4(x[rr], q0, acc[rr]);
+                }
+            }
+#pragma unroll
+            for (int rr = 0; rr < R; ++rr) {
+                const float tot = wave_sum(acc[rr]);
+                if (static_cast<uint32_t>(lane) == r + rr)
+                    mine = tot;
+            }
+        }
+        if (static_cast<uint32_t>(lane) < nr) {
+            scores[row0 + lane] = mine;
+            if (g_hist)
+                atomicAdd(&s_hist[score_key(mine) >> 21], 1u);
+        }
+    }
+    if (g_hist) {
+        __syncthreads();
+        hist_flush(s_hist, g_hist);
+    }
+}
+
+template <int N>
+struct QueryArgN {
+    float4 v[N];
+};
+
+__device__ inline float dot8b(uint4 raw, float4 q0, float4 q1, float acc)
+{
+    float4 a, b;
+    split_widen_hi8(raw, &a, &b);
+    return dot4(b, q1, dot4(a, q0, acc));
+}
+
+template <bool NT>
+__device__ inline uint4 ld16u(const uint4 *p)
+{
+    if constexpr (NT) {
+        typedef unsigned int u32x4 __attribute__((ext_vector_type(4)));
+        const u32x4 v = __builtin_nontemporal_load(reinterpret_cast<const u32x4 *>(p));
+        return make_uint4(v.x, v.y, v.z, v.w);
+    } else {
+        return *p;
+    }
+}
+
+template <int H16>
+struct SplitShape {
+    static constexpr int G = 64 / pack_gcd(H16, 64);
+    static constexpr int M = G * H16 / 64;
+    static constexpr int R = M >= 9 ? 1 : (M >= 5 ? 2 : (M >= 2 ? 4 : 8));
+};
+
+template <int H16, bool FULL, bool KQ>
+__global__ __launch_bounds__(256) void scan_split_kernel(const uint4 *__restrict__ rows, const float *__restrict__ query,
+                                                         float *__restrict__ scores, uint32_t *__restrict__ g_hist,
+                                                         uint32_t n_rows, uint32_t group_rows,
+                                                         QueryArgN<KQ ? 2 * H16 : 0> qarg = QueryArgN<KQ ? 2 * H16 : 0>())
+{
+    constexpr int G = SplitShape<H16>::G, M = SplitShape<H16>::M;
+    constexpr int R = FULL ? (SplitShape<H16>::R + 1) / 2 : SplitShape<H16>::R;
+    constexpr int QF4 = 2 * H16;
+    constexpr int PITCH = 2 * H16;
+    __shared__ float4 s_q[QF4];
+    __shared__ uint32_t s_hist[kHistBins];
+
+    const int tid = threadIdx.x;
+    const int lane = tid & 63;
+    const int wave = __builtin_amdgcn_readfirstlane(tid >> 6);
+    if constexpr (KQ) {
+        for (int i = tid; i < QF4; i += 256) {
+            const float4 v = qarg.v[i];
+            s_q[i] = v;
+            if (blockIdx.x == 0)
+                reinterpret_cast<float4 *>(const_cast<float *>(query))[i] = v;
+        }
+    } else {
+        for (int i = tid; i < QF4; i += 256)
+            s_q[i] = reinterpret_cast<const float4 *>(query)[i];
+    }
+    for (int i = tid; i < kHistBins; i += 256)
+        s_hist[i] = 0;
+    __syncthreads();
+
+    float4 qv[2 * M];
+    uint32_t kof[M];
+    uint32_t col[M];
+#pragma unroll
+    for (int j = 0; j < M; ++j) {
+        kof[j] = static_cast<uint32_t>(j * 64 + lane) / H16;
+        col[j] = static_cast<uint32_t>(j * 64 + lane) % H16;
+        qv[2 * j] = s_q[2 * col[j]];
+        qv[2 * j + 1] = s_q[2 * col[j] + 1];
+    }
+
+    const uint32_t n_groups = (n_rows + group_rows - 1) / group_rows;
+    const uint32_t n_waves = gridDim.x * 4;
+    for (uint32_t g = blockIdx.x * 4 + wave; g < n_groups; g += n_waves) {
+        const uint32_t row0 = g * group_rows;
+        const uint32_t nr = min(group_rows, n_rows - row0);
+        float mine = 0.0f;
+        for (uint32_t r = 0; r < nr; r += R * G) {
+            uint4 x[R][M], y[FULL ? R : 1][FULL ? M : 1];
+#pragma unroll
+            for (int rr = 0; rr < R; ++rr) {
+#pragma unroll
+                for (int j = 0; j < M; ++j) {
+                    const uint32_t row = min(row0 + r + rr * G + kof[j], row0 + nr - 1);
+                    x[rr][j] = ld16u<true>(rows + static_cast<size_t>(row) * PITCH + col[j]);
+                    if constexpr (FULL)
+                        y[rr][j] = ld16u<true>(rows + static_cast<size_t>(row) * PITCH + H16 + col[j]);
+                }
+            }
+            auto dot8 = [&](int rr, int j, float acc) -> float {
+                if constexpr (FULL) {
+                    float4 a, b;
+                    split_decode8(x[rr][j], y[rr][j], &a, &b);
+                    return dot4(b, qv[2 * j + 1], dot4(a, qv[2 * j], acc));
+                } else {
+                    return dot8b(x[rr][j], qv[2 * j], qv[2 * j + 1], acc);
+                }
+            };
+#pragma unroll
+            for (int rr = 0; rr < R; ++rr) {
+                float acc[G];
+#pragma unroll
+                for (int k = 0; k < G; ++k)
+                    acc[k] = 0.0f;
+#pragma unroll
+                for (int j = 0; j < M; ++j) {
+                    const int g_lo = (j * 64) / H16, g_hi = (j * 64 + 63) / H16;
+                    if (g_lo == g_hi) {
+                        acc[g_lo] = dot8(rr, j, acc[g_lo]);
+                    } else {
+                        const float t = dot8(rr, j, 0.0f);
+#pragma unroll
+                        for (int k = 0; k < G; ++k)
+                            if (k >= g_lo && k <= g_hi)
+                                acc[k] += kof[j] == static_cast<uint32_t>(k) ? t : 0.0f;
+                    }
+                }
+#pragma unroll
+                for (int k = 0; k < G; ++k) {
+                    const float tot = wave_sum(acc[k]);
+                    if (static_cast<uint32_t>(lane) == r + rr * G + k)
+                        mine = tot;
+                }
+            }
+        }
+        if (static_cast<uint32_t>(lane) < nr) {
+            scores[row0 + lane] = mine;
+            if (g_hist)
+                atomicAdd(&s_hist[score_key(mine) >> 21], 1u);
+        }
+    }
+    if (g_hist) {
+        __syncthreads();
+        hist_flush(s_hist, g_hist);
+    }
+}
+
+template <int R, bool FULL>
+__global__ __launch_bounds__(256) void scan_split_generic_kernel(const uint4 *__restrict__ rows, const float *__restrict__ query,
+                                                                 float *__restrict__ scores, uint32_t *__restrict__ g_hist,
+                                                                 uint32_t n_rows, uint32_t group_rows, uint32_t half16)
+{
+    extern __shared__ __attribute__((aligned(16))) unsigned char s_raw[];
+    uint32_t *s_hist = reinterpret_cast<uint32_t *>(s_raw);
+    float4 *s_q = reinterpret_cast<float4 *>(s_raw + kHistBins * sizeof(uint32_t));
+
+    const int tid = threadIdx.x;
+    const int lane = tid & 63;
+    const int wave = __builtin_amdgcn_readfirstlane(tid >> 6);
+    for (uint32_t i = tid; i < 2 * half16; i += 256)
+        s_q[i] = reinterpret_cast<const float4 *>(query)[i];
+    for (int i = tid; i < kHistBins; i += 256)
+        s_hist[i] = 0;
+    __syncthreads();
+
+    const uint32_t n_groups = (n_rows + group_rows - 1) / group_rows;
+    const uint32_t n_waves = gridDim.x * 4;
+    for (uint32_t g = blockIdx.x * 4 + wave; g < n_groups; g += n_waves) {
+        const uint32_t row0 = g * group_rows;
+        const uint32_t nr = min(group_rows, n_rows - row0);
+        float mine = 0.0f;
+        for (uint32_t r = 0; r < nr; r += R) {
+            float acc[R];
+            const uint4 *p[R];
+#pragma unroll
+            for (int rr = 0; rr < R; ++rr) {
+                acc[rr] = 0.0f;
+                const uint32_t row = min(row0 + r + rr, row0 + nr - 1);
+                p[rr] = rows + static_cast<size_t>(row) * 2 * half16;
+            }
+            for (uint32_t c = lane; c < half16; c += 64) {
+                uint4 x[R], y[R];
+#pragma unroll
+                for (int rr = 0; rr < R; ++rr) {
+                    x[rr] = ld16u<true>(p[rr] + c);
+                    if constexpr (FULL)
+                        y[rr] = ld16u<true>(p[rr] + half16 + c);
+                }
+                const float4 q0 = s_q[2 * c], q1 = s_q[2 * c + 1];
+#pragma unroll
+                for (int rr = 0; rr < R; ++rr) {
+                    float4 a, b;
+                    if constexpr (FULL)
+                        split_decode8(x[rr], y[rr], &a, &b);
+                    else
+                        split_widen_hi8(x[rr], &a, &b);
+                    acc[rr] = dot4(b, q1, dot4(a, q0, acc[rr]));
                 }
             }
 #pragma unroll
@@ -491,8 +714,6 @@
         group = 64;
         while (group > 16 && (a.n_rows + group - 1) / group < max_blocks * 4 * 4)
             group >>= 1;
-        if (a.dtype == RLR_F32 && a.pitch16 == 192)
-            group = 16;
     }
     if (group > 64)
         group = 64;
@@ -501,14 +722,7 @@
         group = p.r;
     if (r_code == 0 && ((v >> 8) & 0xFF) == 0 && ((v >> 16) & 0xFF) == 0) {
         const uint32_t elems = a.dtype == RLR_F16 ? a.pitch16 * 8 : a.pitch16 * 4;
-        if (elems == a.dim && a.dtype == RLR_F32 && a.pitch16 == 192) {
-            p.r = 4;
-            blocks_per_cu = 1;
-            group = 8;
-        } else if (elems == a.dim && a.dtype == RLR_F32 && a.pitch16 == 384) {
-            blocks_per_cu = 1;
-            group = 8;
-        } else if (elems == a.dim && a.dtype == RLR_F16 && a.pitch16 == 192) {
+        if (elems == a.dim && a.dtype == RLR_F16 && a.pitch16 == 192) {
             blocks_per_cu = 1;
             group = 16;
         }
@@ -533,35 +747,96 @@
     return on;
 }
 
+uint32_t split_pack_h16(const ScanArgs &a)
+{
+    const uint32_t h16 = a.pitch16 / 2;
+    if (a.dim != h16 * 8 || (a.variant & 0x20))
+        return 0;
+    switch (h16) {
+    case 8: case 16: case 32: case 48: case 64: case 96: case 128: case 192: case 256: return h16;
+    default: return 0;
+    }
+}
+
+bool split_takes_kq(const ScanArgs &a)
+{
+    const uint32_t h16 = split_pack_h16(a);
+    return a.query_host && h16 != 0 && h16 <= 96 && kq_enabled();
+}
+
+template <int H16, bool FULL>
+hipError_t launch_split_one(const ScanArgs &a, hipStream_t s)
+{
+    using S = SplitShape<H16>;
+    constexpr uint32_t packs = FULL ? (S::R + 1) / 2 : S::R;
+    constexpr uint32_t step = packs * S::G;
+    constexpr uint32_t loads = S::M * packs * (FULL ? 2 : 1);
+    const int v = a.variant;
+    const bool small = (a.n_rows + 15) / 16 < static_cast<uint32_t>(a.n_cu) * 4 * 4 * 3;
+    uint32_t bpc = (v >> 8) & 0xFF;
+    if (bpc == 0)
+        bpc = loads >= 12 ? 1u : (small ? 8u : 4u);
+    uint32_t group = (v >> 16) & 0xFF;
+    if (group == 0)
+        group = FULL ? 8 : 16;
+    group = std::min<uint32_t>(64, std::max<uint32_t>(group, step));
+    const uint32_t n_groups = (a.n_rows + group - 1) / group;
+    const uint32_t blocks = std::max<uint32_t>(1, std::min<uint32_t>((n_groups + 3) / 4, static_cast<uint32_t>(a.n_cu) * bpc));
+    const uint4 *rows = static_cast<const uint4 *>(a.rows);
+    if constexpr (H16 <= 96) {
+        if (split_takes_kq(a)) {
+            QueryArgN<2 * H16> q;
+            std::memcpy(q.v, a.query_host, sizeof(q.v));
+            hipLaunchKernelGGL((scan_split_kernel<H16, FULL, true>), dim3(blocks), dim3(256), 0, s, rows, a.query, a.scores,
+                               a.hist, a.n_rows, group, q);
+            return hipGetLastError();
+        }
+    }
+    hipLaunchKernelGGL((scan_split_kernel<H16, FULL, false>), dim3(blocks), dim3(256), 0, s, rows, a.query, a.scores, a.hist,
+                       a.n_rows, group);
+    return hipGetLastError();
+}
+
+template <int H16>
+hipError_t launch_split_pack(const ScanArgs &a, hipStream_t s)
+{
+    return a.full_rows ? launch_split_one<H16, true>(a, s) : launch_split_one<H16, false>(a, s);
+}
+
+hipError_t launch_scan_split(const ScanArgs &a, hipStream_t s)
+{
+    switch (split_pack_h16(a)) {
+    case 8: return launch_split_pack<8>(a, s);
+    case 16: return launch_split_pack<16>(a, s);
+    case 32: return launch_split_pack<32>(a, s);
+    case 48: return launch_split_pack<48>(a, s);
+    case 64: return launch_split_pack<64>(a, s);
+    case 96: return launch_split_pack<96>(a, s);
+    case 128: return launch_split_pack<128>(a, s);
+    case 192: return launch_split_pack<192>(a, s);
+    case 256: return launch_split_pack<256>(a, s);
+    default: break;
+    }
+    ScanPlan p = plan_scan(a);
+    const uint32_t half16 = a.pitch16 / 2;
+    const size_t lds = kHistBins * sizeof(uint32_t) + static_cast<size_t>(half16) * 32;
+    p.group_rows = std::max<uint32_t>((p.group_rows / 2) * 2, 2);
+    const uint4 *rows = static_cast<const uint4 *>(a.rows);
+    if (a.full_rows)
+        hipLaunchKernelGGL((scan_split_generic_kernel<2, true>), dim3(p.blocks), dim3(256), lds, s, rows, a.query, a.scores,
+                           a.hist, a.n_rows, p.group_rows, half16);
+    else
+        hipLaunchKernelGGL((scan_split_generic_kernel<2, false>), dim3(p.blocks), dim3(256), lds, s, rows, a.query, a.scores,
+                           a.hist, a.n_rows, p.group_rows, half16);
+    return hipGetLastError();
+}
+
 template <int CH>
-hipError_t launch_fixed_kq(const ScanArgs &a, const ScanPlan &p, hipStream_t s)
-{
-    const float4 *rows = static_cast<const float4 *>(a.rows);
-    QueryArg<CH> q;
-    std::memcpy(q.v, a.query_host, sizeof(q.v));
-#define RLR_SCAN_KQ_CASE(RV)                                                                                  \
-    hipLaunchKernelGGL((scan_fixed_kernel<CH, RV, false, true, true>), dim3(p.blocks), dim3(256), 0, s, rows, \
-                       a.query, a.scores, a.hist, a.n_rows, p.group_rows, q)
-    switch (p.r) {
-    case 1: RLR_SCAN_KQ_CASE(1); break;
-    case 2: RLR_SCAN_KQ_CASE(2); break;
-    case 8: RLR_SCAN_KQ_CASE(8); break;
-    default: RLR_SCAN_KQ_CASE(4); break;
-    }
-#undef RLR_SCAN_KQ_CASE
-    return hipGetLastError();
-}
-
-template <int CH, bool F16>
 hipError_t launch_fixed(const ScanArgs &a, const ScanPlan &p, hipStream_t s)
 {
-    if constexpr (!F16 && CH <= 3) {
-        if (a.query_host && p.nt && kq_enabled())
-            return launch_fixed_kq<CH>(a, p, s);
-    }
     const float4 *rows = static_cast<const float4 *>(a.rows);
 #define RLR_SCAN_CASE(RV, NTV)                                                                    \
-    hipLaunchKernelGGL((scan_fixed_kernel<CH, RV, F16, NTV>), dim3(p.blocks), dim3(256), 0, s,   \
+    hipLaunchKernelGGL((scan_fixed_kernel<CH, RV, true, NTV>), dim3(p.blocks), dim3(256), 0, s,  \
                        rows, a.query, a.scores, a.hist, a.n_rows, p.group_rows)
     if (p.nt) {
         switch (p.r) {
@@ -600,13 +875,13 @@
     return true;
 }
 
-template <int CH, bool F16>
+template <int CH>
 hipError_t launch_fixed_wide(const ScanArgs &a, ScanPlan p, hipStream_t s)
 {
     p.r = 2;
     p.group_rows = std::max<uint32_t>((p.group_rows / 2) * 2, 2);
     p.blocks = std::max<uint32_t>(1, std::min<uint32_t>(p.blocks, ((a.n_rows + p.group_rows - 1) / p.group_rows + 3) / 4));
-    hipLaunchKernelGGL((scan_fixed_kernel<CH, 2, F16, true>), dim3(p.blocks), dim3(256), 0, s,
+    hipLaunchKernelGGL((scan_fixed_kernel<CH, 2, true, true>), dim3(p.blocks), dim3(256), 0, s,
                        static_cast<const float4 *>(a.rows), a.query, a.scores, a.hist, a.n_rows, p.group_rows);
     return hipGetLastError();
 }
@@ -626,13 +901,11 @@
 
 bool launch_packed(const ScanArgs &a, const ScanPlan &p, hipStream_t s, hipError_t *e)
 {
-    const uint32_t elems = a.dtype == RLR_F16 ? a.pitch16 * 8 : a.pitch16 * 4;
-    if (elems != a.dim || (a.variant & 0x20))
+    if (a.pitch16 * 8 != a.dim || (a.variant & 0x20))
         return false;
-    const bool h = a.dtype == RLR_F16;
     switch (a.pitch16) {
-    case 16: *e = h ? launch_packed_one<16, true>(a, p, s) : launch_packed_one<16, false>(a, p, s); return true;
-    case 32: *e = h ? launch_packed_one<32, true>(a, p, s) : launch_packed_one<32, false>(a, p, s); return true;
+    case 16: *e = launch_packed_one<16, true>(a, p, s); return true;
+    case 32: *e = launch_packed_one<32, true>(a, p, s); return true;
     default: return false;
     }
 }
@@ -641,57 +914,43 @@
 
 bool launch_scan_takes_host_query(const ScanArgs &a)
 {
-    int ch = 0;
-    if (!a.query_host || a.n_rows == 0 || a.dtype != RLR_F32 || !fixed_shape(a, &ch) || ch > 3 || !kq_enabled())
-        return false;
-    return plan_scan(a).nt;
+    return a.n_rows != 0 && a.dtype == RLR_F32 && split_takes_kq(a);
 }
 
 hipError_t launch_scan(const ScanArgs &a, hipStream_t s)
 {
     if (a.n_rows == 0)
         return hipSuccess;
+    switch (a.dtype) {
+    case RLR_F32: return launch_scan_split(a, s);
+    case RLR_F16: break;
+    default: return hipErrorInvalidValue;
+    }
     ScanPlan p = plan_scan(a);
     int ch = 0;
     if (fixed_shape(a, &ch)) {
-        if (a.dtype == RLR_F16) {
-            if (p.r == 8) {
-                p.r = 4;
-                p.group_rows = (p.group_rows / 4) * 4;
-            }
-            switch (ch) {
-            case 1: return launch_fixed<1, true>(a, p, s);
-            case 2: return launch_fixed<2, true>(a, p, s);
-            case 3: return launch_fixed_wide<3, true>(a, p, s);
-            default: return launch_fixed_wide<4, true>(a, p, s);
-            }
+        if (p.r == 8) {
+            p.r = 4;
+            p.group_rows = (p.group_rows / 4) * 4;
         }
         switch (ch) {
-        case 1: return launch_fixed<1, false>(a, p, s);
-        case 2: return launch_fixed<2, false>(a, p, s);
-        case 3: return launch_fixed<3, false>(a, p, s);
-        case 4: return launch_fixed<4, false>(a, p, s);
-        case 5: return launch_fixed_wide<5, false>(a, p, s);
-        case 6: return launch_fixed_wide<6, false>(a, p, s);
-        default: return launch_fixed_wide<8, false>(a, p, s);
+        case 1: return launch_fixed<1>(a, p, s);
+        case 2: return launch_fixed<2>(a, p, s);
+        case 3: return launch_fixed_wide<3>(a, p, s);
+        default: return launch_fixed_wide<4>(a, p, s);
         }
     }
     hipError_t pe = hipSuccess;
     if (launch_packed(a, p, s, &pe))
         return pe;
-    const uint32_t qf4 = a.dtype == RLR_F16 ? 2 * a.pitch16 : a.pitch16;
-    const size_t lds = kHistBins * sizeof(uint32_t) + static_cast<size_t>(qf4) * 16;
+    const size_t lds = kHistBins * sizeof(uint32_t) + static_cast<size_t>(2 * a.pitch16) * 16;
     const float4 *rows = static_cast<const float4 *>(a.rows);
     p.r = 2;
     p.group_rows = (p.group_rows / 2) * 2;
     if (p.group_rows == 0)
         p.group_rows = 2;
-    if (a.dtype == RLR_F16)
-        hipLaunchKernelGGL((scan_generic_kernel<2, true>), dim3(p.blocks), dim3(256), lds, s, rows,
-                           a.query, a.scores, a.hist, a.n_rows, p.group_rows, a.pitch16);
-    else
-        hipLaunchKernelGGL((scan_generic_kernel<2, false>), dim3(p.blocks), dim3(256), lds, s, rows,
-                           a.query, a.scores, a.hist, a.n_rows, p.group_rows, a.pitch16);
+    hipLaunchKernelGGL((scan_generic_kernel<2, true>), dim3(p.blocks), dim3(256), lds, s, rows,
+                       a.query, a.scores, a.hist, a.n_rows, p.group_rows, a.pitch16);
     return hipGetLastError();
 }
 
diff --git a/rust-local-rag_amd/csrc/staged_dot.h b/rust-local-rag_amd/csrc/staged_dot.h
--- a/rust-local-rag_amd/csrc/staged_dot.h
+++ b/rust-local-rag_amd/csrc/staged_dot.h
@@ -1,6 +1,7 @@
 #pragma once
 
 #include "common.h"
+#include "row_layout.h"
 
 namespace rlr {
 
@@ -63,8 +64,13 @@
             const uint32_t idx = idx0 + NT * j;
             ci[j] = idx / units;
             uu[j] = idx - ci[j] * units;
-            if (idx < total)
-                x[j] = rows[static_cast<size_t>(s_cand[ci[j]]) * pitch16 + uu[j]];
+            if (idx < total) {
+                const float4 *row = rows + static_cast<size_t>(s_cand[ci[j]]) * pitch16;
+                if constexpr (F16)
+                    x[j] = row[uu[j]];
+                else
+                    x[j] = split_load4(row, pitch16, uu[j] * 4);
+            }
         }
 #pragma unroll
         for (int j = 0; j < kBatch; ++j) {
```
